# argsim/argsim

Hardware: AMD Instinct MI355X
Metric: sentences/sec per ELBO step (higher is better)
Workload: dtype f32; 1 GPU; BASELINE configs[1]: 1xMI355X fp32, latent_dim 128, vocab 8k, seq_len 64, batch 256 per GPU; FULL synthetic Zipf batches, dim_emb 512, 3 layers, step 20000; global_batch=256, seq_len=64, parallelism=dp1, gru=persistent

## Files before the change

argsim_amd/csrc/ctx.h:

```cpp
#pragma once
#include "../../include/argsim_vae.h"
#include "kernels.h"

#include <fcntl.h>
#include <sys/file.h>
#include <unistd.h>

#include <algorithm>
#include <cmath>
#include <cstdio>
#include <cstring>
#include <initializer_list>
#include <string>
#include <vector>

#pragma GCC visibility push(hidden)
namespace avae { namespace host {

struct ParamEntry {
    std::string name;
    int64_t offset;
    int ndim;
    int64_t shape[4];
    int g16;
    int bucket;
};

struct GruP { int64_t W, R, bW, bR; };

}}
#pragma GCC visibility pop

struct avae_ctx {
    avae_config cfg{};
    int device = 0;
    hipStream_t stream = nullptr;
    std::string err;
    std::vector<avae::host::ParamEntry> params;
    int64_t numel = 0;
    std::vector<std::pair<int64_t, int64_t>> buckets;
    float *P = nullptr, *G = nullptr, *M = nullptr, *Vv = nullptr;
    int64_t step = 0;
    avae_grad_hook hook = nullptr; void* hook_user = nullptr;
    std::vector<int> hook_pending;
    int persistent = 1;
    bool first_step_checked = false;
    int gru_ablate = 0, gru_force_slow = 0, gru_stagger = 0, gru_item = 2;
    int skinny = 1;
    int score_plan[4] = {0, 0, 0, 0};
    const int* expect_ptr[3] = {nullptr, nullptr, nullptr}; int expect_val[3] = {0, 0, 0};
    int compact = 2;
    int skip_pad = 1;
    int shared_device = 0; int lock_fd = -1;
    int dyn_split = 1;
    int dyn_thin = 1;
    int enc_top1 = 1;
    int table_l1 = 1;
    int bf16_act = 1;
    int bf16_sv = 1;
    int bf16_tn = 1;
    int logits16 = 1;
    int bf16_nt8 = 1;
    int bf16_direct = 0;
    int gru_spec = 2;
    int gru_ring = 1;
    int bwd_rs = 2;
    int knn_chunk = 0;
    int agg_chunk = 0;
    int ward_form = 0;
    int probe_chunk = 0;
    int gru_bf16 = 1;
    int64_t oE = 0, oKout = 0, oBout = 0, oWmu = 0, oBmu = 0, oWlv = 0, oBlv = 0, oWex = 0, oBex = 0;
    std::vector<avae::host::GruP> enc;
    std::vector<avae::host::GruP> dec;
    float* losses = nullptr;
    float* acc = nullptr;
    int* errw = nullptr;
    unsigned* counters = nullptr;
    float* scratch = nullptr;
    int64_t scratch_n = 0;
    char* ws = nullptr; size_t ws_cap = 0;
    int B = 0, Ss = 0, St = 0;
    int timing = 0, timing_on = 0;
    unsigned short *bfA = nullptr, *bfB = nullptr; size_t bfA_cap = 0, bfB_cap = 0;
    float* slab = nullptr; size_t slab_floats = 0;
    unsigned short* bfP = nullptr; size_t bfP_cap = 0;
    struct Stamp { hipEvent_t a, b; int cls; double flops; const int* dyn; int dyn_max; };
    std::vector<Stamp> stamps; size_t stamps_used = 0;
    int32_t* hint_dev = nullptr; volatile int32_t* hint_host = nullptr;
    const int32_t *cnt_src = nullptr, *cnt_tgt = nullptr;
};

#pragma GCC visibility push(hidden)
namespace avae { namespace host {

#define AV_CHECK(expr)                                                                              \
    do { hipError_t e_ = (expr); if (e_ != hipSuccess) {                                            \
        char b_[512]; snprintf(b_, sizeof b_, "%s:%d: %s -> %s", __FILE__, __LINE__, #expr, hipGetErrorString(e_)); \
        h->err = b_; return 1; } } while (0)
#define AV_TRY(expr) do { int r_ = (expr); if (r_) return r_; } while (0)

inline int fail(avae_ctx* h, const std::string& m) { h->err = m; return 1; }
inline int check_rows(avae_ctx* h, const char* what, int dim, const char* names, std::initializer_list<const void*> ptrs)
{
    if (dim < 4 || dim > 1024 || (dim & 3)) return fail(h, std::string(what) + ": dim must be a multiple of 4 in [4, 1024]");
    uintptr_t bits = 0;
    for (const void* p : ptrs) bits |= (uintptr_t)p;
    if (bits & 15) return fail(h, std::string(what) + ": " + names + " must be 16-byte aligned");
    return 0;
}

#define AV_GRU(expr)                                                                                                \
    do { hipError_t e_ = (expr);                                                                                    \
         if (e_ == hipErrorCooperativeLaunchTooLarge)                                                               \
             return fail(h, "persistent GRU kernel: its workgroups cannot all be resident on this device at once (occupancy query x CU count < grid); " \
                            "run with avae_set_option(\"persistent\", 0)");                                         \
         if (e_ != hipSuccess) { char b_[512]; snprintf(b_, sizeof b_, "%s:%d: %s -> %s", __FILE__, __LINE__, #expr, hipGetErrorString(e_)); \
             h->err = b_; return 1; } } while (0)

struct DeviceTurn {
    avae_ctx* h; bool held = false;
    explicit DeviceTurn(avae_ctx* h_) : h(h_) {
        if (!h->shared_device || !h->persistent) return;
        if (h->lock_fd < 0) {
            char path[64]; snprintf(path, sizeof path, "/tmp/argsim_vae_dev%d.lock", h->device);
            h->lock_fd = open(path, O_CREAT | O_RDWR, 0666);
        }
        if (h->lock_fd >= 0 && flock(h->lock_fd, LOCK_EX) == 0) held = true;
    }
    ~DeviceTurn() { if (held) { (void)hipStreamSynchronize(h->stream); (void)flock(h->lock_fd, LOCK_UN); } }
};

struct Timed {
    avae_ctx* h; avae_ctx::Stamp* s = nullptr;
    Timed(avae_ctx* h_, int cls, double flops, const int* dyn = nullptr, int dyn_max = 0) : h(h_) {
        if (!h->timing) return;
        if (h->stamps_used == h->stamps.size()) {
            avae_ctx::Stamp n{};
            if (hipEventCreate(&n.a) != hipSuccess || hipEventCreate(&n.b) != hipSuccess) return;
            h->stamps.push_back(n);
        }
        s = &h->stamps[h->stamps_used++];
        s->cls = cls; s->flops = flops; s->dyn = dyn; s->dyn_max = dyn_max;
        (void)hipEventRecord(s->a, h->stream);
    }
    ~Timed() { if (s) (void)hipEventRecord(s->b, h->stream); }
};

struct Ws {
    int32_t *src_tm, *lens_src, *lens_tgt, *lead, *gold, *rank, *cidx, *ntok, *pred;
    float *emb_src, *emb_tgt, *ew, *dew;
    std::vector<float*> e_gi, e_hs, e_sv[2], e_hp[2];
    std::vector<float*> d_gi, d_hd, d_sv, d_hp;
    float *hpick, *mu, *lv, *z, *eps, *kld, *h0;
    float *xlast, *gib, *svb, *dgib, *dghb, *dxl;
    float *hc, *ho, *logits;
    float *loss_samp, *errt_samp;
    float *dho, *dhc, *dhd[2], *dgi_d, *dgh_d, *dh0, *carry, *dh0sum, *dz, *dmu, *dlv, *dhpick;
    float *dhs[2], *dgi_e, *dgh_e, *demb_src, *demb_tgt;
    std::vector<unsigned short*> e_hs16, d_hd16, e_hp16[2], d_hp16;
    std::vector<char> act_e, act_d, acth_e, acth_d;
    std::vector<unsigned short*> x16_e, x16_d;
    const unsigned short* x16_kept_e(int i) const { return x16_valid ? x16_e[i] : nullptr; }
    const unsigned short* x16_kept_d(int i) const { return x16_valid ? x16_d[i] : nullptr; }
    bool x16_valid = false;
    unsigned short *dgi16_d, *dgh16_d, *dgi16_e, *dgh16_e;
    int32_t* scat;
    int32_t *grp_src, *grp_tgt;
    int32_t *tokrow_src, *tokrow_tgt;
    float* xbuf; size_t xbuf_floats;
    int32_t *ord_perm[3], *ord_slens[3]; int ord_T[3], ord_cpj[3]; bool ord_ok[3];
    int32_t *map_src, *nact_src, *nsrc; bool compact;
    int32_t *map_tgt, *nact_tgt, *ntgt; bool compact_d;
    int Bx;
    int bx_enc() const { return compact ? Bx : 0; }
    int bx_dec() const { return compact_d ? Bx : 0; }
};

struct Bump {
    char* base; size_t off = 0;
    template <class T> T* take(size_t n) {
        off = (off + 255) & ~(size_t)255;
        T* p = base ? reinterpret_cast<T*>(base + off) : nullptr;
        off += n * sizeof(T);
        return p;
    }
    template <class T> T* opt(bool on, size_t n) { return on ? take<T>(n) : nullptr; }
};

struct Pair { const float* A; const float* B; float* C; const float* bias; };

struct GemmCall {
    const float* A; int lda; bool a_mc;
    const float* B; int ldb; bool b_nc;
    float* C; int ldc;
    int M, N, K;
    float alpha = 1.f; const float* bias = nullptr; int accumulate = 0;
    const int* dyn = nullptr; int dyn_kind = 0;
    const Pair* pair = nullptr;
    bool wgrad = false;
    bool allow_atomic = false;
    bool rows_are_batch = false;
    int thin = -1, split_k = 0;
    const unsigned short* A16 = nullptr; const unsigned short* B16 = nullptr;
    unsigned short* keep_a16 = nullptr;
    unsigned short* c16 = nullptr;

    GemmCall& scaled(float a) { alpha = a; return *this; }
    GemmCall& biased(const float* b) { bias = b; return *this; }
    GemmCall& plus() { accumulate = 1; return *this; }
    GemmCall& rows(const int* d) { dyn = d; dyn_kind = d ? 1 : 0; return *this; }
    GemmCall& depth(const int* d) { dyn = d; dyn_kind = d ? 2 : 0; return *this; }
    GemmCall& with(const Pair* p) { pair = p; return *this; }
    GemmCall& atomic() { allow_atomic = true; return *this; }
    GemmCall& batch_rows() { rows_are_batch = true; return *this; }
    GemmCall& form(int thin_, int split_k_ = 1) { thin = thin_; split_k = split_k_; return *this; }
    GemmCall& a16(const unsigned short* p) { A16 = p; return *this; }
    GemmCall& b16(const unsigned short* p) { B16 = p; return *this; }
    GemmCall& keep(unsigned short* p) { keep_a16 = p; return *this; }
};
inline GemmCall nt(const float* A, int lda, const float* B, int ldb, float* C, int ldc, int M, int N, int K) { return GemmCall{A, lda, false, B, ldb, false, C, ldc, M, N, K}; }
inline GemmCall nn(const float* A, int lda, const float* B, int ldb, float* C, int ldc, int M, int N, int K) { return GemmCall{A, lda, false, B, ldb, true, C, ldc, M, N, K}; }
inline GemmCall tn_grad(const float* A, int lda, const float* B, int ldb, float* C, int ldc, int M, int N, int K)
{
    GemmCall c{A, lda, true, B, ldb, true, C, ldc, M, N, K};
    c.wgrad = true;
    return c;
}

bool use_table(const avae_ctx* h, int rows, int B);
void layout(avae_ctx* h, Bump& b, Ws& w, int B, int Ss, int St, bool train);
int reserve_ws(avae_ctx* h, size_t need);
inline int reserve_named(avae_ctx* h, size_t need, const char* what)
{
    if (reserve_ws(h, need)) {
        (void)hipGetLastError();
        char b[256]; snprintf(b, sizeof b, "%s: the device cannot give the workspace of %zu bytes this call needs", what, need);
        h->err = b;
        return 1;
    }
    return 0;
}
int get_ws(avae_ctx* h, Ws& w, int B, int Ss, int St, bool train);
int gemm(avae_ctx* h, const GemmCall& c);
int gemm_tn16(avae_ctx* h, const GemmCall& c);
void gru_geometry(int D, int njobs, int B, int* G, int* rpg);
void gru_common(avae_ctx* h, const Ws& w, GruArgs& a, int njobs, int S, int B, int ldg, int ldh, const int32_t* lens, int Bx);
int build_row_orders(avae_ctx* h, Ws& w, int B, int Ss, int T, bool with_dec, bool with_enc = true);
int build_compact_dec(avae_ctx* h, Ws& w, int B, int T);
int run_decoder_rnn(avae_ctx* h, Ws& w, int B, int T, const float* state_in, int64_t state_stride, bool save, const int32_t* ids0 = nullptr, bool compact = false,
                    const int32_t* share_rows = nullptr, int share_n = 0);
int run_logits_ce(avae_ctx* h, Ws& w, int rt, bool train, float inv_n);
int encode_ws(avae_ctx* h, Ws& w, const int32_t* src, int b, int t);
inline PrepArgs prep_from_ws(const Ws& w)
{
    PrepArgs p{};
    p.src_tm = w.src_tm; p.lens_src = w.lens_src; p.lens_tgt = w.lens_tgt; p.lead = w.lead; p.gold = w.gold;
    p.rank = w.rank; p.cidx = w.cidx; p.ntok = w.ntok; p.chunk_counts = w.ntok + 4;
    return p;
}

int grow_scratch(avae_ctx* h, size_t need, const char* what);
int check_gru_err(avae_ctx* h);
int dyn_fraction(avae_ctx* h, const avae_ctx::Stamp& s, std::vector<std::pair<const int*, int>>& seen, double* f);
inline int check_bound(avae_ctx* h)
{
    if (!h->P || !h->G || !h->M || !h->Vv) return fail(h, "state buffers not bound (avae_bind_state)");
    return 0;
}
template <class F> int place_scratch(avae_ctx* h, const char* what, F lay)
{
    Bump probe{nullptr};
    lay(probe);
    AV_TRY(grow_scratch(h, probe.off, what));
    Bump real{reinterpret_cast<char*>(h->scratch)};
    lay(real);
    return 0;
}
template <class F> int place_ws(avae_ctx* h, const char* what, F lay, size_t from = 0)
{
    Bump probe{nullptr, from};
    lay(probe);
    AV_TRY(reserve_named(h, probe.off + 4096, what));
    Bump real{h->ws, from};
    lay(real);
    return 0;
}

bool sample_params(avae_ctx* h, const avae_sample_config* sc, int V, SampleParams* sp);
bool sample_params_p(avae_ctx* h, const avae_sample_p_config* sc, int V, SampleParams* sp, float* top_p);

}}
#pragma GCC visibility pop
```

argsim_amd/csrc/handle.cpp:

```cpp
#include "ctx.h"

using namespace avae;
using namespace avae::host;

static std::string g_create_err;

namespace avae { namespace host {

int grow_scratch(avae_ctx* h, size_t need, const char* what)
{
    if (h->scratch_n >= (int64_t)need) return 0;
    AV_CHECK(hipStreamSynchronize(h->stream));
    if (h->scratch) AV_CHECK(hipFree(h->scratch));
    h->scratch = nullptr; h->scratch_n = 0;
    if (hipMalloc(reinterpret_cast<void**>(&h->scratch), need) != hipSuccess) {
        (void)hipGetLastError();
        h->scratch = nullptr;
        char b_[256]; snprintf(b_, sizeof b_, "%s: %.0f MB of scratch could not be allocated on the device", what, (double)need / 1048576.0);
        return fail(h, b_);
    }
    h->scratch_n = (int64_t)need;
    return 0;
}

// ... 69 lines not shown
int check_gru_err(avae_ctx* h)
{
    int e = 0;
    AV_CHECK(hipMemcpyAsync(&e, h->errw, sizeof(int), hipMemcpyDeviceToHost, h->stream));
    AV_CHECK(hipStreamSynchronize(h->stream));
    if (e) {
        (void)hipMemsetAsync(h->errw, 0, sizeof(int), h->stream);
        return fail(h, "GRU persistent kernel: an exchange wait timed out -- its workgroups were not all resident at once.  A persistent "
                       "launch needs every CU of the device (one handle = one GPU = one process, include/argsim_vae.h): another process or "
                       "stream computing on this GPU holds CUs the launch is waiting for.  Give the handle the device to itself, or "
                       "run with avae_set_option(\"persistent\", 0) (one launch per time step)");
    }
    return 0;
}
int dyn_fraction(avae_ctx* h, const avae_ctx::Stamp& s, std::vector<std::pair<const int*, int>>& seen, double* f)
{
    *f = 1.0;
    if (!s.dyn || s.dyn_max <= 0) return 0;
    int c = -1;
    for (auto& e : seen) if (e.first == s.dyn) c = e.second;
    if (c < 0) {
        AV_CHECK(hipMemcpy(&c, s.dyn, sizeof(int), hipMemcpyDeviceToHost));
        if (c < 0) c = 0;
        seen.push_back({s.dyn, c});
    }
    *f = (double)std::min(c, s.dyn_max) / (double)s.dyn_max;
    return 0;
}

}}

extern "C" {

int avae_create(const avae_config* cfg, int device, avae_handle* out)
{
    if (!cfg || !out) { g_create_err = "null argument"; return 1; }
    *out = nullptr;
    if (!gru_dim_supported(cfg->dim_emb)) { g_create_err = "dim_emb must be one of 16, 32, 64, 128, 256, 512 (the GRU kernels are instantiated for these widths only; the reference leaves dim_emb free, config.json uses 512)"; return 1; }
    if (cfg->compute_dtype < 0 || cfg->compute_dtype > 2) { g_create_err = "compute_dtype must be 0 (fp32 MFMA), 1 (bf16 GEMM operands) or 2 (fp32 via split bf16 MFMA)"; return 1; }
    if (cfg->dim_rep % 4 || cfg->dim_tgt % 4 || cfg->rnn_layers < 1 || cfg->rnn_layers > 8) { g_create_err = "dim_rep and dim_tgt must be multiples of 4 (16-byte rows); 1 <= rnn_layers <= 8"; return 1; }
    int ndev = 0;
    if (hipGetDeviceCount(&ndev) != hipSuccess || ndev <= 0) { g_create_err = "no HIP device available: the gfx950 kernels cannot run (no CPU fallback)"; return 1; }
    if (device < 0 || device >= ndev) { g_create_err = "bad device index"; return 1; }
    avae_ctx* h = new avae_ctx();
    h->cfg = *cfg; h->device = device;
    if (h->cfg.kl_beta == 0.f) h->cfg.kl_beta = 1.f;
    build_params(h);
    hipError_t e = hipSetDevice(device);
    if (e == hipSuccess) e = hipMalloc(reinterpret_cast<void**>(&h->losses), 64 * sizeof(float));
    if (e == hipSuccess) e = hipMalloc(reinterpret_cast<void**>(&h->errw), 128 * sizeof(int));
    if (e == hipSuccess) e = hipMalloc(reinterpret_cast<void**>(&h->counters), 2048 * sizeof(unsigned));
    if (e == hipSuccess) e = hipMemset(h->losses, 0, 64 * sizeof(float));
    if (e == hipSuccess) e = hipMemset(h->errw, 0, 128 * sizeof(int));
    if (e == hipSuccess) e = hipMemset(h->counters, 0, 2048 * sizeof(unsigned));
    if (e != hipSuccess) { g_create_err = std::string("hip init failed: ") + hipGetErrorString(e); delete h; return 1; }
    h->acc = h->losses + 8;
    *out = h;
    return 0;
}

void avae_destroy(avae_handle h)
{
    if (!h) return;
    (void)hipSetDevice(h->device);
    if (h->stream) (void)hipStreamSynchronize(h->stream); else (void)hipDeviceSynchronize();
    if (h->ws) (void)hipFree(h->ws);
    if (h->losses) (void)hipFree(h->losses);
    if (h->errw) (void)hipFree(h->errw);
    if (h->hint_host) (void)hipHostFree(const_cast<int32_t*>(h->hint_host));
    if (h->counters) (void)hipFree(h->counters);
    if (h->scratch) (void)hipFree(h->scratch);
    if (h->bfA) (void)hipFree(h->bfA);
    if (h->slab) (void)hipFree(h->slab);
    if (h->bfP) (void)hipFree(h->bfP);
    if (h->bfB) (void)hipFree(h->bfB);
    if (h->lock_fd >= 0) (void)close(h->lock_fd);
    delete h;
}

const char* avae_last_error(avae_handle h) { return h ? h->err.c_str() : g_create_err.c_str(); }

int avae_set_stream(avae_handle h, void* s) { if (!h) return 1; h->stream = reinterpret_cast<hipStream_t>(s); return 0; }

int avae_get_dims(avae_handle h, int32_t* V, int32_t* D, int32_t* R, int32_t* L)
{
    if (!h) return 1;
    if (V) *V = h->cfg.dim_tgt; if (D) *D = h->cfg.dim_emb; if (R) *R = h->cfg.dim_rep; if (L) *L = h->cfg.rnn_layers;
    return 0;
}

int64_t avae_state_numel(avae_handle h) { return h ? h->numel : 0; }

int avae_bind_state(avae_handle h, float* p, float* g, float* m, float* v)
{
    if (!h) return 1;
    if (((uintptr_t)p | (uintptr_t)g | (uintptr_t)m | (uintptr_t)v) & 15) return fail(h, "state buffers must be 16-byte aligned");
    h->P = p; h->G = g; h->M = m; h->Vv = v;
    return 0;
}

int avae_param_count(avae_handle h) { return h ? (int)h->params.size() : 0; }
const char* avae_param_name(avae_handle h, int i) { return (h && i >= 0 && i < (int)h->params.size()) ? h->params[i].name.c_str() : nullptr; }

int avae_param_info(avae_handle h, const char* name, int64_t* offset, int32_t* ndim, int64_t shape[4])
{
    if (!h) return 1;
    const ParamEntry* e = find_param(h, name);
    if (!e) return fail(h, std::string("unknown variable: ") + (name ? name : "(null)"));
    if (offset) *offset = e->offset; if (ndim) *ndim = e->ndim;
    if (shape) for (int i = 0; i < 4; ++i) shape[i] = e->shape[i];
    return 0;
}

static int xfer_tensor(avae_handle h, const char* name, int kind, float* buf, bool get)
{
    if (!h) return 1;
    AV_TRY(check_bound(h));
    const ParamEntry* e = find_param(h, name);
    if (!e) return fail(h, std::string("unknown variable: ") + (name ? name : "(null)"));
    float* base = state_buf(h, kind);
    if (!base) return fail(h, "bad tensor kind");
    float* flat = base + e->offset;
    int64_t n = e->shape[0] * e->shape[1] * e->shape[2] * e->shape[3];
    if (!e->g16) {
        AV_CHECK(hipMemcpyAsync(get ? buf : flat, get ? flat : buf, n * sizeof(float), hipMemcpyDeviceToDevice, h->stream));
    } else {
        int D = h->cfg.dim_emb, cols = (int)(e->ndim == 2 ? e->shape[1] : 1);
        if (get) AV_CHECK(g16_permute(h->stream, buf, flat, D, cols, false));
        else     AV_CHECK(g16_permute(h->stream, flat, buf, D, cols, true));
    }
    return 0;
}
int avae_get_tensor(avae_handle h, const char* name, int kind, float* buf) { return xfer_tensor(h, name, kind, buf, true); }
int avae_set_tensor(avae_handle h, const char* name, int kind, const float* buf) { return xfer_tensor(h, name, kind, const_cast<float*>(buf), false); }

int avae_get_step(avae_handle h, int64_t* s) { if (!h || !s) return 1; *s = h->step; return 0; }
int avae_set_step(avae_handle h, int64_t s) { if (!h) return 1; h->step = s; return 0; }

int avae_set_grad_hook(avae_handle h, avae_grad_hook hook, void* user) { if (!h) return 1; h->hook = hook; h->hook_user = user; return 0; }

int avae_set_option(avae_handle h, const char* key, int value)
{
    if (!h || !key) return 1;
    if (!strcmp(key, "persistent")) { h->persistent = value; return 0; }
    if (!strcmp(key, "gru_item")) { h->gru_item = value; return 0; }
    if (!strcmp(key, "gru_stagger")) { h->gru_stagger = value; return 0; }
    if (!strcmp(key, "gru_force_slow")) { h->gru_force_slow = value; return 0; }
    if (!strcmp(key, "gru_bf16")) { h->gru_bf16 = value != 0; return 0; }
    if (!strcmp(key, "bwd_rs")) { h->bwd_rs = value; return 0; }
    if (!strcmp(key, "dyn_split")) { h->dyn_split = value != 0; return 0; }
    if (!strcmp(key, "shared_device")) { h->shared_device = value != 0; return 0; }
    if (!strcmp(key, "gru_spec")) { h->gru_spec = value; return 0; }
    if (!strcmp(key, "gru_ring")) { h->gru_ring = value != 0; return 0; }
    if (!strcmp(key, "bf16_nt8")) { h->bf16_nt8 = value != 0; return 0; }
    if (!strcmp(key, "logits16")) { h->logits16 = value != 0; return 0; }
    if (!strcmp(key, "bf16_direct")) { h->bf16_direct = value != 0; return 0; }
    if (!strcmp(key, "bf16_tn")) { h->bf16_tn = value != 0; return 0; }
    if (!strcmp(key, "bf16_sv")) { h->bf16_sv = value != 0; return 0; }
    if (!strcmp(key, "bf16_act")) { h->bf16_act = value != 0; return 0; }
    if (!strcmp(key, "table_l1")) { h->table_l1 = value != 0; return 0; }
    if (!strcmp(key, "enc_top1")) { h->enc_top1 = value != 0; return 0; }
    if (!strcmp(key, "dyn_thin")) { h->dyn_thin = value != 0; return 0; }
    if (!strcmp(key, "skip_pad")) { h->skip_pad = value != 0; return 0; }
    if (!strcmp(key, "compact")) { h->compact = value; return 0; }
    if (!strcmp(key, "skinny")) { h->skinny = value; return 0; }
    if (!strcmp(key, "knn_chunk")) { if (value < 0) return fail(h, "knn_chunk must be >= 0"); h->knn_chunk = value; return 0; }
    if (!strcmp(key, "agg_chunk")) { if (value < 0) return fail(h, "agg_chunk must be >= 0"); h->agg_chunk = value; return 0; }
    if (!strcmp(key, "ward_form")) { if (value < 0 || value > 2) return fail(h, "ward_form must be 0 (planner), 1 (one-workgroup) or 2 (launch-per-merge)"); h->ward_form = value; return 0; }
    if (!strcmp(key, "probe_chunk")) { if (value < 0) return fail(h, "probe_chunk must be >= 0"); h->probe_chunk = value; return 0; }
    if (!strcmp(key, "gru_ablate")) {
        if (value && !gru_diag_build()) return fail(h, "gru_ablate needs the diagnostic build of libargsim_vae.so (make -C argsim_amd/csrc DIAG=1)");
        h->gru_ablate = value; return 0;
    }
    if (!strcmp(key, "timing")) { h->timing = value; h->timing_on = value; h->stamps_used = 0; return 0; }
    if (!strcmp(key, "timing_pause")) { h->timing = value ? 0 : h->timing_on; return 0; }
    return fail(h, "unknown option");
}
int avae_timing_collect(avae_handle h, double* out)
{
    if (!h || !out) return 1;
    AV_CHECK(hipStreamSynchronize(h->stream));
    for (int i = 0; i < 9; ++i) out[i] = 0.0;
    std::vector<std::pair<const int*, int>> seen;
    for (size_t i = 0; i < h->stamps_used; ++i) {
        float ms = 0.f;
        AV_CHECK(hipEventElapsedTime(&ms, h->stamps[i].a, h->stamps[i].b));
        double f = 1.0;
        AV_TRY(dyn_fraction(h, h->stamps[i], seen, &f));
        int c = h->stamps[i].cls;
        out[3 * c] += ms; out[3 * c + 1] += 1.0; out[3 * c + 2] += h->stamps[i].flops * f;
    }
    h->stamps_used = 0;
    return 0;
}
int avae_bucket_count(avae_handle h) { return h ? (int)h->buckets.size() : 0; }
int avae_bucket_info(avae_handle h, int i, int64_t* offset, int64_t* count)
{
    if (!h || i < 0 || i >= (int)h->buckets.size()) return 1;
    *offset = h->buckets[i].first; *count = h->buckets[i].second; return 0;
}

}
```

argsim_amd/csrc/hooks.cpp:

```cpp
#include "ctx.h"

using namespace avae;
using namespace avae::host;

extern "C" {

int avae_debug_team_batch(int32_t B) { return B > 0 ? gru_team_batch(B) : 0; }
int avae_debug_gemm_plan(const int32_t* in, int32_t n, int32_t* out)
{
    if (!in || !out || n < 0) return 1;
    for (int r = 0; r < n; ++r, in += 19, out += 15) {
        const GemmShape s{in[0] != 0, in[1] != 0, in[2], in[3], in[4], in[5], in[6], in[7], in[8], in[9], in[10], in[11] != 0, in[12] != 0,
                          in[13] != 0, in[14] != 0, in[15], in[16] != 0, in[17] != 0, in[18] != 0};
        const GemmPlan p = gemm_plan(s);
        out[0] = p.n;
        for (int i = 0; i < 2; ++i) {
            const GemmLaunch l = i < p.n ? p.launch[i] : GemmLaunch{0, 0, 0, 0, 0, 0, 0};
            const int32_t f[7] = {l.row0, l.rows, l.thin, l.split_k, l.accumulate, l.zero, l.dyn};
            std::copy(f, f + 7, out + 1 + 7 * i);
        }
    }
    return 0;
}
int avae_debug_gemm_call(avae_handle h, int a_mc, int b_nc, const float* A, const float* Bm, float* Cm, const float* bias, int M, int N, int K,
// ... 22 lines not shown
        return fail(h, "avae_debug_gemm_forced: thin in 0..3, split_k >= 1, dyn_kind in 0..2 with a count exactly where it is not 0");
    GemmCall c{A, lda, a_mc != 0, Bm, ldb, b_nc != 0, Cm, ldc, M, N, K};
    c.alpha = alpha; c.bias = bias; c.accumulate = accumulate;
    if (dyn_kind == 2) c.depth(count); else c.rows(count);
    c.form(thin, split_k);
    const Pair second{A2, B2, C2, bias2};
    if (A2) c.pair = &second;
    const int* const was_ptr = h->expect_ptr[0]; const int was_val = h->expect_val[0];
    h->expect_ptr[0] = count; h->expect_val[0] = expect;
    const int r = gemm(h, c);
    h->expect_ptr[0] = was_ptr; h->expect_val[0] = was_val;
    return r;
}
int avae_debug_gemm_f32_form(int a_mc, int b_nc, int M, int N, int K, int lda, int ldb, int ldc, int accumulate, int thin, int split_k, int dyn_kind,
                             int expect, int pair, int32_t out[8])
{
    if (!out) return 1;
    alignas(16) static const float other[4] = {0.f, 0.f, 0.f, 0.f};
    const GemmArgs g{nullptr, nullptr, nullptr, nullptr, M, N, K, lda, ldb, ldc, 1.f, accumulate, split_k, nullptr, dyn_kind, expect, thin,
                     pair ? other : nullptr, pair ? other : nullptr, nullptr, nullptr};
    const GemmF32Form f = gemm_f32_form(a_mc != 0, b_nc != 0, g);
    const int32_t v[8] = {f.tile, f.fast, f.db, f.persist, (int32_t)f.gx, (int32_t)f.gy, (int32_t)f.gz, f.err != hipSuccess};
    std::copy(v, v + 8, out);
    return 0;
}
int avae_debug_score_plan(avae_handle h, int32_t out[4])
{
    if (!h || !out) return 1;
    for (int i = 0; i < 4; ++i) out[i] = h->score_plan[i];
    return 0;
}
int avae_debug_present_ids(avae_handle h, int32_t out[2])
{
    if (!h || !out) return 1;
    AV_CHECK(hipStreamSynchronize(h->stream));
    out[0] = out[1] = -1;
    if (h->cnt_src) AV_CHECK(hipMemcpy(&out[0], h->cnt_src, sizeof(int), hipMemcpyDeviceToHost));
    if (h->cnt_tgt) AV_CHECK(hipMemcpy(&out[1], h->cnt_tgt, sizeof(int), hipMemcpyDeviceToHost));
    return 0;
}
int avae_debug_train_ce(avae_handle h, float* out, int32_t max_n, int32_t* n_out)
{
    if (!h || !out || !n_out) return 1;
    if (h->B < 1) return fail(h, "avae_debug_train_ce: no training forward has run on this handle");
    Ws w;
    AV_TRY(get_ws(h, w, h->B, h->Ss, h->St, true));
    int n = 0;
    AV_CHECK(hipMemcpyAsync(&n, w.ntok, sizeof(int), hipMemcpyDeviceToHost, h->stream));
    AV_CHECK(hipStreamSynchronize(h->stream));
    n = std::min(n, (int)max_n);
    AV_CHECK(hipMemcpyAsync(out, w.loss_samp, (size_t)n * sizeof(float), hipMemcpyDeviceToDevice, h->stream));
    *n_out = n;
    return 0;
}
int avae_debug_timing(avae_handle h, double* out, int max_n, int* n)
{
    if (!h || !out || !n) return 1;
    AV_CHECK(hipStreamSynchronize(h->stream));
    *n = (int)std::min<size_t>(h->stamps_used, (size_t)max_n);
    std::vector<std::pair<const int*, int>> seen;
    for (int i = 0; i < *n; ++i) {
        float ms = 0.f;
        AV_CHECK(hipEventElapsedTime(&ms, h->stamps[i].a, h->stamps[i].b));
        double f = 1.0;
        AV_TRY(dyn_fraction(h, h->stamps[i], seen, &f));
        const double fl = h->stamps[i].flops * f;
        out[3 * i] = h->stamps[i].cls; out[3 * i + 1] = ms; out[3 * i + 2] = fl;
    }
    return 0;
}
int avae_debug_stamps(avae_handle h, unsigned long long* out)
{
    if (!h || !out) return 1;
    AV_CHECK(hipStreamSynchronize(h->stream));
    AV_CHECK(hipMemcpy(out, h->errw + 16, 32 * sizeof(unsigned long long), hipMemcpyDeviceToHost));
    AV_CHECK(hipMemset(h->errw + 16, 0, 32 * sizeof(unsigned long long)));
    return 0;
}
int avae_debug_gemm(avae_handle h, int a_mc, int b_nc, const float* A, const float* Bm, float* Cm, const float* bias,
                    int M, int N, int K, int lda, int ldb, int ldc, float alpha, int accumulate, int split_k)
{
    if (!h) return 1;
    GemmCall c{A, lda, a_mc != 0, Bm, ldb, b_nc != 0, Cm, ldc, M, N, K};
    c.alpha = alpha; c.bias = bias; c.accumulate = accumulate;
    return gemm(h, c.form(split_k == -3 ? 3 : (split_k < 0 ? 1 : (split_k >= 1000 ? 2 : 0)), split_k < 0 ? 1 : (split_k >= 1000 ? split_k - 1000 : split_k)));
}
int avae_debug_gemm_dyn(avae_handle h, const float* A, const float* Bm, float* Cm, int M, int N, int K, const int* rows)
{
    if (!h) return 1;
    return gemm(h, nt(A, K, Bm, K, Cm, N, M, N, K).rows(rows).form(0));
}
int avae_debug_gemm_c16(avae_handle h, const float* A, const float* Bm, unsigned short* C16, int M, int N, int K, float alpha, const int* rows)
{
    if (!h) return 1;
    if (h->cfg.compute_dtype != 1 || !gemm_bf16_c16_takes(M, N, K, rows, h->bf16_nt8)) return 3;
    GemmCall c = nt(A, K, Bm, K, nullptr, N, M, N, K).scaled(alpha).rows(rows).form(0);
    c.c16 = C16;
    return gemm(h, c);
}
int avae_debug_gemm_tn16(avae_handle h, const float* A, const float* Bm, float* Cm, int M, int N, int K, int lda, int ldb, int ldc, float alpha)
{
    if (!h) return 1;
    return gemm_tn16(h, tn_grad(A, lda, Bm, ldb, Cm, ldc, M, N, K).scaled(alpha));
}
int avae_debug_softmax_ce(avae_handle h, float* logits, unsigned short* panel, int logits16, const int32_t* gold, const int32_t* cidx,
                          const int32_t* n_dev, int n_max, int V, int write_grad, float inv_n, float* loss_samp, float* errt,
                          int32_t* pred, int* form_out)
{
    if (!h || !form_out) return 1;
    CeArgs c{};
    c.logits = logits; c.gold = gold; c.cidx = cidx; c.n_dev = n_dev; c.n_max = n_max; c.V = V;
    c.write_grad = write_grad; c.inv_n = inv_n;
    c.loss_samp = loss_samp; c.errt_samp = errt; c.pred = pred; c.loss_acc = nullptr;
    c.grad16 = panel; c.logits16 = logits16;
    *form_out = softmax_ce_form(c);
    AV_CHECK(softmax_ce(h->stream, c));
    return 0;
}
int avae_debug_argmax_rows(avae_handle h, const float* logits, int32_t* pred, int n, int V)
{
    if (!h) return 1;
    AV_CHECK(argmax_rows(h->stream, logits, pred, n, V));
    return 0;
}
int avae_debug_op_layout(int64_t n, int64_t V, int64_t out[6])
{
    if (!out || n < 0 || V < 0) return 1;
    int32_t base[1];
    out[0] = (int64_t)embed_scatter_scratch_ints((size_t)n, (size_t)V);
    out[1] = (int64_t)id_groups_ints((size_t)n, (size_t)V);
    out[2] = id_groups_rank(base, (int)n, (int)V) - base;
    out[3] = id_groups_uid(base, (int)n, (int)V) - base;
    out[4] = id_groups_count(base, (int)n, (int)V) - base;
    out[5] = id_groups_supported((int)V) ? 1 : 0;
    return 0;
}
int avae_debug_op(avae_handle h, const char* op, void* const* p, const int64_t* i, const float* f)
{
    if (!h || !op || !p || !i || !f) return 1;
    const std::string o(op);
    hipStream_t st = h->stream;
    auto F = [&](int k) { return static_cast<float*>(p[k]); };
    auto I = [&](int k) { return static_cast<int32_t*>(p[k]); };
    if (o == "prep_ids") {
        PrepArgs a{};
        a.src = I(0); a.tgt = I(1); a.keep_mask = static_cast<const uint8_t*>(p[2]); a.src_tm = I(3); a.lens_src = I(4); a.lens_tgt = I(5);
        a.lead = I(6); a.gold = I(7); a.rank = I(8); a.cidx = I(9); a.ntok = I(10); a.zero2 = F(11); a.chunk_counts = I(12);
        a.B = (int)i[0]; a.Ss = (int)i[1]; a.St = (int)i[2]; a.eos = (int)i[3]; a.bos = (int)i[4]; a.train = (int)i[5]; a.seed = (uint64_t)i[6];
        a.keepwd = f[0];
        AV_CHECK(prep_ids(st, a));
    } else if (o == "embed_gather") AV_CHECK(embed_gather(st, F(0), I(1), F(2), (int)i[0], (int)i[1], (int)i[2]));
    else if (o == "embed_scatter_add2") AV_CHECK(embed_scatter_add2(st, F(0), I(1), F(2), (int)i[0], I(3), F(4), (int)i[1], (int)i[2], (int)i[3], I(5)));
    else if (o == "id_groups_build") AV_CHECK(id_groups_build(st, I(0), (int)i[0], (int)i[1], I(1), i[2] != 0));
    else if (o == "rank_rows") AV_CHECK(rank_rows(st, I(0), I(1), I(2), (int)i[0], (int)i[1]));
    else if (o == "rows_gather_ranked") AV_CHECK(rows_gather_ranked(st, F(0), F(1), I(2), I(3), (int)i[0], (int)i[1], (int)i[2]));
    else if (o == "rows_group_sum") AV_CHECK(rows_group_sum(st, F(0), I(1), F(2), (int)i[0], (int)i[1], (int)i[2], I(3)));
    else if (o == "rows_add_indexed") AV_CHECK(rows_add_indexed(st, F(0), F(1), I(2), I(3), (int)i[0], (int)i[1]));
    else if (o == "rows_gather") AV_CHECK(rows_gather(st, F(0), F(1), I(2), I(3), (int)i[0], (int)i[1], I(4)));
    else if (o == "rows_expand") AV_CHECK(rows_expand(st, F(0), F(1), I(2), (int)i[0], (int)i[1], I(3)));
    else if (o == "zero_rows_dyn") AV_CHECK(zero_rows_dyn(st, F(0), I(1), (int)i[0], (int)i[1]));
    else if (o == "zero_fill") AV_CHECK(zero_fill(st, p[0], (size_t)i[0]));
    else if (o == "row_order") {
        RowOrder ro[4];
        const int n = (int)i[0];
        for (int k = 0; k < std::min(n, 4); ++k) ro[k] = RowOrder{I(3 * k), (int)i[5 + 3 * k], (int)i[6 + 3 * k], (int)i[7 + 3 * k], I(3 * k + 1), I(3 * k + 2)};
        AV_CHECK(row_order(st, ro, n, (int)i[1], (int)i[2], (int)i[3], I(3 * std::min(std::max(n, 0), 4)), (int)i[4]));
    } else if (o == "row_map") AV_CHECK(row_map(st, I(0), (int)i[0], (int)i[1], (int)i[2], I(1), I(2), I(3)));
    else if (o == "pick_last") AV_CHECK(pick_last(st, F(0), F(1), I(2), (int)i[0], (int)i[1], I(3)));
    else if (o == "pick_last16") AV_CHECK(pick_last16(st, F(0), static_cast<const unsigned short*>(p[1]), I(2), (int)i[0], (int)i[1], I(3)));
    else if (o == "pick_last_add") AV_CHECK(pick_last_add(st, F(0), F(1), I(2), (int)i[0], (int)i[1], I(3)));
    else if (o == "pick_last_bwd") AV_CHECK(pick_last_bwd(st, F(0), F(1), I(2), (int)i[0], (int)i[1], (int)i[2]));
    else if (o == "latent_fwd") AV_CHECK(latent_fwd(st, F(0), F(1), F(2), F(3), F(4), F(5), (int)i[0], (int)i[1], (uint64_t)i[2], f[0], F(6)));
    else if (o == "latent_bwd") AV_CHECK(latent_bwd(st, F(0), F(1), F(2), F(3), F(4), F(5), (int)i[0], (int)i[1], f[0], f[1]));
    else if (o == "colsum") AV_CHECK(colsum(st, F(0), (int)i[0], (int)i[1], (int)i[2], F(1), I(2)));
    else if (o == "add3") AV_CHECK(add3(st, F(0), F(1), F(2), F(3), i[0]));
    else if (o == "finalize_losses") AV_CHECK(finalize_losses(st, F(0), F(1), I(2), (int)i[0], F(3), (int)i[1], f[0], f[1], f[2]));
    else if (o == "adam_tf") {
        const AdamArgs a{F(0), F(1), F(2), F(3), i[0], f[0], f[1], f[2], f[3], static_cast<const int*>(p[4])};
        AV_CHECK(adam_tf(st, a));
    } else if (o == "g16_permute") AV_CHECK(g16_permute(st, F(0), F(1), (int)i[0], (int)i[1], i[2] != 0));
    else if (o == "gru_first_step_fwd") AV_CHECK(gru_first_step_fwd(st, F(0), F(1), F(2), (int)i[0], F(3), (int)i[1], (int)i[2], I(4)));
    else if (o == "gru_first_step_bwd") AV_CHECK(gru_first_step_bwd(st, F(0), (int)i[0], F(1), F(2), F(3), (int)i[1], (int)i[2], I(4)));
    else return fail(h, "avae_debug_op: no such launcher: " + o);
    return 0;
}

static void gru_shape(const int64_t* i, GruArgs& a)
{
    a.njobs = (int)i[0]; a.S = (int)i[1]; a.B = (int)i[2]; a.D = (int)i[3]; a.ldg = (int)i[4]; a.ldh = (int)i[5]; a.Bx = (int)i[6];
    a.G = (int)i[7]; a.rows_per_group = (int)i[8]; a.p_begin = (int)i[9]; a.p_end = (int)i[10]; a.item_pipeline = (int)i[11];
    a.bf16 = (int)i[12]; a.bwd_rs = (int)i[13]; a.xbuf_floats = (size_t)std::max<int64_t>(i[14], 0);
    if (a.G == 0 && a.D >= 16 && a.njobs >= 1 && a.B >= 1) gru_geometry(a.D, a.njobs, a.B, &a.G, &a.rows_per_group);
}
static void gru_plan_out(const GruArgs& a, const GruPlan& p, int64_t out[10])
{
    const int64_t v[10] = {(int64_t)p.form, p.T, p.C, p.cpj, p.Bg, p.pipe, a.G, a.rows_per_group, (int64_t)gru_bwd_rs_xbuf_floats(a.njobs, p.Bg), p.ring};
    std::copy(v, v + 10, out);
}
int avae_debug_gru_plan(const int64_t* i, int fwd, int persistent, int64_t out[10])
{
    if (!i || !out) return 1;
    alignas(16) static float dummy[4] = {0.f, 0.f, 0.f, 0.f};
    GruArgs a{};
    gru_shape(i, a);
    a.xbuf = a.xbuf_floats > 0 ? dummy : nullptr; a.ring = 1;
    gru_plan_out(a, gru_plan(a, fwd != 0, persistent != 0), out);
    return 0;
}
int avae_debug_gru(avae_handle h, int fwd, int persistent, const int64_t* i, void* const* jobs, void* const* shared, int64_t plan_out[10])
{
    if (!h || !i || !jobs || !shared || !plan_out) return 1;
    GruArgs a{};
    gru_shape(i, a);
    if (a.njobs < 1 || a.njobs > kMaxGruJobs) return fail(h, "avae_debug_gru: njobs in 1..3");
    if (a.p_begin != 0 || a.p_end != a.S) return fail(h, "avae_debug_gru: whole-sequence launches only (p_begin = 0, p_end = S)");
    a.stagger = (int)i[15]; a.force_slow = (int)i[16]; a.sv16 = (int)i[17]; a.spec = (int)i[18];
    for (int k = 0; k < a.njobs; ++k) {
        void* const* p = jobs + 19 * k;
        auto F = [&](int q) { return static_cast<float*>(p[q]); };
        auto H = [&](int q) { return static_cast<unsigned short*>(p[q]); };
        GruJob& j = a.job[k];
        j.gi = F(0); j.gi_rows = static_cast<const int32_t*>(p[1]); j.R = F(2); j.bR = F(3); j.h0 = F(4); j.hs = F(5); j.sv = F(6); j.hp = F(7);
        j.hs16 = H(8); j.hp16 = H(9); j.dh_out = F(10); j.dgi = F(11); j.dgh = F(12); j.dgi16 = H(13); j.dgh16 = H(14); j.dh0 = F(15);
        j.carry = F(16); j.dbW = F(17); j.dbR = F(18);
        j.reverse = (int)i[19 + 2 * k]; j.dgi_by_pos = (int)i[20 + 2 * k];
    }
    a.lens = static_cast<const int*>(shared[0]); a.slens = static_cast<const int*>(shared[1]); a.perm = static_cast<const int*>(shared[2]);
    a.rowmap = static_cast<const int*>(shared[3]); a.xbuf = static_cast<float*>(shared[4]);
    a.counters = h->counters; a.err = h->errw; a.stamps = reinterpret_cast<unsigned long long*>(h->errw + 16); a.ablate = 0;
    a.ring = h->gru_ring;
    gru_plan_out(a, gru_plan(a, fwd != 0, persistent != 0), plan_out);
    AV_CHECK(hipSetDevice(h->device));
    AV_GRU(fwd ? gru_forward(h->stream, a, persistent != 0) : gru_backward(h->stream, a, persistent != 0));
    return check_gru_err(h);
}

int avae_debug_sample_rows(avae_handle h, const float* logits, int n, int V, int t0, const avae_sample_config* sc, int32_t* pred, float* logp)
{
    if (!h) return 1;
    SampleParams sp{};
    if (!sample_params(h, sc, V, &sp)) return 1;
    if (n < 1 || V < 1 || t0 < 0 || t0 >= (1 << 20)) return fail(h, "sample rows: bad shape or step");
    AV_CHECK(sample_rows(h->stream, logits, n, V, t0, sp, nullptr, h->cfg.eos, pred, logp));
    return 0;
}

int avae_debug_sample_rows_p(avae_handle h, const float* logits, int n, int V, int t0, const avae_sample_p_config* sc, int32_t* pred, float* logp,
                             int32_t* nkept, const int32_t* lead)
{
    if (!h) return 1;
    SampleParams sp{};
    float top_p = 0.f;
    if (!sample_params_p(h, sc, V, &sp, &top_p)) return 1;
    if (n < 1 || V < 1 || t0 < 0 || t0 >= (1 << 20)) return fail(h, "sample rows: bad shape or step");
    if (top_p > 0.f) AV_CHECK(sample_rows_p(h->stream, logits, n, V, t0, sp, top_p, lead, h->cfg.eos, pred, logp, nkept));
    else {
        AV_CHECK(sample_rows(h->stream, logits, n, V, t0, sp, lead, h->cfg.eos, pred, logp));
        if (nkept) AV_CHECK(hipMemsetAsync(nkept, 0xff, (size_t)n * sizeof(int32_t), h->stream));
    }
    return 0;
}

int avae_debug_beam_select(avae_handle h, const float* logits, int n, int width, int V, const float* cum, const int32_t* fin,
                           int32_t* parent, int32_t* token, float* cum_out, int32_t* fin_out)
{
    if (!h) return 1;
    if (!logits || !cum || !fin || !parent || !token || !cum_out || !fin_out) return fail(h, "beam select: every array must be given");
    if (n < 1 || n > (1 << 20) || V < 1 || width < 1 || width > 32 || width > V) return fail(h, "beam select: bad shape or width");
    AV_CHECK(hipSetDevice(h->device));
    const size_t rows = (size_t)n * width;
    float *cand_sc, *lat_cum; int32_t *cand_tok, *cand_cnt, *len_out, *live;
    AV_TRY(place_scratch(h, "beam select", [&](Bump& b) {
        cand_sc = b.take<float>(rows * width); lat_cum = b.take<float>(rows);
        cand_tok = b.take<int32_t>(rows * width); cand_cnt = b.take<int32_t>(rows); len_out = b.take<int32_t>(rows); live = b.take<int32_t>(1);
    }));
    AV_CHECK(beam_rows(h->stream, logits, (int)rows, V, width, cum, fin, h->cfg.eos, cand_sc, cand_tok, cand_cnt));
    BeamStep a{};
    a.n = n; a.Win = width; a.W = width; a.eos = h->cfg.eos;
    a.cand_sc = cand_sc; a.cand_tok = cand_tok; a.cand_cnt = cand_cnt; a.fin_in = fin; a.len_in = nullptr;
    a.lat_parent = parent; a.lat_token = token; a.lat_cum = lat_cum; a.cum_out = cum_out; a.fin_out = fin_out; a.len_out = len_out;
    a.live = live;
    AV_CHECK(hipMemsetAsync(a.live, 0, sizeof(int32_t), h->stream));
    AV_CHECK(beam_select(h->stream, a));
    return 0;
}
int avae_debug_latent_plan(int kind, int64_t n, int64_t N, int k_or_P, int dim, int chunk_opt, int32_t out[5])
{
    if (!out || kind < 0 || kind > 2 || n < 0 || n > 0x7fffffff || N < 0 || N > 0x7fffffff) return 1;
    if (kind == 0) { const KnnPlan p = knn_plan((int)n, (int)N, k_or_P, chunk_opt); const int32_t f[5] = {p.qrows, p.qtiles, 0, p.parts, p.chunk}; std::copy(f, f + 5, out); }
    else if (kind == 1) { const AggPlan p = agg_plan((int)n, (int)N, dim, chunk_opt); const int32_t f[5] = {0, p.qtiles, 0, p.parts, p.chunk}; std::copy(f, f + 5, out); }
    else { const ProbePlan p = probe_plan((int)N, k_or_P, dim, chunk_opt); const int32_t f[5] = {p.ptiles, p.Ppad, p.LD, p.parts, p.chunk}; std::copy(f, f + 5, out); }
    return 0;
}

}
```

argsim_amd/csrc/kernels.h:

```cpp
#pragma once
#include <hip/hip_runtime.h>
#include <stdint.h>

#include "gemm_plan.h"

namespace avae {

struct GemmArgs {
    const float* A; const float* B; float* C; const float* bias;
    int M, N, K, lda, ldb, ldc;
    float alpha;
    int accumulate;
    int split_k;
    const int* dyn; int dyn_kind;
    int dyn_expect;
    int thin;
    const float* A2; const float* B2; float* C2; const float* bias2;
    float* slab = nullptr; size_t slab_floats = 0;
    unsigned short* c16 = nullptr;
    int nt8 = 1;
};
hipError_t gemm_f32(hipStream_t st, bool a_mc, bool b_nc, const GemmArgs& g);
struct GemmF32Form { int tile; bool fast, db, persist; unsigned gx, gy, gz; hipError_t err; };
GemmF32Form gemm_f32_form(bool a_mc, bool b_nc, const GemmArgs& g);
hipError_t gemm_f32s(hipStream_t st, bool a_mc, bool b_nc, const GemmArgs& g);
hipError_t gemm_bf16_direct(hipStream_t st, bool a_mc, bool b_nc, const GemmArgs& g);

hipError_t cvt_bf16(hipStream_t st, const float* src, int ld, bool transpose, int rows_or_K, int cols_or_X,
                    unsigned short* dst, int ldd);
hipError_t gemm_bf16_nt(hipStream_t st, const unsigned short* A, int lda, const unsigned short* B, int ldb, const GemmArgs& g);
bool gemm_bf16_p8_ok(const GemmArgs& g, int lda, int ldb);
hipError_t gemm_bf16_p8(hipStream_t st, const unsigned short* A, int lda, const unsigned short* B, int ldb, const GemmArgs& g, int s2);
bool gemm_bf16_c16_ok(const GemmArgs& g, int lda, int ldb);
bool gemm_bf16_c16_takes(int M, int N, int K, const int* rows, int nt8);
bool gemm_bf16_p8_tn_ok(const GemmArgs& g, int lda, int ldb);
hipError_t gemm_bf16_p8_tn(hipStream_t st, const unsigned short* A, int lda, const unsigned short* B, int ldb, const GemmArgs& g, int s2);
hipError_t gemm_bf16_tn(hipStream_t st, const unsigned short* A, int lda, const unsigned short* B, int ldb, const GemmArgs& g);
hipError_t transpose_bf16(hipStream_t st, const unsigned short* src, int ld, int K, int X, unsigned short* dst, int ldk);

constexpr int kMaxGruJobs = 3;
struct GruJob {
    const float* gi;
    const int32_t* gi_rows;
    const float* R;
    const float* bR;
    const float* h0;
    float* hs;
    float* sv;
    float* hp;
    int reverse;
    unsigned short* hs16;
    unsigned short* hp16;
    const float* dh_out;
    float* dgi;
    float* dgh;
    unsigned short* dgi16;
    unsigned short* dgh16;
    float* dh0;
    float* carry;
    int dgi_by_pos;
    float* dbW;
    float* dbR;
};
struct GruArgs {
    GruJob job[kMaxGruJobs];
    int njobs, S, B, D, ldg, ldh;
    const int* lens;
    const int* slens;
    const int* perm;
    const int* rowmap;
    int Bx;
    int G;
    int rows_per_group;
    int p_begin, p_end;
    unsigned* counters;
    int* err;
    unsigned long long* stamps;
    int item_pipeline;
    float* xbuf;
    size_t xbuf_floats;
    int stagger;
    int force_slow;
    int sv16;
    int bf16;
    int spec;
    int bwd_rs;
    int ring;
    int ablate;
};
constexpr int kGruRing = 4;
enum class GruForm { stepwise, persistent, item, team, team_rs };
struct GruPlan {
    GruForm form;
    int T, C, cpj, Bg;
    bool pipe, diag;
    int ring;
    bool team() const { return form == GruForm::team || form == GruForm::team_rs; }
    bool full() const { return team() && !diag; }
};
GruPlan gru_plan(const GruArgs& a, bool fwd, bool persistent);
hipError_t gru_forward(hipStream_t st, const GruArgs& a, bool persistent);
hipError_t gru_backward(hipStream_t st, const GruArgs& a, bool persistent);
int gru_team_batch(int B);
bool gru_dim_supported(int D);
size_t gru_bwd_rs_xbuf_floats(int njobs, int rows);
hipError_t gru_bwd_rs_launch(hipStream_t st, const GruArgs& a, const GruPlan& p);
hipError_t gru_fwd_team_launch(hipStream_t st, const GruArgs& a, const GruPlan& p);
hipError_t gru_bwd_team_launch(hipStream_t st, const GruArgs& a, const GruPlan& p);
hipError_t gru_reg_launch(hipStream_t st, const GruArgs& a, bool fwd, int grid, bool need_resident);
hipError_t gru_fwd_item_launch(hipStream_t st, const GruArgs& a, int grid);
hipError_t gru_first_step_fwd(hipStream_t st, const float* gi, const float* bR, float* h_out, int ldo, float* sv, int B, int D, const int32_t* lens = nullptr);
hipError_t gru_first_step_bwd(hipStream_t st, const float* dh, int ldd, const float* sv, float* dgi, float* dgh, int B, int D, const int32_t* lens = nullptr);
bool gru_diag_build();

struct PrepArgs {
    const int32_t* src; const int32_t* tgt;
    int B, Ss, St, eos, bos;
    int train; float keepwd; uint64_t seed; const uint8_t* keep_mask;
    int32_t* src_tm;
    int32_t* lens_src;
    int32_t* lens_tgt;
    int32_t* lead;
    int32_t* gold;
    int32_t* rank;
    int32_t* cidx;
    int32_t* ntok;
    float* zero2;
    int32_t* chunk_counts;
};
constexpr int kPrepChunks = 1024;
hipError_t prep_ids(hipStream_t st, const PrepArgs& p);

hipError_t embed_gather(hipStream_t st, const float* E, const int32_t* ids, float* out, int n, int D, int V);
hipError_t embed_scatter_add2(hipStream_t st, float* dE, const int32_t* ids0, const float* dout0, int n0, const int32_t* ids1,
                              const float* dout1, int n1, int D, int V, int32_t* scratch);
bool id_groups_supported(int V);
inline size_t id_groups_ints(size_t n, size_t V) { return 4 * V + 2 + n + (n / 32 + V + 1) + 2 * V + 4; }
hipError_t id_groups_build(hipStream_t st, const int32_t* ids, int n, int V, int32_t* scratch, bool lists);
const int32_t* id_groups_rank(int32_t* scratch, int n, int V);
const int32_t* id_groups_uid(int32_t* scratch, int n, int V);
const int32_t* id_groups_count(int32_t* scratch, int n, int V);
hipError_t rank_rows(hipStream_t st, int32_t* out, const int32_t* ids, const int32_t* rank, int n, int V);
hipError_t rows_gather_ranked(hipStream_t st, float* dst, const float* src, const int32_t* ids, const int32_t* rank, int n, int W, int V);
hipError_t rows_group_sum(hipStream_t st, float* dst, const int32_t* ids, const float* src, int n, int W, int V, int32_t* scratch);
hipError_t rows_add_indexed(hipStream_t st, float* dst, const float* src, const int32_t* uid, const int32_t* nuniq, int n_max, int D);
inline size_t embed_scatter_scratch_ints(size_t n, size_t V) { return 4 * V + 2 + n + (n / 32 + V + 1); }
struct RowOrder { const int32_t* lens; int add, T, cpj; int32_t* perm; int32_t* slens; };
hipError_t row_order(hipStream_t st, const RowOrder* orders, int n, int Breal, int B, int S, int32_t* steps_sum = nullptr, int sum_rows = 0);
hipError_t rows_gather(hipStream_t st, float* dst, const float* src, const int32_t* idx, const int32_t* n_dev, int n_max, int D, const int32_t* map = nullptr);
hipError_t rows_expand(hipStream_t st, float* dst, const float* src, const int32_t* rank, int rows, int D, const int32_t* map = nullptr);
hipError_t pick_last(hipStream_t st, float* h, const float* hs, const int32_t* lens, int B, int W, const int32_t* map = nullptr);
hipError_t pick_last16(hipStream_t st, float* h, const unsigned short* hs16, const int32_t* lens, int B, int W, const int32_t* map = nullptr);
hipError_t pick_last_add(hipStream_t st, float* dhs, const float* d, const int32_t* lens, int B, int W, const int32_t* map = nullptr);
hipError_t row_map(hipStream_t st, const int32_t* lens, int add, int S, int B, int32_t* map, int32_t* nact, int32_t* count);
hipError_t zero_rows_dyn(hipStream_t st, float* X, const int32_t* count, int rows_max, int W);
hipError_t pick_last_bwd(hipStream_t st, float* dhs, const float* dh, const int32_t* lens, int S, int B, int W);

hipError_t latent_fwd(hipStream_t st, const float* mu, const float* lv, const float* eps_in, float* eps_out, float* z,
                      float* kld, int n, int train, uint64_t seed, float free_bits, float* acc);
hipError_t latent_bwd(hipStream_t st, const float* dz, const float* mu, const float* lv, const float* eps_used,
                      float* dmu, float* dlv, int B, int R, float coef, float free_bits);

struct CeArgs {
    float* logits;
    const int32_t* gold;
    const int32_t* cidx;
    const int32_t* n_dev;
    int n_max, V;
    int write_grad; float inv_n;
    float* loss_samp; float* errt_samp; int32_t* pred;
    float* loss_acc;
    unsigned short* grad16;
    int logits16;
};
int softmax_ce_form(const CeArgs& a);
hipError_t softmax_ce(hipStream_t st, const CeArgs& a);
hipError_t argmax_rows(hipStream_t st, const float* logits, int32_t* pred, int n, int V);
struct SampleParams { float inv_t; int top_k; int noise; uint64_t seed; };
hipError_t sample_rows(hipStream_t st, const float* logits, int n, int V, int t, const SampleParams& sp, const int32_t* lead, int eos,
                       int32_t* pred, float* logp);
hipError_t sample_rows_p(hipStream_t st, const float* logits, int n, int V, int t, const SampleParams& sp, float top_p, const int32_t* lead,
                         int eos, int32_t* pred, float* logp, int32_t* nkept);

hipError_t colsum(hipStream_t st, const float* X, int M, int N, int ldx, float* out, const int32_t* m_dev);
hipError_t add3(hipStream_t st, float* out, const float* a, const float* b, const float* c, int64_t n);
hipError_t zero_fill(hipStream_t st, void* p, size_t bytes);

struct AdamArgs { float* p; const float* g; float* m; float* v; int64_t n; float lr_t, b1, b2, eps;
                  const int* skip_if; };
hipError_t adam_tf(hipStream_t st, const AdamArgs& a);

struct ScoreDraw {
    const float* mu; const float* lv;
    const float* eps_in;
    float* eps_out;
    float* z;
    float* lat;
    int* err;
    int k, B, R, rc; uint64_t seed;
};
hipError_t score_draw(hipStream_t st, const ScoreDraw& a);
hipError_t tile_ids(hipStream_t st, int32_t* dst, const int32_t* src, int n, int rc, int S);
hipError_t lead_rows(hipStream_t st, const int32_t* lead, int T, int n, int rc, int32_t* ids0, int32_t* tokrow);
struct ScoreRows {
    const float* loss;
    const int32_t* rank;
    int T, n, rc, k0, r0, B;
    float* logpx;
    int32_t* ntok;
};
hipError_t score_rows(hipStream_t st, const ScoreRows& a);
hipError_t score_bound(hipStream_t st, const float* logpx, const float* lat, int k, int B, float* logw, float* bound);

hipError_t beam_rows(hipStream_t st, const float* logits, int rows, int V, int W, const float* cum, const int32_t* fin, int eos,
                     float* cand_sc, int32_t* cand_tok, int32_t* cand_cnt);
struct BeamStep {
    int n, Win, W, eos;
    const float* cand_sc; const int32_t* cand_tok; const int32_t* cand_cnt;
    const int32_t* fin_in; const int32_t* len_in;
    int32_t* lat_parent; int32_t* lat_token; float* lat_cum;
    float* cum_out; int32_t* fin_out; int32_t* len_out;
    int32_t* live;
};
hipError_t beam_select(hipStream_t st, const BeamStep& a);
hipError_t beam_gather(hipStream_t st, const float* const* hd, int L, int n, int Win, int W, int D, const int32_t* parent, float* state_out);
struct BeamEnd {
    int n, W, n_run, steps, eos;
    const int32_t* lat_parent; const int32_t* lat_token; const float* lat_cum;
    const float* cum; const int32_t* len;
    const float* lenpow;
    int32_t* out_ids;
    float* score_out; float* cum_out; int32_t* len_out;
    int32_t* o_parent; int32_t* o_token; float* o_cum; size_t out_step;
};
hipError_t beam_backtrack(hipStream_t st, const BeamEnd& a);

struct KnnArgs {
    const float* q; const float* bank;
    int n, N, dim, k, metric;
    int64_t idx_base, self_base; int carry;
    int64_t* out_idx; float* out_score;
};
struct KnnPlan { int qrows, qtiles, parts, chunk; };
KnnPlan knn_plan(int n, int N, int k, int chunk_opt);
struct KnnWs { float *qn, *bn; unsigned long long* lists; };
hipError_t knn_search(hipStream_t st, const KnnArgs& g, const KnnPlan& p, const KnnWs& w);

struct AggArgs {
    const float* z; const float* mu; const float* lv;
    int n, N, dim;
    int64_t self_base;
    float* logq; float* logqx;
};
struct AggPlan { int qtiles, parts, chunk; };
AggPlan agg_plan(int n, int N, int dim, int chunk_opt);
hipError_t agg_logq(hipStream_t st, const AggArgs& g, const AggPlan& p, float2* parts_ms);
int moments_blocks(int N);
hipError_t latent_moments(hipStream_t st, const float* mu, const float* lv, int N, int dim, float* out, double* mean, double* part);

constexpr int kProbeTile = 32;
constexpr int kProbeAlphas = 7;
constexpr int kProbeMaxParts = 256;
struct ProbePlan { int ptiles, Ppad, LD, parts, chunk; };
ProbePlan probe_plan(int N, int P, int dim, int chunk_opt);
struct ProbeWs {
    float *sT, *z, *D, *u;
    float *W, *G, *Dv, *Rv, *Pv;
    float *gp, *lp;
    double* tp;
    int* is; float* fs; double* ds;
    int N, dim, LD, Ppad, parts, chunk;
    float *Yv, *Hd, *Hy;
    float* xs;
};
struct ProbeAlphas { int n, last; float a[kProbeAlphas]; };
hipError_t probe_prepare(hipStream_t st, const ProbeWs& b, const float* s, int P);
hipError_t probe_pass(hipStream_t st, const ProbeWs& b, const float* x, int mode);
hipError_t probe_vec(hipStream_t st, const ProbeWs& b, int P, int phase, int k, int max_newton, int max_cg, float tol, const ProbeAlphas& al);
hipError_t probe_trial(hipStream_t st, const ProbeWs& b, const ProbeAlphas& al);
hipError_t probe_finish(hipStream_t st, const ProbeWs& b, int P, float* w, float* stats);
hipError_t probe_l1_prepare(hipStream_t st, const ProbeWs& b, const float* x, const float* s, int P);
hipError_t probe_l1_curv(hipStream_t st, const ProbeWs& b);
hipError_t probe_l1_vec(hipStream_t st, const ProbeWs& b, int P, int phase, int k, int max_newton, int max_inner, float tol, const ProbeAlphas& al);
hipError_t probe_decision(hipStream_t st, const ProbePlan& p, const float* x, int n, int dim, const float* w, int P, float* W, float* out);

constexpr int kWardOneWgMax = 128;
struct WardGroup {
    int off, n, mrg, pad;
    float* D;
    double* S;
    int* cnt;
    unsigned long long* nn;
    int* st;
};
struct WardCutGroup { int off, n, mrg, m; };
hipError_t ward_init(hipStream_t st, const WardGroup* gs, int G, int nmax, const float* x, int dim);
hipError_t ward_tree(hipStream_t st, const WardGroup* gs, int G, int nmax, int dim, int32_t* pair, float* delta, int32_t* size);
hipError_t ward_round(hipStream_t st, const WardGroup* gs, int G, int nmax, int dim, int t, int32_t* pair, float* delta, int32_t* size);
hipError_t ward_cut(hipStream_t st, const WardCutGroup* gs, int G, int nmax, const int32_t* pair, int32_t* p , int32_t* label);

constexpr int kApMaxN = 1 << 14;
constexpr int kApMaxRB = 16;
struct ApState {
    int stop_at;
    int iters, conv, K;
    int cnt[2][2];
    float pref;
    unsigned prefix[2], rank[2];
    unsigned hist[512];
};
struct ApBuffers {
    float *S, *A, *R;
    double* part;
    double* cv;
    int *E, *run, *E2;
    int32_t* c;
    unsigned long long* best;
    ApState* st;
};
int ap_row_block(int N);
hipError_t ap_single(hipStream_t st, int32_t* label, int32_t* stat);
hipError_t ap_similarity(hipStream_t st, const float* x, int N, int dim, int metric, float* S);
hipError_t ap_prepare(hipStream_t st, float* S, int N, int use_pref, float pref, int noise, uint64_t seed, ApState* state);
hipError_t ap_iteration(hipStream_t st, const ApBuffers& b, int N, float lam, int it, int conv_iter);
hipError_t ap_labels(hipStream_t st, const ApBuffers& b, int N, int32_t* label, int32_t* stat);

struct DecodeArgs {
    const float* E;
    const float *W[8], *R[8], *bW[8], *bR[8];
    const float *Kout, *bout;
    float* state[2];
    float* o;
    float* part_val; int32_t* part_idx;
    int32_t* ids_tm;
    int32_t* out_ids;
    int32_t* kept;
    unsigned* bar;
    int* err;
    int b, steps, D, V, L, eos, cache_e; float isd;
    SampleParams sp;
    float *part_x, *part_m, *part_s;
    float* logits;
    float* logp_tm;
    float* logp_out;
    float top_p;
    int32_t* nkept_tm;
    int32_t* nkept_out;
};
hipError_t decode_greedy(hipStream_t st, DecodeArgs a, int* grid_out);
hipError_t decode_sample(hipStream_t st, DecodeArgs a, int* grid_out);
int decode_workgroups();

hipError_t g16_permute(hipStream_t st, float* dst, const float* src, int D, int cols, bool to_g16);

hipError_t finalize_losses(hipStream_t st, float* losses, const float* loss_samp, const int32_t* n_dev, int n_max,
                           const float* kld, int nk, float free_bits, float inv_br, float anneal);

}
```

argsim_amd/csrc/model.cpp:

```cpp
#include "ctx.h"

using namespace avae;

namespace avae { namespace host {

static bool phantom_batch(const avae_ctx* h, int B)
{
    return h->compact && h->skip_pad && h->persistent && h->cfg.dim_emb == 512 && gru_team_batch(B) > B;
}
bool use_table(const avae_ctx* h, int rows, int B)
{
    if (!h->table_l1 || !id_groups_supported(h->cfg.dim_tgt)) return false;
    return rows >= h->cfg.dim_tgt || (rows >= 1024 && phantom_batch(h, B));
}

void layout(avae_ctx* h, Bump& b, Ws& w, int B, int Ss, int St, bool train)
{
    const int D = h->cfg.dim_emb, V = h->cfg.dim_tgt, R = h->cfg.dim_rep, L = h->cfg.rnn_layers;
    const size_t T = St + 1, rs = (size_t)Ss * B, rt = T * B;
    w.src_tm = b.take<int32_t>(rs); w.lens_src = b.take<int32_t>(B); w.lens_tgt = b.take<int32_t>(B);
    w.lead = b.take<int32_t>(rt); w.gold = b.take<int32_t>(rt); w.rank = b.take<int32_t>(rt);
    w.cidx = b.take<int32_t>(rt); w.ntok = b.take<int32_t>(4 + kPrepChunks); w.pred = b.take<int32_t>(rt);
    w.emb_src = b.take<float>(rs * D); w.emb_tgt = b.take<float>(rt * D);
    const bool tab_s = use_table(h, (int)rs, B), tab_t = use_table(h, (int)rt, B);
// ... 238 lines not shown
struct Sched { float keepwd, anneal, lr; };
static Sched schedule(const avae_ctx* h)
{
    float rate = h->cfg.accelerate * (float)h->step;
    Sched s;
    s.keepwd = 1.f / (1.f + expf(-rate));
    s.anneal = tanhf(rate);
    s.lr = h->cfg.learn_rate / (sqrtf(rate) + 1.f);
    return s;
}

static bool top_one_step(const avae_ctx* h) { return h->enc_top1 && h->cfg.rnn_layers >= 2; }

struct FillHint { int32_t real, rows; };
static FillHint fill_hint(const avae_ctx* h)
{
    const uint64_t pair = h->hint_host ? *reinterpret_cast<const volatile uint64_t*>(h->hint_host) : 0xffffffffull;
    return {(int32_t)(uint32_t)(pair & 0xffffffffull), (int32_t)(uint32_t)(pair >> 32)};
}
static double expected_fill(const avae_ctx* h)
{
    const FillHint f = fill_hint(h);
    return (f.real > 0 && f.rows > 0) ? std::min(1.0, (double)f.real / (double)f.rows) : 1.0;
}
static int rs_pick(const avae_ctx* h)
{
    if (h->bwd_rs != 2) return h->bwd_rs;
    return expected_fill(h) < 0.40 ? 1 : 0;
}
static int spec_pick(const avae_ctx* h)
{
    if (h->gru_spec != 2) return h->gru_spec;
    return expected_fill(h) < 0.60 ? 1 : 0;
}

void gru_common(avae_ctx* h, const Ws& w, GruArgs& a, int njobs, int S, int B, int ldg, int ldh, const int32_t* lens, int Bx)
{
    const int D = h->cfg.dim_emb;
    a.njobs = njobs; a.S = S; a.B = B; a.D = D; a.ldg = ldg; a.ldh = ldh; a.lens = lens;
    a.Bx = Bx;
    gru_geometry(D, njobs, B, &a.G, &a.rows_per_group);
    a.p_begin = 0; a.p_end = S; a.counters = h->counters; a.err = h->errw; a.ablate = h->gru_ablate; a.force_slow = h->gru_force_slow;
    a.bf16 = h->cfg.compute_dtype == 1 && h->gru_bf16; a.stagger = h->gru_stagger; a.item_pipeline = h->gru_item;
    a.xbuf = w.xbuf; a.xbuf_floats = w.xbuf_floats; a.stamps = reinterpret_cast<unsigned long long*>(h->errw + 16); a.bwd_rs = h->bwd_rs != 0;
    a.ring = h->gru_ring;
}
int build_row_orders(avae_ctx* h, Ws& w, int B, int Ss, int T, bool with_dec, bool with_enc)
{
    if (!h->skip_pad || !h->persistent || w.Bx % 16) return 0;
    if (w.Bx != B && !h->compact) return 0;
    const int D = h->cfg.dim_emb;
    RowOrder ord[3]; int n = 0, which[3];
    auto want = [&](int k, int njobs, int S, int ldg, int ldh, const int32_t* lens, int add) {
        GruArgs a{};
        gru_common(h, w, a, njobs, S, B, ldg, ldh, lens, w.Bx);
        const GruPlan p = gru_plan(a, true, true);
        if (p.form != GruForm::team) return;
        ord[n] = RowOrder{lens, add, p.T, p.cpj, w.ord_perm[k], w.ord_slens[k]};
        which[n++] = k; w.ord_T[k] = p.T; w.ord_cpj[k] = p.cpj;
    };
    if (with_enc) want(0, 2, Ss, 6 * D, 2 * D, w.lens_src, 0);
    if (with_enc && top_one_step(h)) want(1, 1, Ss, 6 * D, 2 * D, w.lens_src, 0);
    if (with_dec) want(2, 1, T, 3 * D, D, w.lens_tgt, 1);
    if (!n) return 0;
    const bool hint = which[0] == 0 && h->compact == 2;
    if (hint && !h->hint_host) {
        int32_t* hp = nullptr;
        if (hipHostMalloc(reinterpret_cast<void**>(&hp), 64, hipHostMallocDefault) == hipSuccess) { hp[0] = -1; hp[1] = 0; h->hint_host = hp; }
    }
    h->hint_dev = reinterpret_cast<int32_t*>(h->errw + 100);
    hipError_t e = row_order(h->stream, ord, n, B, w.Bx, std::max(Ss, T), hint ? h->hint_dev : nullptr, Ss * B);
    if (e == hipErrorInvalidValue) return 0;
    AV_CHECK(e);
    if (hint && h->hint_host) {
        AV_CHECK(hipMemcpyAsync(const_cast<int32_t*>(h->hint_host), h->hint_dev, 2 * sizeof(int32_t), hipMemcpyDeviceToHost, h->stream));
    }
    for (int i = 0; i < n; ++i) w.ord_ok[which[i]] = true;
    return 0;
}
static bool both_team_bf16(avae_ctx* h, const GruArgs& a, bool train)
{
    return train && a.bf16 && gru_plan(a, true, h->persistent != 0).full() && gru_plan(a, false, h->persistent != 0).full();
}
static void attach_sv16(avae_ctx* h, GruArgs& a, bool train) { a.sv16 = h->bf16_sv && both_team_bf16(h, a, train); }
static void attach_order(avae_ctx* h, const Ws& w, GruArgs& a, bool fwd, int k)
{
    const GruPlan p = gru_plan(a, fwd, h->persistent != 0);
    if (!w.ord_ok[k] || !p.team() || p.T != w.ord_T[k] || p.cpj != w.ord_cpj[k]) return;
    a.slens = w.ord_slens[k]; a.perm = w.ord_perm[k];
}

static int build_compact(avae_ctx* h, Ws& w, int B, int Ss, int T, bool train)
{
    w.compact = false; w.compact_d = false;
    h->expect_ptr[0] = h->expect_ptr[1] = h->expect_ptr[2] = nullptr;
    if (!h->compact || !h->persistent || Ss < 2 || !use_table(h, Ss * B, B)) return 0;
    const bool phantom = w.Bx != B;
    if (phantom && !(w.ord_ok[0] && (w.ord_ok[1] || !top_one_step(h)))) return 0;
    if (h->compact == 2 && !phantom) {
        const FillHint f = fill_hint(h);
        if (f.real < 0 || f.rows <= 0 || (double)f.real >= 0.92 * (double)f.rows) return 0;
    }
    const int D = h->cfg.dim_emb;
    auto team = [&](int njobs, int S, int ldg, int ldh, const int32_t* lens) {
        GruArgs q{};
        gru_common(h, w, q, njobs, S, B, ldg, ldh, lens, w.Bx);
        return gru_plan(q, true, true).full() && (!train || gru_plan(q, false, true).full());
    };
    if (!team(2, Ss, 6 * D, 2 * D, w.lens_src) || (top_one_step(h) && !team(1, Ss, 6 * D, 2 * D, w.lens_src))) return 0;
    AV_CHECK(row_map(h->stream, w.lens_src, 0, Ss, B, w.map_src, w.nact_src, w.nsrc));
    w.compact = true;
    {
        const FillHint f = fill_hint(h);
        const double fill = (f.real > 0 && f.rows > 0) ? std::min(1.0, (double)f.real / (double)f.rows) : 0.0;
        h->expect_ptr[0] = w.nsrc; h->expect_val[0] = (int)(fill * Ss * B);
        h->expect_ptr[1] = w.ntgt; h->expect_val[1] = (int)(fill * T * B);
        h->expect_ptr[2] = w.ntok; h->expect_val[2] = (int)(fill * T * B);
    }
    if (T < 2 || !use_table(h, T * B, B) || h->compact == 3) return 0;
    if ((phantom && !w.ord_ok[2]) || !team(1, T, 3 * D, D, nullptr)) return 0;
    AV_CHECK(row_map(h->stream, w.lens_tgt, 1, T, B, w.map_tgt, w.nact_tgt, w.ntgt));
    w.compact_d = true;
    return 0;
}
int build_compact_dec(avae_ctx* h, Ws& w, int B, int T)
{
    w.compact = false; w.compact_d = false;
    h->expect_ptr[0] = h->expect_ptr[1] = h->expect_ptr[2] = nullptr;
    if (!h->compact || h->compact == 3 || !h->persistent || T < 2 || !use_table(h, T * B, B)) return 0;
    if (w.Bx == B || !w.ord_ok[2]) return 0;
    GruArgs q{};
    gru_common(h, w, q, 1, T, B, 3 * h->cfg.dim_emb, h->cfg.dim_emb, nullptr, w.Bx);
    if (!gru_plan(q, true, true).full()) return 0;
    AV_CHECK(row_map(h->stream, w.lens_tgt, 1, T, B, w.map_tgt, w.nact_tgt, w.ntgt));
    w.compact_d = true;
    return 0;
}

static int run_encoder(avae_ctx* h, Ws& w, int B, int Ss, bool save)
{
    const int D = h->cfg.dim_emb, V = h->cfg.dim_tgt, L = h->cfg.rnn_layers;
    const int rs = Ss * B;
    const bool table = use_table(h, rs, B);
    h->cnt_src = table ? id_groups_count(w.grp_src, rs, V) : nullptr;
    const int32_t* const cdyn = w.compact ? w.nsrc : nullptr;
    const int32_t* const cmap = w.compact ? w.map_src : nullptr;
    if (!table) AV_CHECK(embed_gather(h->stream, h->P + h->oE, w.src_tm, w.emb_src, rs, D, V));
    const float* x = w.emb_src; int In = D;
    for (int i = 0; i < L; ++i) {
        const GruP& p = h->enc[i];
        const bool top1 = i == L - 1 && top_one_step(h);
        if (i == 0 && table) {
            const int32_t* cnt = id_groups_count(w.grp_src, rs, V);
            AV_CHECK(id_groups_build(h->stream, w.src_tm, rs, V, w.grp_src, save));
            AV_CHECK(rows_gather(h->stream, w.emb_src, h->P + h->oE, id_groups_uid(w.grp_src, rs, V), cnt, std::min(V, rs), D));
            AV_TRY(gemm(h, nt(w.emb_src, D, h->P + p.W, D, w.ew, 6 * D, std::min(V, rs), 6 * D, D).biased(h->P + p.bW).rows(cnt)));
        } else if (i > 0 && w.act_e[i - 1]) {
            AV_TRY(gemm_bf16_pre(h, nt(nullptr, In, h->P + p.W, In, w.e_gi[i], 6 * D, rs, top1 ? 3 * D : 6 * D, In).a16(w.e_hs16[i - 1]).biased(h->P + p.bW).rows(cdyn)));
        } else {
        AV_TRY(gemm(h, nt(x, In, h->P + p.W, In, w.e_gi[i], 6 * D, rs, top1 ? 3 * D : 6 * D, In).biased(h->P + p.bW).rows(cdyn).keep(save ? w.x16_e[i] : nullptr)));
        }
        GruArgs a{};
        gru_common(h, w, a, top1 ? 1 : 2, Ss, B, 6 * D, 2 * D, w.lens_src, w.bx_enc());
        const bool table0 = i == 0 && table, indirect = table0 && gru_plan(a, true, h->persistent != 0).form == GruForm::team;
        if (indirect) AV_CHECK(rank_rows(h->stream, w.tokrow_src, w.src_tm, id_groups_rank(w.grp_src, rs, V), rs, V));
        else if (table0) AV_CHECK(rows_gather_ranked(h->stream, w.e_gi[0], w.ew, w.src_tm, id_groups_rank(w.grp_src, rs, V), rs, 6 * D, V));
        for (int d = 0; d < a.njobs; ++d) {
            GruJob& j = a.job[d];
            j.gi = (indirect ? w.ew : w.e_gi[i]) + d * 3 * D;
            j.gi_rows = indirect ? w.tokrow_src : nullptr;
            j.R = h->P + p.R + (int64_t)d * 3 * D * D;
            j.bR = h->P + p.bR + d * 3 * D;
            j.h0 = nullptr;
            j.hs = w.e_hs[i] + d * D;
            j.sv = save ? w.e_sv[d][i] : nullptr;
            j.hp = save ? w.e_hp[d][i] : nullptr;
            j.reverse = d;
        }
        attach_sv16(h, a, save);
        if (w.e_hs16[i] && tn16_ok(h, 3 * D, D) && both_team_bf16(h, a, save)) {
            w.act_e[i] = 1; w.acth_e[i] = 1;
            for (int d = 0; d < a.njobs; ++d) { a.job[d].hs16 = w.e_hs16[i] + d * D; a.job[d].hp16 = w.e_hp16[d][i]; }
        }
        attach_order(h, w, a, true, top1 ? 1 : 0);
        a.rowmap = cmap;
        a.spec = spec_pick(h);
        { Timed t(h, 1, 2.0 * a.njobs * Ss * (double)B * D * 3 * D);
          DeviceTurn turn(h);
          AV_GRU(gru_forward(h->stream, a, h->persistent != 0)); }
        if (top1) {
            const int64_t oWb = p.W + (int64_t)3 * D * In;
            if (w.act_e[i - 1]) AV_CHECK(pick_last16(h->stream, w.xlast, w.e_hs16[i - 1], w.lens_src, B, In, cmap));
            else
            AV_CHECK(pick_last(h->stream, w.xlast, x, w.lens_src, B, In, cmap));
            AV_TRY(gemm(h, nt(w.xlast, In, h->P + oWb, In, w.gib, 3 * D, B, 3 * D, In).biased(h->P + p.bW + 3 * D).batch_rows()));
        }
        x = w.e_hs[i]; In = 2 * D;
    }
    if (w.act_e[L - 1]) AV_CHECK(pick_last16(h->stream, w.hpick, w.e_hs16[L - 1], w.lens_src, B, 2 * D, cmap));
    else
    AV_CHECK(pick_last(h->stream, w.hpick, w.e_hs[L - 1], w.lens_src, B, 2 * D, cmap));
    if (top_one_step(h))
        AV_CHECK(gru_first_step_fwd(h->stream, w.gib, h->P + h->enc[L - 1].bR + 3 * D, w.hpick + D, 2 * D, save ? w.svb : nullptr, B, D, w.lens_src));
    return 0;
}

static int run_latent(avae_ctx* h, Ws& w, int B, bool train, uint64_t seed, const float* eps)
{
    const int D = h->cfg.dim_emb, R = h->cfg.dim_rep;
    {
        const Pair lv{w.hpick, h->P + h->oWlv, w.lv, h->P + h->oBlv};
        AV_TRY(gemm(h, nn(w.hpick, 2 * D, h->P + h->oWmu, R, w.mu, R, B, R, 2 * D).biased(h->P + h->oBmu).with(&lv)));
    }
    AV_CHECK(latent_fwd(h->stream, w.mu, w.lv, eps, w.eps, w.z, w.kld, B * R, train ? 1 : 0, seed, h->cfg.free_bits, nullptr));
    return 0;
}

int run_decoder_rnn(avae_ctx* h, Ws& w, int B, int T, const float* state_in, int64_t state_stride, bool save, const int32_t* ids0, bool compact, const int32_t* share_rows, int share_n)
{
    const int32_t* const cdyn = compact ? w.ntgt : nullptr;
    const int32_t* const cmap = compact ? w.map_tgt : nullptr;
    const int D = h->cfg.dim_emb, L = h->cfg.rnn_layers;
    const int rt = T * B;
    const float* x = w.emb_tgt;
    h->cnt_tgt = ids0 ? id_groups_count(w.grp_tgt, rt, h->cfg.dim_tgt) : nullptr;
    for (int i = 0; i < L; ++i) {
        const GruP& p = h->dec[i];
        if (i == 0 && ids0) {
            const int V = h->cfg.dim_tgt;
            const int32_t* cnt = id_groups_count(w.grp_tgt, rt, V);
            AV_CHECK(id_groups_build(h->stream, ids0, rt, V, w.grp_tgt, save));
            AV_CHECK(rows_gather(h->stream, w.emb_tgt, h->P + h->oE, id_groups_uid(w.grp_tgt, rt, V), cnt, std::min(V, rt), D));
            AV_TRY(gemm(h, nt(w.emb_tgt, D, h->P + p.W, D, w.ew, 3 * D, std::min(V, rt), 3 * D, D).biased(h->P + p.bW).rows(cnt)));
        } else if (i == 0 && share_rows) {
            AV_TRY(gemm(h, nt(x, D, h->P + p.W, D, w.d_gi[0], 3 * D, share_n, 3 * D, D).biased(h->P + p.bW)));
        } else if (i > 0 && w.act_d[i - 1]) {
            AV_TRY(gemm_bf16_pre(h, nt(nullptr, D, h->P + p.W, D, w.d_gi[i], 3 * D, rt, 3 * D, D).a16(w.d_hd16[i - 1]).biased(h->P + p.bW).rows(cdyn)));
        } else {
        AV_TRY(gemm(h, nt(x, D, h->P + p.W, D, w.d_gi[i], 3 * D, rt, 3 * D, D).biased(h->P + p.bW).rows(cdyn).keep(save ? w.x16_d[i] : nullptr)));
        }
        GruArgs a{};
        gru_common(h, w, a, 1, T, B, 3 * D, D, nullptr, compact ? w.Bx : 0);
        GruJob& j = a.job[0];
        const bool table0 = i == 0 && ids0, indirect = table0 && gru_plan(a, true, h->persistent != 0).form == GruForm::team;
        if (indirect) AV_CHECK(rank_rows(h->stream, w.tokrow_tgt, ids0, id_groups_rank(w.grp_tgt, rt, h->cfg.dim_tgt), rt, h->cfg.dim_tgt));
        else if (table0) AV_CHECK(rows_gather_ranked(h->stream, w.d_gi[0], w.ew, ids0, id_groups_rank(w.grp_tgt, rt, h->cfg.dim_tgt), rt, 3 * D, h->cfg.dim_tgt));
        j.gi = indirect ? w.ew : w.d_gi[i]; j.gi_rows = indirect ? w.tokrow_tgt : nullptr;
        if (i == 0 && share_rows) j.gi_rows = share_rows;
        j.R = h->P + p.R; j.bR = h->P + p.bR;
        j.h0 = state_in + state_stride * i;
        j.hs = w.d_hd[i];
        j.sv = save ? w.d_sv[i] : nullptr;
        j.hp = save ? w.d_hp[i] : nullptr;
        j.reverse = 0;
        attach_sv16(h, a, save);
        if (w.d_hp16[i] && tn16_ok(h, 3 * D, D) && both_team_bf16(h, a, save)) {
            if (i < L - 1) { w.act_d[i] = 1; j.hs16 = w.d_hd16[i]; }
            w.acth_d[i] = 1; j.hp16 = w.d_hp16[i];
        }
        if (T > 1) attach_order(h, w, a, true, 2);
        a.rowmap = cmap;
        a.spec = spec_pick(h);
        { Timed t(h, 1, 2.0 * T * (double)B * D * 3 * D);
          DeviceTurn turn(h);
          AV_GRU(gru_forward(h->stream, a, h->persistent != 0)); }
        x = w.d_hd[i];
    }
    return 0;
}

static int forward(avae_ctx* h, Ws& w, const int32_t* src, const int32_t* tgt, int B, int Ss, int St, bool train,
            uint64_t seed, const uint8_t* keep_mask, const float* eps, float inv_n)
{
    const int D = h->cfg.dim_emb, V = h->cfg.dim_tgt, R = h->cfg.dim_rep;
    const int T = St + 1, rt = T * B;
    Sched sc = schedule(h);
    PrepArgs p = prep_from_ws(w);
    p.src = src; p.tgt = tgt; p.B = B; p.Ss = Ss; p.St = St; p.eos = h->cfg.eos; p.bos = h->cfg.bos;
    p.train = train ? 1 : 0; p.keepwd = sc.keepwd; p.seed = seed; p.keep_mask = keep_mask;
    AV_CHECK(prep_ids(h->stream, p));
    AV_TRY(build_row_orders(h, w, B, Ss, T, true));
    AV_TRY(build_compact(h, w, B, Ss, T, train));
    AV_TRY(run_encoder(h, w, B, Ss, train));
    AV_TRY(run_latent(h, w, B, train, seed, eps));
    AV_TRY(gemm(h, nn(w.z, R, h->P + h->oWex, D, w.h0, D, B, D, R).biased(h->P + h->oBex).batch_rows()));
    if (use_table(h, rt, B)) AV_TRY(run_decoder_rnn(h, w, B, T, w.h0, 0, train, w.lead, w.compact_d));
    else {
        AV_CHECK(embed_gather(h->stream, h->P + h->oE, w.lead, w.emb_tgt, rt, D, V));
        AV_TRY(run_decoder_rnn(h, w, B, T, w.h0, 0, train));
    }
    AV_TRY(run_logits_ce(h, w, rt, train, inv_n));
    float beta = h->cfg.kl_beta;
    AV_CHECK(finalize_losses(h->stream, h->losses, w.loss_samp, w.ntok, rt, w.kld, B * R, h->cfg.free_bits, 1.f / ((float)B * R), sc.anneal * beta));
    return 0;
}

int run_logits_ce(avae_ctx* h, Ws& w, int rt, bool train, float inv_n)
{
    const int D = h->cfg.dim_emb, V = h->cfg.dim_tgt, L = h->cfg.rnn_layers;
    AV_CHECK(rows_gather(h->stream, w.hc, w.d_hd[L - 1], w.cidx, w.ntok, rt, D, w.compact_d ? w.map_tgt : nullptr));
    AV_TRY(gemm(h, nn(w.hc, D, h->P + h->oKout, D, w.ho, D, rt, D, D).biased(h->P + h->oBout).rows(w.ntok)));
    CeArgs c{};
    c.logits = w.logits; c.gold = w.gold; c.cidx = w.cidx; c.n_dev = w.ntok; c.n_max = rt; c.V = V;
    c.write_grad = train ? 1 : 0; c.inv_n = inv_n;
    if (train && h->cfg.compute_dtype == 1 && (V & 7) == 0) {
        AV_TRY(grow_bf16(h, &h->bfP, &h->bfP_cap, (size_t)rt * V));
        c.grad16 = h->bfP;
        if (h->logits16 && !h->bf16_direct && gemm_bf16_c16_takes(rt, V, D, w.ntok, h->bf16_nt8)) c.logits16 = 1;
    }
    GemmCall lg = nt(w.ho, D, h->P + h->oE, D, w.logits, V, rt, V, D).scaled(1.f / sqrtf((float)D)).rows(w.ntok);
    if (c.logits16) lg.form(0).c16 = h->bfP;
    AV_TRY(gemm(h, lg));
    c.loss_samp = w.loss_samp; c.errt_samp = w.errt_samp; c.pred = w.pred; c.loss_acc = nullptr;
    AV_CHECK(softmax_ce(h->stream, c));
    return 0;
}

static void fire_hook(avae_ctx* h, int bucket)
{
    if (h->hook && bucket >= 0 && bucket < (int)h->buckets.size()) h->hook_pending.push_back(bucket);
}
static void hook_fence(avae_ctx* h)
{
    if (h->hook) h->hook(h->hook_user, AVAE_HOOK_FENCE, 0, 0);
}
static void hook_flush(avae_ctx* h)
{
    for (int b : h->hook_pending) h->hook(h->hook_user, b, h->buckets[b].first, h->buckets[b].second);
    h->hook_pending.clear();
}

static int backward(avae_ctx* h, Ws& w, int B, int Ss, int St, float b_global)
{
    const int D = h->cfg.dim_emb, V = h->cfg.dim_tgt, R = h->cfg.dim_rep, L = h->cfg.rnn_layers;
    const int T = St + 1, rt = T * B, rs = Ss * B;
    const float isd = 1.f / sqrtf((float)D);
    Sched sc = schedule(h);
    hipStream_t st = h->stream;
    float* G = h->G; const float* P = h->P;
    h->hook_pending.clear();
    AV_CHECK(zero_fill(st, G, sizeof(float) * h->numel));

    if (h->cfg.compute_dtype == 1 && (V & 7) == 0) {
        AV_TRY(gemm_bf16_pre(h, nn(nullptr, V, P + h->oE, D, w.dho, D, rt, D, V).a16(h->bfP).scaled(isd).rows(w.ntok)));
        const GemmCall dE = tn_grad(nullptr, V, w.ho, D, G + h->oE, D, V, D, rt).a16(h->bfP).scaled(isd).depth(w.ntok);
        AV_TRY(tn16_ok(h, V, D) ? gemm_tn16(h, dE) : gemm_bf16_pre(h, dE));
    } else {
    AV_TRY(gemm(h, nn(w.logits, V, P + h->oE, D, w.dho, D, rt, D, V).scaled(isd).rows(w.ntok).atomic()));
    AV_TRY(gemm(h, tn_grad(w.logits, V, w.ho, D, G + h->oE, D, V, D, rt).scaled(isd).depth(w.ntok)));
    }
    AV_TRY(gemm(h, tn_grad(w.hc, D, w.dho, D, G + h->oKout, D, D, D, rt).depth(w.ntok)));
    AV_CHECK(colsum(st, w.dho, rt, D, D, G + h->oBout, w.ntok));
    AV_TRY(gemm(h, nt(w.dho, D, P + h->oKout, D, w.dhc, D, rt, D, D).rows(w.ntok).atomic()));
    fire_hook(h, 0);
    const int32_t* const ddyn = w.compact_d ? w.ntgt : nullptr;
    const int32_t* const dmap = w.compact_d ? w.map_tgt : nullptr;
    AV_CHECK(rows_expand(st, w.dhd[0], w.dhc, w.rank, rt, D, dmap));

    int cur = 0;
    for (int i = L - 1; i >= 0; --i) {
        const GruP& p = h->dec[i];
        GruArgs a{};
        gru_common(h, w, a, 1, T, B, 3 * D, D, nullptr, w.bx_dec());
        GruJob& j = a.job[0];
        j.R = P + p.R; j.sv = w.d_sv[i]; j.hp = w.d_hp[i]; j.reverse = 0;
        j.dh_out = w.dhd[cur]; j.dgi = w.dgi_d; j.dgh = w.dgh_d;
        j.dh0 = w.dh0 + (size_t)i * B * D; j.carry = w.carry;
        j.dbW = G + p.bW; j.dbR = G + p.bR;
        const bool team16 = tn16_ok(h, 3 * D, D) && a.bf16 && gru_plan(a, false, h->persistent != 0).full();
        const bool g16 = team16 && !(i == 0 && use_table(h, rt, B));
        const bool gh16 = !g16 && w.dgh16_d && team16 && w.acth_d[i];
        if (g16) { j.dgi16 = w.dgi16_d; j.dgh16 = w.dgh16_d; }
        if (gh16) j.dgh16 = w.dgh16_d;
        if (!g16 && !gh16 && w.acth_d[i]) return fail(h, "internal: the forward kept this layer's h_prev as bf16 only and the backward cannot read it");
        if (w.acth_d[i]) j.hp16 = w.d_hp16[i];
        attach_sv16(h, a, true);
        attach_order(h, w, a, false, 2);
        a.rowmap = dmap;
        if (dmap && i == 0) j.dgi_by_pos = 1;
        a.bwd_rs = rs_pick(h); a.spec = spec_pick(h);
        hook_fence(h);
        { Timed t(h, 2, 2.0 * T * (double)B * D * 3 * D);
          DeviceTurn turn(h);
          AV_GRU(gru_backward(st, a, h->persistent != 0)); }
        hook_flush(h);
        if (i == 0 && use_table(h, rt, B)) {
            const int32_t* cnt = id_groups_count(w.grp_tgt, rt, V); const int U = std::min(V, rt);
            AV_CHECK(rows_group_sum(st, w.dew, w.lead, w.dgi_d, rt, 3 * D, V, w.grp_tgt));
            AV_TRY(gemm(h, tn_grad(w.dew, 3 * D, w.emb_tgt, D, G + p.W, D, 3 * D, D, U).depth(cnt)));
            if (gh16) AV_TRY(gemm_tn16(h, tn_grad(nullptr, 3 * D, nullptr, D, G + p.R, D, 3 * D, D, rt).a16(w.dgh16_d).b16(w.d_hp16[i]).depth(ddyn)));
            else
            AV_TRY(gemm(h, tn_grad(w.dgh_d, 3 * D, w.d_hp[i], D, G + p.R, D, 3 * D, D, rt).depth(ddyn)));
            AV_TRY(gemm(h, nn(w.dew, 3 * D, P + p.W, D, w.demb_tgt, D, U, D, 3 * D).rows(cnt).atomic()));
            AV_CHECK(rows_add_indexed(st, G + h->oE, w.demb_tgt, id_groups_uid(w.grp_tgt, rt, V), cnt, U, D));
        } else if (g16) {
            const float* x = i == 0 ? w.emb_tgt : w.d_hd[i - 1];
            AV_TRY(gemm_tn16(h, tn_grad(nullptr, 3 * D, x, D, G + p.W, D, 3 * D, D, rt).a16(w.dgi16_d).b16((i > 0 && w.act_d[i - 1]) ? w.d_hd16[i - 1] : w.x16_kept_d(i)).depth(ddyn)));
            AV_TRY(gemm_tn16(h, tn_grad(nullptr, 3 * D, w.d_hp[i], D, G + p.R, D, 3 * D, D, rt).a16(w.dgh16_d).b16(w.acth_d[i] ? w.d_hp16[i] : nullptr).depth(ddyn)));
            float* dx = i == 0 ? w.demb_tgt : w.dhd[cur ^ 1];
            AV_TRY(gemm_bf16_pre(h, nn(nullptr, 3 * D, P + p.W, D, dx, D, rt, D, 3 * D).a16(w.dgi16_d).rows(ddyn)));
        } else {
        const float* x = i == 0 ? w.emb_tgt : w.d_hd[i - 1];
        {
            const Pair dR{w.dgh_d, w.d_hp[i], G + p.R, nullptr};
            AV_TRY(gemm(h, tn_grad(w.dgi_d, 3 * D, x, D, G + p.W, D, 3 * D, D, rt).depth(ddyn).with(&dR)));
        }
        float* dx = i == 0 ? w.demb_tgt : w.dhd[cur ^ 1];
        AV_TRY(gemm(h, nn(w.dgi_d, 3 * D, P + p.W, D, dx, D, rt, D, 3 * D).rows(ddyn).atomic()));
        }
        cur ^= 1;
        fire_hook(h, 1 + (L - 1 - i));
    }

    AV_CHECK(add3(st, w.dh0sum, w.dh0, L > 1 ? w.dh0 + (size_t)B * D : nullptr, L > 2 ? w.dh0 + (size_t)2 * B * D : nullptr, (int64_t)B * D));
    for (int i = 3; i < L; ++i) AV_CHECK(add3(st, w.dh0sum, w.dh0sum, w.dh0 + (size_t)i * B * D, nullptr, (int64_t)B * D));
    AV_TRY(gemm(h, tn_grad(w.z, R, w.dh0sum, D, G + h->oWex, D, R, D, B)));
    AV_CHECK(colsum(st, w.dh0sum, B, D, D, G + h->oBex, nullptr));
    AV_TRY(gemm(h, nt(w.dh0sum, D, P + h->oWex, D, w.dz, R, B, R, D)));
    float bg = b_global > 0.f ? b_global : (float)B;
    AV_CHECK(latent_bwd(st, w.dz, w.mu, w.lv, w.eps, w.dmu, w.dlv, B, R, sc.anneal * h->cfg.kl_beta / (bg * R), h->cfg.free_bits));
    {
        const Pair dlv{w.hpick, w.dlv, G + h->oWlv, nullptr};
        AV_TRY(gemm(h, tn_grad(w.hpick, 2 * D, w.dmu, R, G + h->oWmu, R, 2 * D, R, B).with(&dlv)));
    }
    AV_CHECK(colsum(st, w.dmu, B, R, R, G + h->oBmu, nullptr));
    AV_CHECK(colsum(st, w.dlv, B, R, R, G + h->oBlv, nullptr));
    AV_TRY(gemm(h, nt(w.dmu, R, P + h->oWmu, R, w.dhpick, 2 * D, B, 2 * D, R)));
    AV_TRY(gemm(h, nt(w.dlv, R, P + h->oWlv, R, w.dhpick, 2 * D, B, 2 * D, R).plus()));
    fire_hook(h, 1 + L);
    const int32_t* const cdyn = w.compact ? w.nsrc : nullptr;
    const int32_t* const cmap = w.compact ? w.map_src : nullptr;
    if (w.compact) {
        AV_CHECK(zero_rows_dyn(st, w.dhs[0], w.nsrc, rs, 2 * D));
        AV_CHECK(pick_last_add(st, w.dhs[0], w.dhpick, w.lens_src, B, 2 * D, cmap));
    } else
    AV_CHECK(pick_last_bwd(st, w.dhs[0], w.dhpick, w.lens_src, Ss, B, 2 * D));

    cur = 0;
    for (int i = L - 1; i >= 0; --i) {
        const GruP& p = h->enc[i];
        const int In = i == 0 ? D : 2 * D;
        const bool top1 = i == L - 1 && top_one_step(h);
        const int64_t oWb = p.W + (int64_t)3 * D * In;
        if (top1) {
            AV_CHECK(gru_first_step_bwd(st, w.dhpick + D, 2 * D, w.svb, w.dgib, w.dghb, B, D, w.lens_src));
            AV_CHECK(colsum(st, w.dgib, B, 3 * D, 3 * D, G + p.bW + 3 * D, nullptr));
            AV_CHECK(colsum(st, w.dghb, B, 3 * D, 3 * D, G + p.bR + 3 * D, nullptr));
        }
        GruArgs a{};
        gru_common(h, w, a, top1 ? 1 : 2, Ss, B, 6 * D, 2 * D, w.lens_src, w.bx_enc());
        for (int d = 0; d < a.njobs; ++d) {
            GruJob& j = a.job[d];
            j.R = P + p.R + (int64_t)d * 3 * D * D; j.sv = w.e_sv[d][i]; j.hp = w.e_hp[d][i]; j.reverse = d;
            j.dh_out = w.dhs[cur] + d * D; j.dgi = w.dgi_e + d * 3 * D; j.dgh = w.dgh_e + d * 3 * D;
            j.dh0 = nullptr; j.carry = w.carry + (size_t)d * w.Bx * D;
            j.dbW = G + p.bW + d * 3 * D; j.dbR = G + p.bR + d * 3 * D;
        }
        const bool team16 = tn16_ok(h, 3 * D, D) && a.bf16 && gru_plan(a, false, h->persistent != 0).full();
        const bool g16 = team16 && !(i == 0 && use_table(h, rs, B));
        const bool gh16 = !g16 && w.dgh16_e && team16 && w.acth_e[i];
        if (g16) for (int d = 0; d < a.njobs; ++d) { a.job[d].dgi16 = w.dgi16_e + d * 3 * D; a.job[d].dgh16 = w.dgh16_e + d * 3 * D; }
        if (gh16) for (int d = 0; d < a.njobs; ++d) a.job[d].dgh16 = w.dgh16_e + d * 3 * D;
        if (!g16 && !gh16 && w.acth_e[i]) return fail(h, "internal: the forward kept this layer's h_prev as bf16 only and the backward cannot read it");
        if (w.acth_e[i]) for (int d = 0; d < a.njobs; ++d) a.job[d].hp16 = w.e_hp16[d][i];
        attach_sv16(h, a, true);
        attach_order(h, w, a, false, top1 ? 1 : 0);
        a.rowmap = cmap;
        if (cmap && i == 0) for (int d = 0; d < a.njobs; ++d) a.job[d].dgi_by_pos = 1;
        a.bwd_rs = rs_pick(h); a.spec = spec_pick(h);
        hook_fence(h);
        { Timed t(h, 2, 2.0 * a.njobs * (Ss - 1) * (double)B * D * 3 * D);
          DeviceTurn turn(h);
          AV_GRU(gru_backward(st, a, h->persistent != 0)); }
        hook_flush(h);
        const bool table = i == 0 && use_table(h, rs, B);
        const float* x = i == 0 ? w.emb_src : w.e_hs[i - 1];
        float* dx = i == 0 ? w.demb_src : w.dhs[cur ^ 1];
        if (g16) {
            const int Gc = a.njobs * 3 * D;
            if (i == 0) {
                AV_TRY(gemm_bf16_pre(h, nn(nullptr, 6 * D, P + p.W, In, dx, In, rs, In, Gc).a16(w.dgi16_e)));
                AV_CHECK(embed_scatter_add2(st, G + h->oE, w.src_tm, w.demb_src, rs, w.lead, w.demb_tgt, use_table(h, rt, B) ? 0 : rt, D, V, w.scat));
                fire_hook(h, 2 + 2 * L);
                hook_flush(h);
            }
            AV_TRY(gemm_tn16(h, tn_grad(nullptr, 6 * D, x, In, G + p.W, In, Gc, In, rs).a16(w.dgi16_e).b16((i > 0 && w.act_e[i - 1]) ? w.e_hs16[i - 1] : w.x16_kept_e(i)).depth(cdyn)));
            if (top1) AV_TRY(gemm(h, tn_grad(w.dgib, 3 * D, w.xlast, In, G + oWb, In, 3 * D, In, B)));
            for (int d = 0; d < a.njobs; ++d)
                AV_TRY(gemm_tn16(h, tn_grad(nullptr, 6 * D, w.e_hp[d][i], D, G + p.R + (int64_t)d * 3 * D * D, D, 3 * D, D, rs).a16(w.dgh16_e + d * 3 * D).b16(w.acth_e[i] ? w.e_hp16[d][i] : nullptr).depth(cdyn)));
            if (i > 0) AV_TRY(gemm_bf16_pre(h, nn(nullptr, 6 * D, P + p.W, In, dx, In, rs, In, Gc).a16(w.dgi16_e).rows(cdyn)));
            if (top1) {
                AV_TRY(gemm(h, nn(w.dgib, 3 * D, P + oWb, In, w.dxl, In, B, In, 3 * D).atomic()));
                AV_CHECK(pick_last_add(st, dx, w.dxl, w.lens_src, B, In, cmap));
            }
            cur ^= 1;
            fire_hook(h, 2 + L + (L - 1 - i));
            continue;
        }
        if (i == 0) {
            if (table) {
                const int32_t* cnt = id_groups_count(w.grp_src, rs, V); const int U = std::min(V, rs);
                AV_CHECK(rows_group_sum(st, w.dew, w.src_tm, w.dgi_e, rs, 6 * D, V, w.grp_src));
                AV_TRY(gemm(h, nn(w.dew, 6 * D, P + p.W, D, w.demb_src, D, U, D, 6 * D).rows(cnt).atomic()));
                AV_CHECK(rows_add_indexed(st, G + h->oE, w.demb_src, id_groups_uid(w.grp_src, rs, V), cnt, U, D));
            } else
            AV_TRY(gemm(h, nn(w.dgi_e, 6 * D, P + p.W, In, dx, In, rs, In, 6 * D).atomic()));
            AV_CHECK(embed_scatter_add2(st, G + h->oE, w.src_tm, w.demb_src, table ? 0 : rs, w.lead, w.demb_tgt, use_table(h, rt, B) ? 0 : rt, D, V, w.scat));
            fire_hook(h, 2 + 2 * L);
            hook_flush(h);
            if (table) {
                const int32_t* cnt = id_groups_count(w.grp_src, rs, V); const int U = std::min(V, rs);
                AV_TRY(gemm(h, tn_grad(w.dew, 6 * D, w.emb_src, D, G + p.W, D, 6 * D, D, U).depth(cnt)));
            } else
            AV_TRY(gemm(h, tn_grad(w.dgi_e, 6 * D, x, In, G + p.W, In, 6 * D, In, rs)));
        } else if (top1) {
            AV_TRY(gemm(h, tn_grad(w.dgi_e, 6 * D, x, In, G + p.W, In, 3 * D, In, rs).depth(cdyn)));
            AV_TRY(gemm(h, tn_grad(w.dgib, 3 * D, w.xlast, In, G + oWb, In, 3 * D, In, B)));
        } else
        AV_TRY(gemm(h, tn_grad(w.dgi_e, 6 * D, x, In, G + p.W, In, 6 * D, In, rs).depth(cdyn)));
        if (gh16) {
            for (int d = 0; d < a.njobs; ++d)
                AV_TRY(gemm_tn16(h, tn_grad(nullptr, 6 * D, nullptr, D, G + p.R + (int64_t)d * 3 * D * D, D, 3 * D, D, rs).a16(w.dgh16_e + d * 3 * D).b16(w.e_hp16[d][i]).depth(cdyn)));
        } else if (top1) AV_TRY(gemm(h, tn_grad(w.dgh_e, 6 * D, w.e_hp[0][i], D, G + p.R, D, 3 * D, D, rs).depth(cdyn)));
        else {
            const Pair bwd{w.dgh_e + 3 * D, w.e_hp[1][i], G + p.R + (int64_t)3 * D * D, nullptr};
            AV_TRY(gemm(h, tn_grad(w.dgh_e, 6 * D, w.e_hp[0][i], D, G + p.R, D, 3 * D, D, rs).depth(cdyn).with(&bwd)));
        }
        if (i > 0)
        AV_TRY(gemm(h, nn(w.dgi_e, 6 * D, P + p.W, In, dx, In, rs, In, top1 ? 3 * D : 6 * D).rows(cdyn).atomic()));
        if (top1) {
            AV_TRY(gemm(h, nn(w.dgib, 3 * D, P + oWb, In, w.dxl, In, B, In, 3 * D).atomic()));
            AV_CHECK(pick_last_add(st, dx, w.dxl, w.lens_src, B, In, cmap));
        }
        cur ^= 1;
        fire_hook(h, 2 + L + (L - 1 - i));
    }
    hook_flush(h);
    return 0;
}

int encode_ws(avae_ctx* h, Ws& w, const int32_t* src, int b, int t)
{
    PrepArgs p = prep_from_ws(w);
    p.src = src; p.tgt = src; p.B = b; p.Ss = t; p.St = 1; p.eos = h->cfg.eos; p.bos = h->cfg.bos;
    AV_CHECK(prep_ids(h->stream, p));
    AV_TRY(build_row_orders(h, w, b, t, 2, false));
    AV_TRY(build_compact(h, w, b, t, 0, false));
    AV_TRY(run_encoder(h, w, b, t, false));
    AV_TRY(run_latent(h, w, b, false, 0, nullptr));
    return 0;
}

}}

using namespace avae::host;

extern "C" {

int avae_get_schedule(avae_handle h, float out[3])
{
    if (!h || !out) return 1;
    Sched s = schedule(h); out[0] = s.keepwd; out[1] = s.anneal; out[2] = s.lr;
    return 0;
}

int avae_forward_backward(avae_handle h, const int32_t* src, const int32_t* tgt, int32_t B, int32_t Ss, int32_t St,
                          uint64_t seed, const uint8_t* keep_mask, const float* eps, float n_tok_global, float b_global)
{
    if (!h) return 1;
    AV_TRY(check_bound(h));
    if (B < 1 || Ss < 1 || St < 1) return fail(h, "empty batch");
    AV_CHECK(hipSetDevice(h->device));
    Ws w;
    AV_TRY(get_ws(h, w, B, Ss, St, true));
    h->B = B; h->Ss = Ss; h->St = St;
    AV_TRY(forward(h, w, src, tgt, B, Ss, St, true, seed, keep_mask, eps, n_tok_global > 0.f ? 1.f / n_tok_global : 0.f));
    AV_TRY(backward(h, w, B, Ss, St, b_global));
    if (h->persistent && !h->first_step_checked) {
        h->first_step_checked = true;
        AV_TRY(check_gru_err(h));
    }
    return 0;
}

int avae_adam_step(avae_handle h)
{
    if (!h) return 1;
    AV_TRY(check_bound(h));
    Sched sc = schedule(h);
    const double b1 = 0.9, b2 = 0.999;
    double t = (double)h->step + 1.0;
    AdamArgs a{h->P, h->G, h->M, h->Vv, h->numel, (float)(sc.lr * std::sqrt(1.0 - std::pow(b2, t)) / (1.0 - std::pow(b1, t))), 0.9f, 0.999f, 1e-8f, h->errw};
    AV_CHECK(adam_tf(h->stream, a));
    h->step += 1;
    return 0;
}

int avae_train_step(avae_handle h, const int32_t* src, const int32_t* tgt, int32_t B, int32_t Ss, int32_t St,
                    uint64_t seed, const uint8_t* keep_mask, const float* eps)
{
    AV_TRY(avae_forward_backward(h, src, tgt, B, Ss, St, seed, keep_mask, eps, 0.f, 0.f));
// ... 49 lines not shown
```

argsim_amd/csrc/ops.hip:

```cpp
#include <algorithm>
#include "kernels.h"
#include "mfma_tile.h"
#include "reduce_dev.h"
#include "sample_dev.h"

namespace avae {


__device__ __forceinline__ bool prep_kept(const PrepArgs& p, int i)
{
    const int t = i / p.B, b = i - t * p.B;
    return t == 0 || p.tgt[(size_t)b * p.St + t - 1] != p.eos;
}
__device__ __forceinline__ int block_sum256(int v, int* red)
{
    v = wave_sum(v);
    if ((threadIdx.x & 63) == 0) red[threadIdx.x >> 6] = v;
    __syncthreads();
    const int s = red[0] + red[1] + red[2] + red[3];
    __syncthreads();
    return s;
}
__global__ __launch_bounds__(256) void prep_ids_kernel(PrepArgs p, int per, int nchunks)
{
    __shared__ int red[4];
    const int tid = threadIdx.x, lane = tid & 63, B = p.B, T = p.St + 1, total = T * B;
    const int nthr = gridDim.x * 256, gid = blockIdx.x * 256 + tid;
    for (int b = gid >> 6; b < B; b += nthr >> 6) {
        int ls = 0, lt = 0;
        for (int s = lane; s < p.Ss; s += 64) ls += p.src[(size_t)b * p.Ss + s] != p.eos;
        for (int s = lane; s < p.St; s += 64) if (p.tgt[(size_t)b * p.St + s] != p.eos) lt = s + 1;
        ls = wave_sum(ls);
#pragma unroll
        for (int o = 32; o > 0; o >>= 1) lt = max(lt, __shfl_xor(lt, o));
        if (lane == 0) { p.lens_src[b] = ls; p.lens_tgt[b] = lt; }
    }
    for (int i = gid; i < p.Ss * B; i += nthr) {
        const int s = i / B, b = i - s * B;
        p.src_tm[i] = p.src[(size_t)b * p.Ss + s];
    }
    for (int i = gid; i < total; i += nthr) {
        const int t = i / B, b = i - t * B;
        p.gold[i] = t < p.St ? p.tgt[(size_t)b * p.St + t] : p.eos;
        int lead = p.bos;
        if (t > 0) {
            lead = p.tgt[(size_t)b * p.St + t - 1];
            if (p.train) {
                const int j = (t - 1) * B + b;
                const bool keep = p.keep_mask ? p.keep_mask[j] != 0 : uniform01(p.seed, 1, j) < p.keepwd;
                if (!keep) lead = 0;
            }
        }
        p.lead[i] = lead;
    }
    if (gid < 2 && p.zero2) p.zero2[gid] = 0.f;
    if ((int)blockIdx.x < nchunks) {
        const int beg = blockIdx.x * per, end = min(total, beg + per);
        int cnt = 0;
        for (int i = beg + tid; i < end; i += 256) cnt += prep_kept(p, i);
        cnt = block_sum256(cnt, red);
        if (tid == 0) p.chunk_counts[blockIdx.x] = cnt;
    }
}
__global__ __launch_bounds__(256) void prep_rank_kernel(PrepArgs p, int per)
{
    __shared__ int red[4];
    __shared__ int scan[256];
    const int tid = threadIdx.x, total = (p.St + 1) * p.B;
    int pre = 0;
    for (int c = tid; c < (int)blockIdx.x; c += 256) pre += p.chunk_counts[c];
    pre = block_sum256(pre, red);
    const int ept = per >> 8, beg = min(total, (int)blockIdx.x * per + tid * ept), end = min(total, beg + ept);
    int cnt = 0;
    for (int i = beg; i < end; ++i) cnt += prep_kept(p, i);
    scan[tid] = cnt;
    __syncthreads();
    for (int off = 1; off < 256; off <<= 1) {
        const int v = tid >= off ? scan[tid - off] : 0;
        __syncthreads();
        scan[tid] += v;
        __syncthreads();
    }
    int run = pre + scan[tid] - cnt;
    for (int i = beg; i < end; ++i) {
        const bool m = prep_kept(p, i);
        p.rank[i] = m ? run : -1;
        if (m) p.cidx[run++] = i;
    }
    if (blockIdx.x == gridDim.x - 1 && tid == 255) p.ntok[0] = pre + scan[255];
}
hipError_t prep_ids(hipStream_t st, const PrepArgs& p)
{
    const int total = (p.St + 1) * p.B;
    int per = 2048;
    while ((total + per - 1) / per > kPrepChunks) per *= 2;
    const int nchunks = (total + per - 1) / per;
    const int grid = std::max(nchunks, std::min(1024, (total + 255) / 256));
    hipLaunchKernelGGL(prep_ids_kernel, dim3(grid), dim3(256), 0, st, p, per, nchunks);
    hipLaunchKernelGGL(prep_rank_kernel, dim3(nchunks), dim3(256), 0, st, p, per);
    return hipGetLastError();
}

__global__ __launch_bounds__(256) void embed_gather_kernel(const float* __restrict__ E, const int32_t* __restrict__ ids,
                                                           float* __restrict__ out, int n, int D, int V)
{
    const int lane = threadIdx.x & 63;
    const int wpb = blockDim.x >> 6;
    for (int row = blockIdx.x * wpb + (threadIdx.x >> 6); row < n; row += gridDim.x * wpb) {
        int id = ids[row];
        id = id < 0 ? 0 : (id >= V ? V - 1 : id);
        const float4* s = reinterpret_cast<const float4*>(E + (size_t)id * D);
        float4* d = reinterpret_cast<float4*>(out + (size_t)row * D);
        for (int c = lane; c < D / 4; c += 64) d[c] = s[c];
    }
}
hipError_t embed_gather(hipStream_t st, const float* E, const int32_t* ids, float* out, int n, int D, int V)
{
    if (n <= 0) return hipSuccess;
    int blocks = min((n + 3) / 4, 2048);
    hipLaunchKernelGGL(embed_gather_kernel, dim3(blocks), dim3(256), 0, st, E, ids, out, n, D, V);
    return hipGetLastError();
}

constexpr int kScatterSeg = 32;
struct Scatter2 {
    float* dE; const int32_t* ids0; const float* dout0; int n0; const int32_t* ids1; const float* dout1; int n1; int D, V;
    int32_t* cnt;
    int32_t* cur;
    int32_t* off;
    int32_t* segoff;
    int32_t* list;
    int32_t* segid;
    int32_t* rank;
    int32_t* uid;
    int32_t* nuniq;
};
__device__ __forceinline__ int scatter_id(const Scatter2& a, int t)
{
    int id = t < a.n0 ? a.ids0[t] : a.ids1[t - a.n0];
    return id < 0 ? 0 : (id >= a.V ? a.V - 1 : id);
}
constexpr int kScatterLdsV = 12288, kScatterTok = 1024;
__global__ __launch_bounds__(256) void scatter_hist_kernel(Scatter2 a)
{
    __shared__ int lc[kScatterLdsV];
    const int n = a.n0 + a.n1, tid = threadIdx.x, t0 = blockIdx.x * kScatterTok;
    for (int i = tid; i < a.V; i += 256) lc[i] = 0;
    __syncthreads();
    for (int t = t0 + tid; t < min(n, t0 + kScatterTok); t += 256) atomicAdd(&lc[scatter_id(a, t)], 1);
    __syncthreads();
    for (int i = tid; i < a.V; i += 256) { const int c = lc[i]; if (c) atomicAdd(a.cnt + i, c); }
}
__device__ __forceinline__ int block_scan1024(int v, int* wsum )
{
    const int lane = threadIdx.x & 63, wave = threadIdx.x >> 6;
#pragma unroll
    for (int o = 1; o < 64; o <<= 1) { const int t = __shfl_up(v, o, 64); if (lane >= o) v += t; }
    if (lane == 63) wsum[wave] = v;
    __syncthreads();
    if (wave == 0) {
        int w = lane < 16 ? wsum[lane] : 0;
#pragma unroll
        for (int o = 1; o < 16; o <<= 1) { const int t = __shfl_up(w, o, 64); if (lane >= o) w += t; }
        if (lane < 16) wsum[lane] = w;
    }
    __syncthreads();
    const int r = v + (wave ? wsum[wave - 1] : 0);
    __syncthreads();
    return r;
}
__global__ __launch_bounds__(1024) void scatter_scan_kernel(Scatter2 a)
{
    __shared__ int wsum[16];
    const int tid = threadIdx.x, per = (a.V + 1023) / 1024, beg = min(a.V, tid * per), end = min(a.V, beg + per);
    int tok = 0, seg = 0, uni = 0;
    for (int i = beg; i < end; ++i) { const int c = a.cnt[i]; tok += c; seg += (c + kScatterSeg - 1) / kScatterSeg; uni += c > 0; }
    const int itok = block_scan1024(tok, wsum), iseg = block_scan1024(seg, wsum), iuni = block_scan1024(uni, wsum);
    int rt = itok - tok, rs = iseg - seg, ru = iuni - uni;
    for (int i = beg; i < end; ++i) {
        const int c = a.cnt[i];
        a.off[i] = rt; a.segoff[i] = rs;
        rt += c;
        for (int k = (c + kScatterSeg - 1) / kScatterSeg; k > 0; --k) a.segid[rs++] = i;
        if (a.rank) { a.rank[i] = c > 0 ? ru : -1; if (c > 0) a.uid[ru++] = i; }
    }
    if (tid == 1023) { a.off[a.V] = itok; a.segoff[a.V] = iseg; if (a.rank) a.nuniq[0] = iuni; }
}
__global__ __launch_bounds__(256) void scatter_fill_kernel(Scatter2 a)
{
    __shared__ int lc[kScatterLdsV];
    const int n = a.n0 + a.n1, tid = threadIdx.x, t0 = blockIdx.x * kScatterTok;
    for (int i = tid; i < a.V; i += 256) lc[i] = 0;
    __syncthreads();
    int id[kScatterTok / 256], rk[kScatterTok / 256];
#pragma unroll
    for (int q = 0; q < kScatterTok / 256; ++q) {
        const int t = t0 + tid + 256 * q;
        id[q] = -1; rk[q] = 0;
        if (t < n) { id[q] = scatter_id(a, t); rk[q] = atomicAdd(&lc[id[q]], 1); }
    }
    __syncthreads();
    for (int i = tid; i < a.V; i += 256) { const int c = lc[i]; if (c) lc[i] = atomicAdd(a.cur + i, c); }
    __syncthreads();
#pragma unroll
    for (int q = 0; q < kScatterTok / 256; ++q)
        if (id[q] >= 0) a.list[a.off[id[q]] + lc[id[q]] + rk[q]] = t0 + tid + 256 * q;
}
__global__ __launch_bounds__(256) void scatter_reduce_kernel(Scatter2 a)
{
    const int lane = threadIdx.x & 63, wpb = blockDim.x >> 6, nseg = a.segoff[a.V], D = a.D;
    for (int sg = blockIdx.x * wpb + (threadIdx.x >> 6); sg < nseg; sg += gridDim.x * wpb) {
        const int id = a.segid[sg], first = a.segoff[id], cnt = a.off[id + 1] - a.off[id];
        const int beg = a.off[id] + (sg - first) * kScatterSeg, end = min(a.off[id] + cnt, beg + kScatterSeg);
        float4 acc[2] = {make_float4(0.f, 0.f, 0.f, 0.f), make_float4(0.f, 0.f, 0.f, 0.f)};
        for (int i = beg; i < end; i += 4) {
            int t[4]; float4 v[4][2];
#pragma unroll
            for (int u = 0; u < 4; ++u) t[u] = a.list[min(i + u, end - 1)];
#pragma unroll
            for (int u = 0; u < 4; ++u) {
                const float* s = t[u] < a.n0 ? a.dout0 + (size_t)t[u] * D : a.dout1 + (size_t)(t[u] - a.n0) * D;
#pragma unroll
                for (int q = 0; q < 2; ++q) {
                    const int c = 4 * lane + 256 * q;
                    v[u][q] = (c < D && i + u < end) ? *reinterpret_cast<const float4*>(s + c) : make_float4(0.f, 0.f, 0.f, 0.f);
                }
            }
#pragma unroll
            for (int u = 0; u < 4; ++u)
#pragma unroll
                for (int q = 0; q < 2; ++q) { acc[q].x += v[u][q].x; acc[q].y += v[u][q].y; acc[q].z += v[u][q].z; acc[q].w += v[u][q].w; }
        }
        float* d = a.dE + (size_t)id * D;
        const bool alone = cnt <= kScatterSeg;
#pragma unroll
        for (int q = 0; q < 2; ++q) {
            const int c = 4 * lane + 256 * q;
            if (c >= D) continue;
            if (alone) {
                float4 v = *reinterpret_cast<float4*>(d + c);
                v.x += acc[q].x; v.y += acc[q].y; v.z += acc[q].z; v.w += acc[q].w;
                *reinterpret_cast<float4*>(d + c) = v;
            } else {
                atomicAdd(d + c, acc[q].x); atomicAdd(d + c + 1, acc[q].y); atomicAdd(d + c + 2, acc[q].z); atomicAdd(d + c + 3, acc[q].w);
            }
        }
    }
}
__global__ __launch_bounds__(256) void embed_scatter_atomic_kernel(float* __restrict__ dE, const int32_t* __restrict__ ids,
                                                                   const float* __restrict__ dout, int n, int D, int V)
{
    const int lane = threadIdx.x & 63, wpb = blockDim.x >> 6;
    for (int row = blockIdx.x * wpb + (threadIdx.x >> 6); row < n; row += gridDim.x * wpb) {
        int id = ids[row];
        id = id < 0 ? 0 : (id >= V ? V - 1 : id);
        const float* s = dout + (size_t)row * D;
        float* d = dE + (size_t)id * D;
        for (int c = lane; c < D; c += 64) atomicAdd(d + c, s[c]);
    }
}
__global__ __launch_bounds__(256) void zero_fill_kernel(uint4* __restrict__ p16, size_t n16, unsigned* __restrict__ tail, int ntail)
{
    const size_t stride = (size_t)gridDim.x * blockDim.x;
    const uint4 z = make_uint4(0u, 0u, 0u, 0u);
    for (size_t i = (size_t)blockIdx.x * blockDim.x + threadIdx.x; i < n16; i += stride) p16[i] = z;
    if (blockIdx.x == 0 && (int)threadIdx.x < ntail) tail[threadIdx.x] = 0u;
}
hipError_t zero_fill(hipStream_t st, void* p, size_t bytes)
{
    if (!bytes) return hipSuccess;
    if (((uintptr_t)p & 15) || (bytes & 3)) return hipMemsetAsync(p, 0, bytes, st);
    const size_t n16 = bytes >> 4; const int ntail = (int)((bytes & 15) >> 2);
    const size_t want = (n16 + 255) / 256;
    hipLaunchKernelGGL(zero_fill_kernel, dim3((unsigned)std::max<size_t>(1, std::min<size_t>(want, 2048))), dim3(256), 0, st,
                       reinterpret_cast<uint4*>(p), n16, reinterpret_cast<unsigned*>(p) + 4 * n16, ntail);
    return hipGetLastError();
}

hipError_t embed_scatter_add2(hipStream_t st, float* dE, const int32_t* ids0, const float* dout0, int n0, const int32_t* ids1,
                              const float* dout1, int n1, int D, int V, int32_t* scratch)
{
    const int n = n0 + n1;
    if (n <= 0) return hipSuccess;
    if (D > 512 || (D & 3) || V > kScatterLdsV) {
        if (n0 > 0) hipLaunchKernelGGL(embed_scatter_atomic_kernel, dim3(std::min((n0 + 3) / 4, 4096)), dim3(256), 0, st, dE, ids0, dout0, n0, D, V);
        if (n1 > 0) hipLaunchKernelGGL(embed_scatter_atomic_kernel, dim3(std::min((n1 + 3) / 4, 4096)), dim3(256), 0, st, dE, ids1, dout1, n1, D, V);
        return hipGetLastError();
    }
    Scatter2 a{dE, ids0, dout0, n0, ids1, dout1, n1, D, V, scratch, scratch + V, scratch + 2 * V, scratch + 3 * V + 1, scratch + 4 * V + 2, scratch + 4 * V + 2 + n, nullptr, nullptr, nullptr};
    hipError_t e = zero_fill(st, scratch, sizeof(int32_t) * 2 * (size_t)V);
    if (e != hipSuccess) return e;
    const int blocks = (n + kScatterTok - 1) / kScatterTok;
    hipLaunchKernelGGL(scatter_hist_kernel, dim3(blocks), dim3(256), 0, st, a);
    hipLaunchKernelGGL(scatter_scan_kernel, dim3(1), dim3(1024), 0, st, a);
    hipLaunchKernelGGL(scatter_fill_kernel, dim3(blocks), dim3(256), 0, st, a);
    hipLaunchKernelGGL(scatter_reduce_kernel, dim3(std::min((n / 4 + V + 3) / 4, 4096)), dim3(256), 0, st, a);
    return hipGetLastError();
}

static Scatter2 id_groups_view(const int32_t* ids, int n, int V, int32_t* scratch)
{
    int32_t* rank = scratch + 4 * (size_t)V + 2 + n + ((size_t)n / kScatterSeg + V + 1);
    return Scatter2{nullptr, ids, nullptr, n, nullptr, nullptr, 0, 0, V, scratch, scratch + V, scratch + 2 * V, scratch + 3 * V + 1,
                    scratch + 4 * V + 2, scratch + 4 * (size_t)V + 2 + n, rank, rank + V, rank + 2 * (size_t)V};
}
const int32_t* id_groups_rank(int32_t* scratch, int n, int V) { return id_groups_view(nullptr, n, V, scratch).rank; }
const int32_t* id_groups_uid(int32_t* scratch, int n, int V) { return id_groups_view(nullptr, n, V, scratch).uid; }
const int32_t* id_groups_count(int32_t* scratch, int n, int V) { return id_groups_view(nullptr, n, V, scratch).nuniq; }
bool id_groups_supported(int V) { return V <= kScatterLdsV; }
hipError_t id_groups_build(hipStream_t st, const int32_t* ids, int n, int V, int32_t* scratch, bool lists)
{
    if (n <= 0 || V > kScatterLdsV) return hipErrorInvalidValue;
    Scatter2 a = id_groups_view(ids, n, V, scratch);
    hipError_t e = zero_fill(st, scratch, sizeof(int32_t) * 2 * (size_t)V);
    if (e != hipSuccess) return e;
    const int blocks = (n + kScatterTok - 1) / kScatterTok;
    hipLaunchKernelGGL(scatter_hist_kernel, dim3(blocks), dim3(256), 0, st, a);
    hipLaunchKernelGGL(scatter_scan_kernel, dim3(1), dim3(1024), 0, st, a);
    if (lists) hipLaunchKernelGGL(scatter_fill_kernel, dim3(blocks), dim3(256), 0, st, a);
    return hipGetLastError();
}
__global__ __launch_bounds__(256) void rows_gather_ranked_kernel(float* __restrict__ dst, const float* __restrict__ src,
                                                                 const int32_t* __restrict__ ids, const int32_t* __restrict__ rank, int n, int W, int V)
{
    const int lane = threadIdx.x & 63, wpb = blockDim.x >> 6;
    for (int row = blockIdx.x * wpb + (threadIdx.x >> 6); row < n; row += gridDim.x * wpb) {
        int id = ids[row];
        id = id < 0 ? 0 : (id >= V ? V - 1 : id);
        const float4* s = reinterpret_cast<const float4*>(src + (size_t)rank[id] * W);
        float4* d = reinterpret_cast<float4*>(dst + (size_t)row * W);
        for (int c = lane; c < W / 4; c += 64) d[c] = s[c];
    }
}
__global__ __launch_bounds__(256) void rank_rows_kernel(int32_t* __restrict__ out, const int32_t* __restrict__ ids, const int32_t* __restrict__ rank, int n, int V)
{
    for (int t = blockIdx.x * 256 + threadIdx.x; t < n; t += gridDim.x * 256) {
        int id = ids[t];
        id = id < 0 ? 0 : (id >= V ? V - 1 : id);
        out[t] = rank[id];
    }
}
hipError_t rank_rows(hipStream_t st, int32_t* out, const int32_t* ids, const int32_t* rank, int n, int V)
{
    if (n <= 0) return hipSuccess;
    hipLaunchKernelGGL(rank_rows_kernel, dim3(std::min((n + 255) / 256, 2048)), dim3(256), 0, st, out, ids, rank, n, V);
    return hipGetLastError();
}
hipError_t rows_gather_ranked(hipStream_t st, float* dst, const float* src, const int32_t* ids, const int32_t* rank, int n, int W, int V)
{
    if (n <= 0) return hipSuccess;
    if (W & 3) return hipErrorInvalidValue;
    hipLaunchKernelGGL(rows_gather_ranked_kernel, dim3(std::min((n + 3) / 4, 8192)), dim3(256), 0, st, dst, src, ids, rank, n, W, V);
    return hipGetLastError();
}
__global__ __launch_bounds__(256) void scatter_reduce_wide_kernel(Scatter2 a, float* __restrict__ dst, const float* __restrict__ src, int W)
{
    const int lane = threadIdx.x & 63, wpb = blockDim.x >> 6, nseg = a.segoff[a.V], ncb = (W + 255) / 256;
    const long long items = (long long)nseg * ncb;
    for (long long it = (long long)blockIdx.x * wpb + (threadIdx.x >> 6); it < items; it += (long long)gridDim.x * wpb) {
        const int sg = (int)(it / ncb), c = (int)(it - (long long)sg * ncb) * 256 + 4 * lane;
        const int id = a.segid[sg], first = a.segoff[id], cnt = a.off[id + 1] - a.off[id];
        const int beg = a.off[id] + (sg - first) * kScatterSeg, end = min(a.off[id] + cnt, beg + kScatterSeg);
        float4 acc = make_float4(0.f, 0.f, 0.f, 0.f);
        for (int i = beg; i < end; i += 4) {
            int t[4]; float4 v[4];
#pragma unroll
            for (int u = 0; u < 4; ++u) t[u] = a.list[min(i + u, end - 1)];
#pragma unroll
            for (int u = 0; u < 4; ++u)
                v[u] = (c < W && i + u < end) ? *reinterpret_cast<const float4*>(src + (size_t)t[u] * W + c) : make_float4(0.f, 0.f, 0.f, 0.f);
#pragma unroll
            for (int u = 0; u < 4; ++u) { acc.x += v[u].x; acc.y += v[u].y; acc.z += v[u].z; acc.w += v[u].w; }
        }
        if (c >= W) continue;
        float* d = dst + (size_t)a.rank[id] * W + c;
        if (cnt <= kScatterSeg) *reinterpret_cast<float4*>(d) = acc;
        else { atomicAdd(d, acc.x); atomicAdd(d + 1, acc.y); atomicAdd(d + 2, acc.z); atomicAdd(d + 3, acc.w); }
    }
}
__global__ __launch_bounds__(256) void zero_hot_rows_kernel(Scatter2 a, float* __restrict__ dst, int W)
{
    const int lane = threadIdx.x & 63, wpb = blockDim.x >> 6;
    for (int id = blockIdx.x * wpb + (threadIdx.x >> 6); id < a.V; id += gridDim.x * wpb) {
        if (a.off[id + 1] - a.off[id] <= kScatterSeg) continue;
        float4* d = reinterpret_cast<float4*>(dst + (size_t)a.rank[id] * W);
        for (int c = lane; c < W / 4; c += 64) d[c] = make_float4(0.f, 0.f, 0.f, 0.f);
    }
}
hipError_t rows_group_sum(hipStream_t st, float* dst, const int32_t* ids, const float* src, int n, int W, int V, int32_t* scratch)
{
    if ((W & 3) || n <= 0 || V > kScatterLdsV) return hipErrorInvalidValue;
    Scatter2 a = id_groups_view(ids, n, V, scratch);
    hipLaunchKernelGGL(zero_hot_rows_kernel, dim3(std::min((V + 3) / 4, 2048)), dim3(256), 0, st, a, dst, W);
    const long long items = ((long long)n / 8 + V) * ((W + 255) / 256);
    hipLaunchKernelGGL(scatter_reduce_wide_kernel, dim3((unsigned)std::min<long long>((items + 3) / 4, 8192)), dim3(256), 0, st, a, dst, src, W);
    return hipGetLastError();
}
__global__ __launch_bounds__(256) void rows_add_indexed_kernel(float* __restrict__ dst, const float* __restrict__ src,
                                                               const int32_t* __restrict__ uid, const int32_t* __restrict__ nuniq, int n_max, int D)
{
    const int lane = threadIdx.x & 63, wpb = blockDim.x >> 6, n = min(n_max, *nuniq);
    for (int row = blockIdx.x * wpb + (threadIdx.x >> 6); row < n; row += gridDim.x * wpb) {
        const float4* s = reinterpret_cast<const float4*>(src + (size_t)row * D);
        float4* d = reinterpret_cast<float4*>(dst + (size_t)uid[row] * D);
        for (int c = lane; c < D / 4; c += 64) { float4 v = d[c]; const float4 x = s[c]; v.x += x.x; v.y += x.y; v.z += x.z; v.w += x.w; d[c] = v; }
    }
}
hipError_t rows_add_indexed(hipStream_t st, float* dst, const float* src, const int32_t* uid, const int32_t* nuniq, int n_max, int D)
{
    if (n_max <= 0) return hipSuccess;
    if (D & 3) return hipErrorInvalidValue;
    hipLaunchKernelGGL(rows_add_indexed_kernel, dim3(std::min((n_max + 3) / 4, 4096)), dim3(256), 0, st, dst, src, uid, nuniq, n_max, D);
    return hipGetLastError();
}

__global__ __launch_bounds__(256) void rows_gather_kernel(float* __restrict__ dst, const float* __restrict__ src,
                                                          const int32_t* __restrict__ idx, const int32_t* __restrict__ n_dev,
                                                          int n_max, int D, const int32_t* __restrict__ map)
{
    const int lane = threadIdx.x & 63, wpb = blockDim.x >> 6;
    const int n = min(n_max, *n_dev);
    for (int row = blockIdx.x * wpb + (threadIdx.x >> 6); row < n; row += gridDim.x * wpb) {
        const int sr = map ? map[idx[row]] : idx[row];
        const float4* s = reinterpret_cast<const float4*>(src + (size_t)sr * D);
        float4* d = reinterpret_cast<float4*>(dst + (size_t)row * D);
        for (int c = lane; c < D / 4; c += 64) d[c] = s[c];
    }
}
hipError_t rows_gather(hipStream_t st, float* dst, const float* src, const int32_t* idx, const int32_t* n_dev, int n_max, int D, const int32_t* map)
{
    if (n_max <= 0) return hipSuccess;
    hipLaunchKernelGGL(rows_gather_kernel, dim3(min((n_max + 3) / 4, 2048)), dim3(256), 0, st, dst, src, idx, n_dev, n_max, D, map);
    return hipGetLastError();
}
__global__ __launch_bounds__(256) void rows_expand_kernel(float* __restrict__ dst, const float* __restrict__ src,
                                                          const int32_t* __restrict__ rank, int rows, int D, const int32_t* __restrict__ map)
{
    const int lane = threadIdx.x & 63, wpb = blockDim.x >> 6;
    for (int row = blockIdx.x * wpb + (threadIdx.x >> 6); row < rows; row += gridDim.x * wpb) {
        int r = rank[row];
        const int dr = map ? map[row] : row;
        if (dr < 0) continue;
        float4* d = reinterpret_cast<float4*>(dst + (size_t)dr * D);
        if (r >= 0) {
            const float4* s = reinterpret_cast<const float4*>(src + (size_t)r * D);
            for (int c = lane; c < D / 4; c += 64) d[c] = s[c];
        } else {
            for (int c = lane; c < D / 4; c += 64) d[c] = make_float4(0.f, 0.f, 0.f, 0.f);
        }
    }
}
hipError_t rows_expand(hipStream_t st, float* dst, const float* src, const int32_t* rank, int rows, int D, const int32_t* map)
{
    if (rows <= 0) return hipSuccess;
    hipLaunchKernelGGL(rows_expand_kernel, dim3(min((rows + 3) / 4, 2048)), dim3(256), 0, st, dst, src, rank, rows, D, map);
    return hipGetLastError();
}

struct RowOrders { RowOrder o[3]; };
__global__ __launch_bounds__(1024) void row_order_kernel(RowOrders ro, int Breal, int B, int S, int32_t* __restrict__ steps_sum, int sum_rows)
{
    extern __shared__ int steps[];
    const RowOrder o = ro.o[blockIdx.x];
    for (int b = threadIdx.x; b < B; b += blockDim.x) steps[b] = b < Breal ? min(max(o.lens[b] + o.add, 1), S) : 1;
    __syncthreads();
    if (steps_sum && blockIdx.x == 0 && threadIdx.x < 64) {
        int v = 0;
        for (int b = threadIdx.x; b < Breal; b += 64) v += steps[b];
        for (int off = 32; off > 0; off >>= 1) v += __shfl_xor(v, off, 64);
        if (threadIdx.x == 0) { steps_sum[0] = v; steps_sum[1] = sum_rows; }
    }
    for (int b = threadIdx.x; b < B; b += blockDim.x) {
        const int mine = steps[b];
        int rank = 0;
        for (int c = 0; c < B; ++c) { const int v = steps[c]; rank += (v > mine) || (v == mine && c < b); }
        const int g = rank >> 4, w = g % o.cpj, jj = g / o.cpj;
        const int slot = (((w + (jj / o.T) * o.cpj) * o.T + jj % o.T) << 4) + (rank & 15);
        o.perm[slot] = b;
        o.slens[slot] = mine;
    }
}
hipError_t row_order(hipStream_t st, const RowOrder* orders, int n, int Breal, int B, int S, int32_t* steps_sum, int sum_rows)
{
    if (n <= 0) return hipSuccess;
    if (n > 3 || B % 16 || B < Breal || (size_t)B * 4 > 64 * 1024) return hipErrorInvalidValue;
    RowOrders ro{};
    for (int i = 0; i < n; ++i) ro.o[i] = orders[i];
    hipLaunchKernelGGL(row_order_kernel, dim3(n), dim3(1024), (size_t)B * sizeof(int), st, ro, Breal, B, S, steps_sum, sum_rows);
    return hipGetLastError();
}

__global__ __launch_bounds__(256) void row_map_local_kernel(const int32_t* __restrict__ lens, int add, int B, int32_t* __restrict__ map, int32_t* __restrict__ nact)
{
    __shared__ int scan[256];
    __shared__ int base_s;
    const int t = blockIdx.x, tid = threadIdx.x;
    if (tid == 0) base_s = 0;
    __syncthreads();
    for (int b0 = 0; b0 < B; b0 += 256) {
        const int b = b0 + tid;
        const int act = (b < B && t < lens[b] + add) ? 1 : 0;
        scan[tid] = act;
        __syncthreads();
        for (int off = 1; off < 256; off <<= 1) {
            const int v = tid >= off ? scan[tid - off] : 0;
            __syncthreads();
            scan[tid] += v;
            __syncthreads();
        }
        const int base = base_s;
        if (b < B) map[(size_t)t * B + b] = act ? base + scan[tid] - 1 : -1;
        __syncthreads();
        if (tid == 255) base_s = base + scan[255];
        __syncthreads();
    }
    if (tid == 0) nact[t] = base_s;
}
__global__ __launch_bounds__(256) void row_map_offset_kernel(int B, int S, int32_t* __restrict__ map, const int32_t* __restrict__ nact, int32_t* __restrict__ count)
{
    __shared__ int red[4];
    const int t = blockIdx.x, tid = threadIdx.x;
    int pre = 0;
    for (int c = tid; c < t; c += 256) pre += nact[c];
    pre = block_sum256(pre, red);
    __shared__ int off_s;
    if (tid == 0) off_s = pre;
    __syncthreads();
    const int off = off_s;
    for (int b = tid; b < B; b += 256) { const int v = map[(size_t)t * B + b]; if (v >= 0) map[(size_t)t * B + b] = v + off; }
    if (t == S - 1 && tid == 0) count[0] = off + nact[t];
}
hipError_t row_map(hipStream_t st, const int32_t* lens, int add, int S, int B, int32_t* map, int32_t* nact, int32_t* count)
{
    hipLaunchKernelGGL(row_map_local_kernel, dim3(S), dim3(256), 0, st, lens, add, B, map, nact);
    hipLaunchKernelGGL(row_map_offset_kernel, dim3(S), dim3(256), 0, st, B, S, map, nact, count);
    return hipGetLastError();
}
__global__ __launch_bounds__(256) void zero_rows_dyn_kernel(float4* __restrict__ X, const int32_t* __restrict__ count, int rows_max, int W4)
{
    const size_t n = (size_t)min(rows_max, *count) * W4, stride = (size_t)gridDim.x * blockDim.x;
    const float4 z = make_float4(0.f, 0.f, 0.f, 0.f);
    for (size_t i = (size_t)blockIdx.x * blockDim.x + threadIdx.x; i < n; i += stride) X[i] = z;
}
hipError_t zero_rows_dyn(hipStream_t st, float* X, const int32_t* count, int rows_max, int W)
{
    hipLaunchKernelGGL(zero_rows_dyn_kernel, dim3(2048), dim3(256), 0, st, reinterpret_cast<float4*>(X), count, rows_max, W / 4);
    return hipGetLastError();
}

__global__ __launch_bounds__(256) void pick_last_kernel(float* __restrict__ h, const float* __restrict__ hs,
                                                        const int32_t* __restrict__ lens, int B, int W, const int32_t* __restrict__ map)
{
    const int b = blockIdx.x;
    int t = max(lens[b] - 1, 0);
    const long long mrow = map ? (long long)map[(size_t)t * B + b] : (long long)t * B + b;
    float4* d = reinterpret_cast<float4*>(h + (size_t)b * W);
    if (mrow < 0 || lens[b] <= 0) { for (int c = threadIdx.x; c < W / 4; c += blockDim.x) d[c] = make_float4(0.f, 0.f, 0.f, 0.f); return; }
    const float4* s = reinterpret_cast<const float4*>(hs + (size_t)mrow * W);
    for (int c = threadIdx.x; c < W / 4; c += blockDim.x) d[c] = s[c];
}
hipError_t pick_last(hipStream_t st, float* h, const float* hs, const int32_t* lens, int B, int W, const int32_t* map)
{
    hipLaunchKernelGGL(pick_last_kernel, dim3(B), dim3(256), 0, st, h, hs, lens, B, W, map);
    return hipGetLastError();
}
__global__ __launch_bounds__(256) void pick_last16_kernel(float* __restrict__ h, const unsigned short* __restrict__ hs, const int32_t* __restrict__ lens, int B, int W,
                                                          const int32_t* __restrict__ map)
{
    const int b = blockIdx.x;
    const int t = max(lens[b] - 1, 0);
    const long long mrow = map ? (long long)map[(size_t)t * B + b] : (long long)t * B + b;
    float4* d = reinterpret_cast<float4*>(h + (size_t)b * W);
    if (mrow < 0 || lens[b] <= 0) { for (int c = threadIdx.x; c < W / 4; c += blockDim.x) d[c] = make_float4(0.f, 0.f, 0.f, 0.f); return; }
    const uint2* s = reinterpret_cast<const uint2*>(hs + (size_t)mrow * W);
    for (int c = threadIdx.x; c < W / 4; c += blockDim.x) {
        const uint2 v = s[c];
        d[c] = make_float4(__uint_as_float(v.x << 16), __uint_as_float(v.x & 0xffff0000u), __uint_as_float(v.y << 16), __uint_as_float(v.y & 0xffff0000u));
    }
}
hipError_t pick_last16(hipStream_t st, float* h, const unsigned short* hs16, const int32_t* lens, int B, int W, const int32_t* map)
{
    hipLaunchKernelGGL(pick_last16_kernel, dim3(B), dim3(256), 0, st, h, hs16, lens, B, W, map);
    return hipGetLastError();
}
__global__ __launch_bounds__(256) void pick_last_add_kernel(float* __restrict__ dhs, const float* __restrict__ d,
// ... 324 lines not shown
    if (tid == 0 && a.loss_acc) atomicAdd(a.loss_acc, s_acc);
}
int softmax_ce_form(const CeArgs& a)
{
    if (a.V & 3) return -1;
    if (a.logits16 && (!a.grad16 || !a.write_grad)) return -1;
    if (a.logits16 && a.V <= 8192 && (a.V & 7) == 0 && !a.loss_acc) return 1;
    return a.V <= 8192 ? 0 : 2;
}
hipError_t softmax_ce(hipStream_t st, const CeArgs& a)
{
    if (a.n_max <= 0) return hipSuccess;
    const int form = softmax_ce_form(a);
    if (form < 0) return hipErrorInvalidValue;
    if (form == 1)      hipLaunchKernelGGL(softmax_ce_h16_kernel, dim3(min(a.n_max, 8192)), dim3(256), 0, st, a);
    else if (form == 0) hipLaunchKernelGGL(softmax_ce_reg_kernel, dim3(min(a.n_max, 8192)), dim3(256), 0, st, a);
    else                hipLaunchKernelGGL(softmax_ce_kernel, dim3(min(a.n_max, 8192)), dim3(256), 0, st, a);
    return hipGetLastError();
}

__global__ __launch_bounds__(256) void argmax_rows_kernel(const float* __restrict__ logits, int32_t* __restrict__ pred, int n, int V)
{
    __shared__ float s_bv[4]; __shared__ int s_bi[4];
    const int tid = threadIdx.x;
    for (int row = blockIdx.x; row < n; row += gridDim.x) {
        const float* x = logits + (size_t)row * V;
        ArgFirst am;
        for (int c = tid; c < V; c += 256) am.take(x[c], c);
        am.wave_merge();
        __syncthreads();
        am.block_merge<4, false>(s_bv, s_bi);
        if (tid == 0) pred[row] = am.i;
    }
}
hipError_t argmax_rows(hipStream_t st, const float* logits, int32_t* pred, int n, int V)
{
    if (n <= 0) return hipSuccess;
    hipLaunchKernelGGL(argmax_rows_kernel, dim3(min(n, 4096)), dim3(256), 0, st, logits, pred, n, V);
    return hipGetLastError();
}

__global__ __launch_bounds__(256) void sample_rows_kernel(const float* __restrict__ logits, int n, int V, int t, SampleParams sp,
                                                          const int32_t* __restrict__ lead, int eos,
                                                          int32_t* __restrict__ pred, float* __restrict__ logp)
{
    __shared__ unsigned s_sel[258];
    __shared__ float s_pick[5 * 4];
    const int tid = threadIdx.x;
    const uint64_t key = sample_key(sp.seed);
    for (int row = blockIdx.x; row < n; row += gridDim.x) {
        if (lead && t > 0 && lead[row] == eos) {
            if (tid == 0) { pred[row] = eos; if (logp) logp[row] = 0.f; }
            continue;
        }
        const float* x = logits + (size_t)row * V;
        unsigned thr = 0;
        if (sp.top_k > 0 && sp.top_k < V)
            thr = kth_largest_key([&](auto f) { for (int c = tid; c < V; c += 256) f(order_key(x[c])); }, (unsigned)sp.top_k, s_sel);
        Pick p = pick_kept([&](auto f) { for (int c = tid; c < V; c += 256) { const float l = x[c]; if (l == l) f(c, l); } },
                           thr, sp.inv_t, sp.noise != 0, key, sample_base(row, t));
        p.wave_merge();
        __syncthreads();
        p.block_merge<4>(s_pick);
        if (tid == 0) {
            pred[row] = p.token();
            if (logp) logp[row] = p.none() ? __int_as_float(0x7fc00000) : p.logp();
        }
    }
}
hipError_t sample_rows(hipStream_t st, const float* logits, int n, int V, int t, const SampleParams& sp, const int32_t* lead, int eos,
                       int32_t* pred, float* logp)
{
    if (n <= 0) return hipSuccess;
    if (V < 1 || V > (1 << 20) || t < 0 || t >= (1 << 20) || sp.top_k < 0) return hipErrorInvalidValue;
    hipLaunchKernelGGL(sample_rows_kernel, dim3(min(n, 4096)), dim3(256), 0, st, logits, n, V, t, sp, lead, eos, pred, logp);
    return hipGetLastError();
}

constexpr int kRowRegs = 32;
template <bool kReg>
__global__ __launch_bounds__(256) void sample_rows_p_kernel(const float* __restrict__ logits, int n, int V, int t, SampleParams sp, float top_p,
                                                            const int32_t* __restrict__ lead, int eos,
                                                            int32_t* __restrict__ pred, float* __restrict__ logp, int32_t* __restrict__ nkept)
{
    __shared__ unsigned s_sel[258];
    __shared__ unsigned long long s_mass[260];
    __shared__ float s_pick[5 * 4], s_mx[4];
    const int tid = threadIdx.x, lane = tid & 63, wave = tid >> 6;
    const uint64_t key = sample_key(sp.seed);
    for (int row = blockIdx.x; row < n; row += gridDim.x) {
        if (lead && t > 0 && lead[row] == eos) {
            if (tid == 0) { pred[row] = eos; if (logp) logp[row] = 0.f; if (nkept) nkept[row] = 0; }
            continue;
        }
        const float* x = logits + (size_t)row * V;
        [[maybe_unused]] float lv[kReg ? kRowRegs : 1];
        [[maybe_unused]] unsigned long long wt[kReg ? kRowRegs : 1];
        if constexpr (kReg) {
#pragma unroll
            for (int i = 0; i < kRowRegs; ++i) { const int c = tid + i * 256; lv[i] = c < V ? x[c] : __int_as_float(0x7fc00000); }
        }
        auto each = [&](auto f) {
            if constexpr (kReg) {
#pragma unroll
                for (int i = 0; i < kRowRegs; ++i) if (lv[i] == lv[i]) f(i, tid + i * 256, lv[i]);
            } else {
                for (int c = tid; c < V; c += 256) { const float l = x[c]; if (l == l) f(0, c, l); }
            }
        };
        unsigned thr = 0;
        if (sp.top_k > 0 && sp.top_k < V)
            thr = kth_largest_key([&](auto f) { each([&](int, int, float l) { f(order_key(l)); }); }, (unsigned)sp.top_k, s_sel);
        float mx = -INFINITY;
        each([&](int, int, float l) { if (order_key(l) >= thr) mx = fmaxf(mx, l * sp.inv_t); });
        mx = wave_max(mx);
        if (lane == 0) s_mx[wave] = mx;
        __syncthreads();
        mx = fmaxf(fmaxf(s_mx[0], s_mx[1]), fmaxf(s_mx[2], s_mx[3]));
        if constexpr (kReg) {
#pragma unroll
            for (int i = 0; i < kRowRegs; ++i) wt[i] = mass_weight(lv[i] * sp.inv_t, mx);
        }
        unsigned nk = 0;
        thr = mass_threshold_key([&](auto f) {
            each([&](int i, int, float l) {
                const unsigned k = order_key(l);
                if (k < thr) return;
                if constexpr (kReg) f(k, wt[i]); else f(k, mass_weight(l * sp.inv_t, mx));
            });
        }, top_p, s_mass, &nk);
        Pick p = pick_kept([&](auto f) { each([&](int, int c, float l) { f(c, l); }); }, thr, sp.inv_t, true, key, sample_base(row, t));
        p.wave_merge();
        p.block_merge<4>(s_pick);
        if (tid == 0) {
            pred[row] = p.token();
            if (logp) logp[row] = p.none() ? __int_as_float(0x7fc00000) : p.logp();
            if (nkept) nkept[row] = (int)nk;
        }
        __syncthreads();
    }
}
hipError_t sample_rows_p(hipStream_t st, const float* logits, int n, int V, int t, const SampleParams& sp, float top_p, const int32_t* lead,
                         int eos, int32_t* pred, float* logp, int32_t* nkept)
{
    if (n <= 0) return hipSuccess;
    if (V < 1 || V > (1 << 20) || t < 0 || t >= (1 << 20) || sp.top_k < 0 || !sp.noise || !(top_p > 0.f && top_p < 1.f)) return hipErrorInvalidValue;
    if (V <= kRowRegs * 256)
        hipLaunchKernelGGL(sample_rows_p_kernel<true>, dim3(min(n, 4096)), dim3(256), 0, st, logits, n, V, t, sp, top_p, lead, eos, pred, logp, nkept);
    else
        hipLaunchKernelGGL(sample_rows_p_kernel<false>, dim3(min(n, 4096)), dim3(256), 0, st, logits, n, V, t, sp, top_p, lead, eos, pred, logp, nkept);
    return hipGetLastError();
}

__global__ __launch_bounds__(256) void colsum_kernel(const float* __restrict__ X, int M, int N, int ldx,
                                                     float* __restrict__ out, const int32_t* __restrict__ m_dev, int chunk)
{
    __shared__ float sh[4][64];
    if (m_dev) M = min(M, *m_dev);
    const int c = blockIdx.x * 64 + (threadIdx.x & 63), rl = threadIdx.x >> 6;
    const int r0 = blockIdx.y * chunk, r1 = min(M, r0 + chunk);
    float s0 = 0.f, s1 = 0.f, s2 = 0.f, s3 = 0.f;
    if (c < N) {
        int r = r0 + rl;
        for (; r + 12 < r1; r += 16) {
            s0 += X[(size_t)r * ldx + c]; s1 += X[(size_t)(r + 4) * ldx + c];
            s2 += X[(size_t)(r + 8) * ldx + c]; s3 += X[(size_t)(r + 12) * ldx + c];
        }
        for (; r < r1; r += 4) s0 += X[(size_t)r * ldx + c];
    }
    sh[rl][threadIdx.x & 63] = (s0 + s1) + (s2 + s3);
    __syncthreads();
    if (rl == 0 && c < N && r0 < r1) atomicAdd(out + c, (sh[0][threadIdx.x] + sh[1][threadIdx.x]) + (sh[2][threadIdx.x] + sh[3][threadIdx.x]));
}
hipError_t colsum(hipStream_t st, const float* X, int M, int N, int ldx, float* out, const int32_t* m_dev)
{
    if (M <= 0 || N <= 0) return hipSuccess;
    const int gx = (N + 63) / 64, want = std::max(1, 1024 / gx);
    int chunk = std::max(16, (M + want - 1) / want);
    chunk = (chunk + 3) & ~3;
    hipLaunchKernelGGL(colsum_kernel, dim3(gx, (M + chunk - 1) / chunk), dim3(256), 0, st, X, M, N, ldx, out, m_dev, chunk);
    return hipGetLastError();
}

__global__ __launch_bounds__(256) void add3_kernel(float* __restrict__ out, const float* __restrict__ a, const float* __restrict__ b,
                                                   const float* __restrict__ c, int64_t n)
{
    for (int64_t i = (int64_t)blockIdx.x * blockDim.x + threadIdx.x; i < n; i += (int64_t)gridDim.x * blockDim.x)
        out[i] = a[i] + (b ? b[i] : 0.f) + (c ? c[i] : 0.f);
}
hipError_t add3(hipStream_t st, float* out, const float* a, const float* b, const float* c, int64_t n)
{
    hipLaunchKernelGGL(add3_kernel, dim3((unsigned)((n + 255) / 256 < 2048 ? (n + 255) / 256 : 2048)), dim3(256), 0, st, out, a, b, c, n);
    return hipGetLastError();
}

__global__ __launch_bounds__(256) void adam_kernel(AdamArgs a)
{
    const int64_t n4 = a.n >> 2;
    float4* p = reinterpret_cast<float4*>(a.p);
    const float4* g = reinterpret_cast<const float4*>(a.g);
    float4* m = reinterpret_cast<float4*>(a.m);
    float4* v = reinterpret_cast<float4*>(a.v);
    const float c1 = 1.f - a.b1, c2 = 1.f - a.b2;
    if (a.skip_if && *a.skip_if != 0) return;
    for (int64_t i = (int64_t)blockIdx.x * blockDim.x + threadIdx.x; i < n4; i += (int64_t)gridDim.x * blockDim.x) {
        float4 P = p[i], G = g[i], Mv = m[i], V = v[i];
#define AVAE_ADAM1(f) Mv.f = a.b1 * Mv.f + c1 * G.f; V.f = a.b2 * V.f + c2 * G.f * G.f; P.f -= a.lr_t * Mv.f / (sqrtf(V.f) + a.eps);
        AVAE_ADAM1(x) AVAE_ADAM1(y) AVAE_ADAM1(z) AVAE_ADAM1(w)
#undef AVAE_ADAM1
        p[i] = P; m[i] = Mv; v[i] = V;
    }
    if (blockIdx.x == 0 && threadIdx.x == 0)
        for (int64_t i = n4 << 2; i < a.n; ++i) {
            float G = a.g[i];
            a.m[i] = a.b1 * a.m[i] + c1 * G; a.v[i] = a.b2 * a.v[i] + c2 * G * G;
            a.p[i] -= a.lr_t * a.m[i] / (sqrtf(a.v[i]) + a.eps);
        }
}
hipError_t adam_tf(hipStream_t st, const AdamArgs& a)
{
    hipLaunchKernelGGL(adam_kernel, dim3(2048), dim3(256), 0, st, a);
    return hipGetLastError();
}

__global__ __launch_bounds__(256) void g16_permute_kernel(float* __restrict__ dst, const float* __restrict__ src, int D, int cols, int to_g16)
{
    const int64_t total = (int64_t)3 * D * cols;
    for (int64_t i = (int64_t)blockIdx.x * blockDim.x + threadIdx.x; i < total; i += (int64_t)gridDim.x * blockDim.x) {
        int64_t row = i / cols; int col = (int)(i - row * cols);
        int ht = (int)(row / 48), rem = (int)(row % 48), u = rem / 3, gate = rem % 3;
        int64_t nat = (int64_t)gate * D + ht * 16 + u;
        if (to_g16) dst[i] = src[nat * cols + col];
        else dst[nat * cols + col] = src[i];
    }
}
hipError_t g16_permute(hipStream_t st, float* dst, const float* src, int D, int cols, bool to_g16)
{
    int64_t total = (int64_t)3 * D * cols;
    hipLaunchKernelGGL(g16_permute_kernel, dim3((unsigned)((total + 255) / 256 < 2048 ? (total + 255) / 256 : 2048)), dim3(256), 0, st, dst, src, D, cols, to_g16 ? 1 : 0);
    return hipGetLastError();
}

__global__ __launch_bounds__(1024) void finalize_losses_kernel(float* losses, const float* __restrict__ loss_samp, const int32_t* n_dev, int n_max,
                                                               const float* __restrict__ kld, int nk, float free_bits, float inv_br, float anneal)
{
    __shared__ float sh[2][1024];
    const int tid = threadIdx.x, n = min(n_max, *n_dev);
    float sg = 0.f, sk = 0.f;
    for (int i = tid; i < n; i += 1024) sg += loss_samp[i];
    for (int i = tid; i < nk; i += 1024) sk += fmaxf(kld[i], free_bits);
    sh[0][tid] = sg; sh[1][tid] = sk;
    __syncthreads();
    for (int o = 512; o > 0; o >>= 1) {
        if (tid < o) { sh[0][tid] += sh[0][tid + o]; sh[1][tid] += sh[1][tid + o]; }
        __syncthreads();
    }
    if (tid == 0) {
        const float gen = sh[0][0] / (float)max(n, 1), kl = sh[1][0] * inv_br;
        losses[0] = gen; losses[1] = kl; losses[2] = anneal * kl + gen;
    }
}
hipError_t finalize_losses(hipStream_t st, float* losses, const float* loss_samp, const int32_t* n_dev, int n_max,
                           const float* kld, int nk, float free_bits, float inv_br, float anneal)
{
    hipLaunchKernelGGL(finalize_losses_kernel, dim3(1), dim3(1024), 0, st, losses, loss_samp, n_dev, n_max, kld, nk, free_bits, inv_br, anneal);
    return hipGetLastError();
}

}
```

Measured before the change: 16020 sentences/sec.

## Fuse encoder/decoder id-group builds, row gathers, bias colsums, and batch loss loads

Result: no change. 16090 sentences/sec, median of 6 (+0.4%).

```diff
diff --git a/argsim_amd/csrc/ctx.h b/argsim_amd/csrc/ctx.h
--- a/argsim_amd/csrc/ctx.h
+++ b/argsim_amd/csrc/ctx.h
@@ -63,6 +63,8 @@
     int bf16_nt8 = 1;
     int bf16_direct = 0;
     int gru_spec = 2;
+    int groups2_last = 0;
+    int id_groups2 = 1;
     int gru_ring = 1;
     int bwd_rs = 2;
     int knn_chunk = 0;
@@ -168,6 +170,7 @@
     int32_t* scat;
     int32_t *grp_src, *grp_tgt;
     int32_t *tokrow_src, *tokrow_tgt;
+    bool groups2 = false;
     float* xbuf; size_t xbuf_floats;
     int32_t *ord_perm[3], *ord_slens[3]; int ord_T[3], ord_cpj[3]; bool ord_ok[3];
     int32_t *map_src, *nact_src, *nsrc; bool compact;
diff --git a/argsim_amd/csrc/handle.cpp b/argsim_amd/csrc/handle.cpp
--- a/argsim_amd/csrc/handle.cpp
+++ b/argsim_amd/csrc/handle.cpp
@@ -245,6 +245,7 @@
     if (!strcmp(key, "shared_device")) { h->shared_device = value != 0; return 0; }
     if (!strcmp(key, "gru_spec")) { h->gru_spec = value; return 0; }
     if (!strcmp(key, "gru_ring")) { h->gru_ring = value != 0; return 0; }
+    if (!strcmp(key, "id_groups2")) { h->id_groups2 = value != 0; return 0; }
     if (!strcmp(key, "bf16_nt8")) { h->bf16_nt8 = value != 0; return 0; }
     if (!strcmp(key, "logits16")) { h->logits16 = value != 0; return 0; }
     if (!strcmp(key, "bf16_direct")) { h->bf16_direct = value != 0; return 0; }
diff --git a/argsim_amd/csrc/hooks.cpp b/argsim_amd/csrc/hooks.cpp
--- a/argsim_amd/csrc/hooks.cpp
+++ b/argsim_amd/csrc/hooks.cpp
@@ -198,6 +198,7 @@
     } else if (o == "embed_gather") AV_CHECK(embed_gather(st, F(0), I(1), F(2), (int)i[0], (int)i[1], (int)i[2]));
     else if (o == "embed_scatter_add2") AV_CHECK(embed_scatter_add2(st, F(0), I(1), F(2), (int)i[0], I(3), F(4), (int)i[1], (int)i[2], (int)i[3], I(5)));
     else if (o == "id_groups_build") AV_CHECK(id_groups_build(st, I(0), (int)i[0], (int)i[1], I(1), i[2] != 0));
+    else if (o == "id_groups_build2") AV_CHECK(id_groups_build2(st, I(0), (int)i[0], I(1), I(2), (int)i[1], I(3), (int)i[2], i[3] != 0, I(4), I(5)));
     else if (o == "rank_rows") AV_CHECK(rank_rows(st, I(0), I(1), I(2), (int)i[0], (int)i[1]));
     else if (o == "rows_gather_ranked") AV_CHECK(rows_gather_ranked(st, F(0), F(1), I(2), I(3), (int)i[0], (int)i[1], (int)i[2]));
     else if (o == "rows_group_sum") AV_CHECK(rows_group_sum(st, F(0), I(1), F(2), (int)i[0], (int)i[1], (int)i[2], I(3)));
@@ -219,14 +220,37 @@
     else if (o == "latent_fwd") AV_CHECK(latent_fwd(st, F(0), F(1), F(2), F(3), F(4), F(5), (int)i[0], (int)i[1], (uint64_t)i[2], f[0], F(6)));
     else if (o == "latent_bwd") AV_CHECK(latent_bwd(st, F(0), F(1), F(2), F(3), F(4), F(5), (int)i[0], (int)i[1], f[0], f[1]));
     else if (o == "colsum") AV_CHECK(colsum(st, F(0), (int)i[0], (int)i[1], (int)i[2], F(1), I(2)));
+    else if (o == "colsum_multi") {
+        ColsumProblem cs[kColsumMulti];
+        const int n = (int)i[0];
+        for (int k = 0; k < std::min(std::max(n, 0), kColsumMulti); ++k) cs[k] = ColsumProblem{F(2 * k), (int)i[1 + 3 * k], (int)i[2 + 3 * k], (int)i[3 + 3 * k], F(2 * k + 1)};
+        AV_CHECK(colsum_multi(st, cs, n));
+    }
     else if (o == "add3") AV_CHECK(add3(st, F(0), F(1), F(2), F(3), i[0]));
     else if (o == "finalize_losses") AV_CHECK(finalize_losses(st, F(0), F(1), I(2), (int)i[0], F(3), (int)i[1], f[0], f[1], f[2]));
+    else if (o == "finalize_losses_serial") AV_CHECK(finalize_losses(st, F(0), F(1), I(2), (int)i[0], F(3), (int)i[1], f[0], f[1], f[2], true));
     else if (o == "adam_tf") {
         const AdamArgs a{F(0), F(1), F(2), F(3), i[0], f[0], f[1], f[2], f[3], static_cast<const int*>(p[4])};
         AV_CHECK(adam_tf(st, a));
     } else if (o == "g16_permute") AV_CHECK(g16_permute(st, F(0), F(1), (int)i[0], (int)i[1], i[2] != 0));
     else if (o == "gru_first_step_fwd") AV_CHECK(gru_first_step_fwd(st, F(0), F(1), F(2), (int)i[0], F(3), (int)i[1], (int)i[2], I(4)));
     else if (o == "gru_first_step_bwd") AV_CHECK(gru_first_step_bwd(st, F(0), (int)i[0], F(1), F(2), F(3), (int)i[1], (int)i[2], I(4)));
+    else if (o == "last_step_tables") {
+        if (h->B < 1) return fail(h, "avae_debug_op: last_step_tables: no training forward has run on this handle");
+        Ws w;
+        AV_TRY(get_ws(h, w, h->B, h->Ss, h->St, true));
+        const int D = h->cfg.dim_emb, V = h->cfg.dim_tgt, rs = h->Ss * h->B, rt = (h->St + 1) * h->B;
+        if (!host::use_table(h, rs, h->B) || !host::use_table(h, rt, h->B)) return fail(h, "avae_debug_op: last_step_tables: a first layer of that step was not table-fed");
+        auto copy = [&](void* dst, const void* src, size_t bytes) { return dst ? hipMemcpyAsync(dst, src, bytes, hipMemcpyDeviceToDevice, st) : hipSuccess; };
+        AV_CHECK(copy(p[0], w.tokrow_src, sizeof(int32_t) * rs));
+        AV_CHECK(copy(p[1], w.tokrow_tgt, sizeof(int32_t) * rt));
+        AV_CHECK(copy(p[2], w.ew, sizeof(float) * std::min(V, rt) * 3 * D));
+        AV_CHECK(copy(p[3], w.emb_src, sizeof(float) * std::min(V, rs) * D));
+        AV_CHECK(copy(p[4], w.emb_tgt, sizeof(float) * std::min(V, rt) * D));
+        AV_CHECK(copy(p[5], w.grp_src, sizeof(int32_t) * id_groups_ints(rs, V)));
+        AV_CHECK(copy(p[6], w.grp_tgt, sizeof(int32_t) * id_groups_ints(rt, V)));
+        if (p[7]) AV_CHECK(hipMemcpyAsync(p[7], &h->groups2_last, sizeof(int), hipMemcpyHostToDevice, st));
+    }
     else return fail(h, "avae_debug_op: no such launcher: " + o);
     return 0;
 }
diff --git a/argsim_amd/csrc/kernels.h b/argsim_amd/csrc/kernels.h
--- a/argsim_amd/csrc/kernels.h
+++ b/argsim_amd/csrc/kernels.h
@@ -137,6 +137,9 @@
 bool id_groups_supported(int V);
 inline size_t id_groups_ints(size_t n, size_t V) { return 4 * V + 2 + n + (n / 32 + V + 1) + 2 * V + 4; }
 hipError_t id_groups_build(hipStream_t st, const int32_t* ids, int n, int V, int32_t* scratch, bool lists);
+hipError_t id_groups_build2(hipStream_t st, const int32_t* ids_a, int n_a, int32_t* scratch_a, const int32_t* ids_b, int n_b, int32_t* scratch_b,
+                            int V, bool lists, int32_t* tokrow_a, int32_t* tokrow_b);
+bool id_groups2_takes(int n_a, int n_b);
 const int32_t* id_groups_rank(int32_t* scratch, int n, int V);
 const int32_t* id_groups_uid(int32_t* scratch, int n, int V);
 const int32_t* id_groups_count(int32_t* scratch, int n, int V);
@@ -148,6 +151,8 @@
 struct RowOrder { const int32_t* lens; int add, T, cpj; int32_t* perm; int32_t* slens; };
 hipError_t row_order(hipStream_t st, const RowOrder* orders, int n, int Breal, int B, int S, int32_t* steps_sum = nullptr, int sum_rows = 0);
 hipError_t rows_gather(hipStream_t st, float* dst, const float* src, const int32_t* idx, const int32_t* n_dev, int n_max, int D, const int32_t* map = nullptr);
+hipError_t rows_gather2(hipStream_t st, const float* src, int D, float* dst0, const int32_t* idx0, const int32_t* n0_dev, int n0_max,
+                        float* dst1, const int32_t* idx1, const int32_t* n1_dev, int n1_max);
 hipError_t rows_expand(hipStream_t st, float* dst, const float* src, const int32_t* rank, int rows, int D, const int32_t* map = nullptr);
 hipError_t pick_last(hipStream_t st, float* h, const float* hs, const int32_t* lens, int B, int W, const int32_t* map = nullptr);
 hipError_t pick_last16(hipStream_t st, float* h, const unsigned short* hs16, const int32_t* lens, int B, int W, const int32_t* map = nullptr);
@@ -183,6 +188,9 @@
                          int eos, int32_t* pred, float* logp, int32_t* nkept);
 
 hipError_t colsum(hipStream_t st, const float* X, int M, int N, int ldx, float* out, const int32_t* m_dev);
+struct ColsumProblem { const float* X; int M, N, ld; float* out; };
+constexpr int kColsumMulti = 8;
+hipError_t colsum_multi(hipStream_t st, const ColsumProblem* probs, int n);
 hipError_t add3(hipStream_t st, float* out, const float* a, const float* b, const float* c, int64_t n);
 hipError_t zero_fill(hipStream_t st, void* p, size_t bytes);
 
@@ -354,6 +362,6 @@
 hipError_t g16_permute(hipStream_t st, float* dst, const float* src, int D, int cols, bool to_g16);
 
 hipError_t finalize_losses(hipStream_t st, float* losses, const float* loss_samp, const int32_t* n_dev, int n_max,
-                           const float* kld, int nk, float free_bits, float inv_br, float anneal);
+                           const float* kld, int nk, float free_bits, float inv_br, float anneal, bool serial = false);
 
 }
diff --git a/argsim_amd/csrc/model.cpp b/argsim_amd/csrc/model.cpp
--- a/argsim_amd/csrc/model.cpp
+++ b/argsim_amd/csrc/model.cpp
@@ -414,8 +414,10 @@
         const bool top1 = i == L - 1 && top_one_step(h);
         if (i == 0 && table) {
             const int32_t* cnt = id_groups_count(w.grp_src, rs, V);
+            if (!w.groups2) {
             AV_CHECK(id_groups_build(h->stream, w.src_tm, rs, V, w.grp_src, save));
             AV_CHECK(rows_gather(h->stream, w.emb_src, h->P + h->oE, id_groups_uid(w.grp_src, rs, V), cnt, std::min(V, rs), D));
+            }
             AV_TRY(gemm(h, nt(w.emb_src, D, h->P + p.W, D, w.ew, 6 * D, std::min(V, rs), 6 * D, D).biased(h->P + p.bW).rows(cnt)));
         } else if (i > 0 && w.act_e[i - 1]) {
             AV_TRY(gemm_bf16_pre(h, nt(nullptr, In, h->P + p.W, In, w.e_gi[i], 6 * D, rs, top1 ? 3 * D : 6 * D, In).a16(w.e_hs16[i - 1]).biased(h->P + p.bW).rows(cdyn)));
@@ -425,8 +427,9 @@
         GruArgs a{};
         gru_common(h, w, a, top1 ? 1 : 2, Ss, B, 6 * D, 2 * D, w.lens_src, w.bx_enc());
         const bool table0 = i == 0 && table, indirect = table0 && gru_plan(a, true, h->persistent != 0).form == GruForm::team;
-        if (indirect) AV_CHECK(rank_rows(h->stream, w.tokrow_src, w.src_tm, id_groups_rank(w.grp_src, rs, V), rs, V));
-        else if (table0) AV_CHECK(rows_gather_ranked(h->stream, w.e_gi[0], w.ew, w.src_tm, id_groups_rank(w.grp_src, rs, V), rs, 6 * D, V));
+        if (table0 && w.groups2 && !indirect) return fail(h, "internal: the token rows were built for a first encoder layer that does not read through them");
+        if (indirect && !w.groups2) AV_CHECK(rank_rows(h->stream, w.tokrow_src, w.src_tm, id_groups_rank(w.grp_src, rs, V), rs, V));
+        else if (table0 && !indirect) AV_CHECK(rows_gather_ranked(h->stream, w.e_gi[0], w.ew, w.src_tm, id_groups_rank(w.grp_src, rs, V), rs, 6 * D, V));
         for (int d = 0; d < a.njobs; ++d) {
             GruJob& j = a.job[d];
             j.gi = (indirect ? w.ew : w.e_gi[i]) + d * 3 * D;
@@ -491,8 +494,10 @@
         if (i == 0 && ids0) {
             const int V = h->cfg.dim_tgt;
             const int32_t* cnt = id_groups_count(w.grp_tgt, rt, V);
+            if (!w.groups2) {
             AV_CHECK(id_groups_build(h->stream, ids0, rt, V, w.grp_tgt, save));
             AV_CHECK(rows_gather(h->stream, w.emb_tgt, h->P + h->oE, id_groups_uid(w.grp_tgt, rt, V), cnt, std::min(V, rt), D));
+            }
             AV_TRY(gemm(h, nt(w.emb_tgt, D, h->P + p.W, D, w.ew, 3 * D, std::min(V, rt), 3 * D, D).biased(h->P + p.bW).rows(cnt)));
         } else if (i == 0 && share_rows) {
             AV_TRY(gemm(h, nt(x, D, h->P + p.W, D, w.d_gi[0], 3 * D, share_n, 3 * D, D).biased(h->P + p.bW)));
@@ -505,8 +510,9 @@
         gru_common(h, w, a, 1, T, B, 3 * D, D, nullptr, compact ? w.Bx : 0);
         GruJob& j = a.job[0];
         const bool table0 = i == 0 && ids0, indirect = table0 && gru_plan(a, true, h->persistent != 0).form == GruForm::team;
-        if (indirect) AV_CHECK(rank_rows(h->stream, w.tokrow_tgt, ids0, id_groups_rank(w.grp_tgt, rt, h->cfg.dim_tgt), rt, h->cfg.dim_tgt));
-        else if (table0) AV_CHECK(rows_gather_ranked(h->stream, w.d_gi[0], w.ew, ids0, id_groups_rank(w.grp_tgt, rt, h->cfg.dim_tgt), rt, 3 * D, h->cfg.dim_tgt));
+        if (table0 && w.groups2 && !indirect) return fail(h, "internal: the token rows were built for a first decoder layer that does not read through them");
+        if (indirect && !w.groups2) AV_CHECK(rank_rows(h->stream, w.tokrow_tgt, ids0, id_groups_rank(w.grp_tgt, rt, h->cfg.dim_tgt), rt, h->cfg.dim_tgt));
+        else if (table0 && !indirect) AV_CHECK(rows_gather_ranked(h->stream, w.d_gi[0], w.ew, ids0, id_groups_rank(w.grp_tgt, rt, h->cfg.dim_tgt), rt, 3 * D, h->cfg.dim_tgt));
         j.gi = indirect ? w.ew : w.d_gi[i]; j.gi_rows = indirect ? w.tokrow_tgt : nullptr;
         if (i == 0 && share_rows) j.gi_rows = share_rows;
         j.R = h->P + p.R; j.bR = h->P + p.bR;
@@ -531,6 +537,22 @@
     return 0;
 }
 
+static int build_groups2(avae_ctx* h, Ws& w, int B, int Ss, int T, bool train)
+{
+    const int D = h->cfg.dim_emb, V = h->cfg.dim_tgt, rs = Ss * B, rt = T * B;
+    w.groups2 = false; h->groups2_last = 0;
+    if (!h->id_groups2 || !train || !use_table(h, rs, B) || !use_table(h, rt, B) || !id_groups2_takes(rs, rt)) return 0;
+    GruArgs e{}, d{};
+    gru_common(h, w, e, 2, Ss, B, 6 * D, 2 * D, w.lens_src, w.bx_enc());
+    gru_common(h, w, d, 1, T, B, 3 * D, D, nullptr, w.compact_d ? w.Bx : 0);
+    if (gru_plan(e, true, h->persistent != 0).form != GruForm::team || gru_plan(d, true, h->persistent != 0).form != GruForm::team) return 0;
+    AV_CHECK(id_groups_build2(h->stream, w.src_tm, rs, w.grp_src, w.lead, rt, w.grp_tgt, V, true, w.tokrow_src, w.tokrow_tgt));
+    AV_CHECK(rows_gather2(h->stream, h->P + h->oE, D, w.emb_src, id_groups_uid(w.grp_src, rs, V), id_groups_count(w.grp_src, rs, V), std::min(V, rs),
+                          w.emb_tgt, id_groups_uid(w.grp_tgt, rt, V), id_groups_count(w.grp_tgt, rt, V), std::min(V, rt)));
+    w.groups2 = true; h->groups2_last = 1;
+    return 0;
+}
+
 static int forward(avae_ctx* h, Ws& w, const int32_t* src, const int32_t* tgt, int B, int Ss, int St, bool train,
             uint64_t seed, const uint8_t* keep_mask, const float* eps, float inv_n)
 {
@@ -543,6 +565,7 @@
     AV_CHECK(prep_ids(h->stream, p));
     AV_TRY(build_row_orders(h, w, B, Ss, T, true));
     AV_TRY(build_compact(h, w, B, Ss, T, train));
+    AV_TRY(build_groups2(h, w, B, Ss, T, train));
     AV_TRY(run_encoder(h, w, B, Ss, train));
     AV_TRY(run_latent(h, w, B, train, seed, eps));
     AV_TRY(gemm(h, nn(w.z, R, h->P + h->oWex, D, w.h0, D, B, D, R).biased(h->P + h->oBex).batch_rows()));
@@ -677,7 +700,6 @@
     AV_CHECK(add3(st, w.dh0sum, w.dh0, L > 1 ? w.dh0 + (size_t)B * D : nullptr, L > 2 ? w.dh0 + (size_t)2 * B * D : nullptr, (int64_t)B * D));
     for (int i = 3; i < L; ++i) AV_CHECK(add3(st, w.dh0sum, w.dh0sum, w.dh0 + (size_t)i * B * D, nullptr, (int64_t)B * D));
     AV_TRY(gemm(h, tn_grad(w.z, R, w.dh0sum, D, G + h->oWex, D, R, D, B)));
-    AV_CHECK(colsum(st, w.dh0sum, B, D, D, G + h->oBex, nullptr));
     AV_TRY(gemm(h, nt(w.dh0sum, D, P + h->oWex, D, w.dz, R, B, R, D)));
     float bg = b_global > 0.f ? b_global : (float)B;
     AV_CHECK(latent_bwd(st, w.dz, w.mu, w.lv, w.eps, w.dmu, w.dlv, B, R, sc.anneal * h->cfg.kl_beta / (bg * R), h->cfg.free_bits));
@@ -685,10 +707,19 @@
         const Pair dlv{w.hpick, w.dlv, G + h->oWlv, nullptr};
         AV_TRY(gemm(h, tn_grad(w.hpick, 2 * D, w.dmu, R, G + h->oWmu, R, 2 * D, R, B).with(&dlv)));
     }
-    AV_CHECK(colsum(st, w.dmu, B, R, R, G + h->oBmu, nullptr));
-    AV_CHECK(colsum(st, w.dlv, B, R, R, G + h->oBlv, nullptr));
     AV_TRY(gemm(h, nt(w.dmu, R, P + h->oWmu, R, w.dhpick, 2 * D, B, 2 * D, R)));
     AV_TRY(gemm(h, nt(w.dlv, R, P + h->oWlv, R, w.dhpick, 2 * D, B, 2 * D, R).plus()));
+    {
+        ColsumProblem cs[5] = {{w.dh0sum, B, D, D, G + h->oBex}, {w.dmu, B, R, R, G + h->oBmu}, {w.dlv, B, R, R, G + h->oBlv}};
+        int ncs = 3;
+        if (top_one_step(h)) {
+            const GruP& p = h->enc[L - 1];
+            AV_CHECK(gru_first_step_bwd(st, w.dhpick + D, 2 * D, w.svb, w.dgib, w.dghb, B, D, w.lens_src));
+            cs[ncs++] = ColsumProblem{w.dgib, B, 3 * D, 3 * D, G + p.bW + 3 * D};
+            cs[ncs++] = ColsumProblem{w.dghb, B, 3 * D, 3 * D, G + p.bR + 3 * D};
+        }
+        AV_CHECK(colsum_multi(st, cs, ncs));
+    }
     fire_hook(h, 1 + L);
     const int32_t* const cdyn = w.compact ? w.nsrc : nullptr;
     const int32_t* const cmap = w.compact ? w.map_src : nullptr;
@@ -704,11 +735,6 @@
         const int In = i == 0 ? D : 2 * D;
         const bool top1 = i == L - 1 && top_one_step(h);
         const int64_t oWb = p.W + (int64_t)3 * D * In;
-        if (top1) {
-            AV_CHECK(gru_first_step_bwd(st, w.dhpick + D, 2 * D, w.svb, w.dgib, w.dghb, B, D, w.lens_src));
-            AV_CHECK(colsum(st, w.dgib, B, 3 * D, 3 * D, G + p.bW + 3 * D, nullptr));
-            AV_CHECK(colsum(st, w.dghb, B, 3 * D, 3 * D, G + p.bR + 3 * D, nullptr));
-        }
         GruArgs a{};
         gru_common(h, w, a, top1 ? 1 : 2, Ss, B, 6 * D, 2 * D, w.lens_src, w.bx_enc());
         for (int d = 0; d < a.njobs; ++d) {
diff --git a/argsim_amd/csrc/ops.hip b/argsim_amd/csrc/ops.hip
--- a/argsim_amd/csrc/ops.hip
+++ b/argsim_amd/csrc/ops.hip
@@ -141,6 +141,7 @@
     return id < 0 ? 0 : (id >= a.V ? a.V - 1 : id);
 }
 constexpr int kScatterLdsV = 12288, kScatterTok = 1024;
+constexpr int kGroups2Tok = 32768;
 __global__ __launch_bounds__(256) void scatter_hist_kernel(Scatter2 a)
 {
     __shared__ int lc[kScatterLdsV];
@@ -168,6 +169,27 @@
     const int r = v + (wave ? wsum[wave - 1] : 0);
     __syncthreads();
     return r;
+}
+__device__ __forceinline__ void block_scan1024x3(int& v0, int& v1, int& v2, int& t0, int& t1, int& t2, int (*wsum)[16] )
+{
+    const int lane = threadIdx.x & 63, wave = threadIdx.x >> 6;
+#pragma unroll
+    for (int o = 1; o < 64; o <<= 1) {
+        const int a = __shfl_up(v0, o, 64), b = __shfl_up(v1, o, 64), c = __shfl_up(v2, o, 64);
+        if (lane >= o) { v0 += a; v1 += b; v2 += c; }
+    }
+    if (lane == 63) { wsum[0][wave] = v0; wsum[1][wave] = v1; wsum[2][wave] = v2; }
+    __syncthreads();
+    if (wave < 3) {
+        int w = lane < 16 ? wsum[wave][lane] : 0;
+#pragma unroll
+        for (int o = 1; o < 16; o <<= 1) { const int t = __shfl_up(w, o, 64); if (lane >= o) w += t; }
+        if (lane < 16) wsum[wave][lane] = w;
+    }
+    __syncthreads();
+    if (wave) { v0 += wsum[0][wave - 1]; v1 += wsum[1][wave - 1]; v2 += wsum[2][wave - 1]; }
+    t0 = wsum[0][15]; t1 = wsum[1][15]; t2 = wsum[2][15];
+    __syncthreads();
 }
 __global__ __launch_bounds__(1024) void scatter_scan_kernel(Scatter2 a)
 {
@@ -320,6 +342,80 @@
     if (lists) hipLaunchKernelGGL(scatter_fill_kernel, dim3(blocks), dim3(256), 0, st, a);
     return hipGetLastError();
 }
+struct Groups2 { Scatter2 s[2]; int32_t* tokrow[2]; int lists; };
+constexpr int kGroups2Batch = 8;
+__device__ __forceinline__ int groups2_id(const Scatter2& a, int t)
+{
+    const int id = a.ids0[t];
+    return id < 0 ? 0 : (id >= a.V ? a.V - 1 : id);
+}
+__global__ __launch_bounds__(1024) void id_groups2_kernel(Groups2 g)
+{
+    __shared__ int lc[kScatterLdsV];
+    __shared__ int wsum[3][16];
+    const Scatter2& a = g.s[blockIdx.x];
+    int32_t* const tokrow = g.tokrow[blockIdx.x];
+    const int tid = threadIdx.x, n = a.n0, V = a.V;
+    for (int i = tid; i < V; i += 1024) lc[i] = 0;
+    __syncthreads();
+    for (int t0 = tid; t0 < n; t0 += 1024 * kGroups2Batch) {
+        int id[kGroups2Batch];
+#pragma unroll
+        for (int u = 0; u < kGroups2Batch; ++u) id[u] = groups2_id(a, min(t0 + 1024 * u, n - 1));
+#pragma unroll
+        for (int u = 0; u < kGroups2Batch; ++u) if (t0 + 1024 * u < n) atomicAdd(&lc[id[u]], 1);
+    }
+    __syncthreads();
+    int tok0 = 0, seg0 = 0, uni0 = 0;
+    for (int base = 0; base < V; base += 1024) {
+        const int i = base + tid, c = i < V ? lc[i] : 0, sg = (c + kScatterSeg - 1) / kScatterSeg, un = c > 0;
+        int itok = c, iseg = sg, iuni = un, ttok, tseg, tuni;
+        block_scan1024x3(itok, iseg, iuni, ttok, tseg, tuni, wsum);
+        if (i < V) {
+            const int rt = tok0 + itok - c, ru = uni0 + iuni - un;
+            int rs = seg0 + iseg - sg;
+            a.cnt[i] = c; a.cur[i] = g.lists ? c : 0;
+            a.off[i] = rt; a.segoff[i] = rs;
+            lc[i] = rt;
+            for (int k = sg; k > 0; --k) a.segid[rs++] = i;
+            a.rank[i] = c > 0 ? ru : -1;
+            if (c > 0) a.uid[ru] = i;
+        }
+        tok0 += ttok; seg0 += tseg; uni0 += tuni;
+    }
+    if (tid == 0) { a.off[V] = tok0; a.segoff[V] = seg0; a.nuniq[0] = uni0; }
+    if (!g.lists && !tokrow) return;
+    __syncthreads();
+    for (int t0 = tid; t0 < n; t0 += 1024 * kGroups2Batch) {
+        int id[kGroups2Batch], slot[kGroups2Batch], row[kGroups2Batch];
+#pragma unroll
+        for (int u = 0; u < kGroups2Batch; ++u) id[u] = groups2_id(a, min(t0 + 1024 * u, n - 1));
+#pragma unroll
+        for (int u = 0; u < kGroups2Batch; ++u) {
+            slot[u] = (g.lists && t0 + 1024 * u < n) ? atomicAdd(&lc[id[u]], 1) : 0;
+            row[u] = tokrow ? a.rank[id[u]] : 0;
+        }
+#pragma unroll
+        for (int u = 0; u < kGroups2Batch; ++u) {
+            const int t = t0 + 1024 * u;
+            if (t >= n) continue;
+            if (g.lists) a.list[slot[u]] = t;
+            if (tokrow) tokrow[t] = row[u];
+        }
+    }
+}
+bool id_groups2_takes(int n_a, int n_b) { return std::max(n_a, n_b) <= kGroups2Tok; }
+hipError_t id_groups_build2(hipStream_t st, const int32_t* ids_a, int n_a, int32_t* scratch_a, const int32_t* ids_b, int n_b, int32_t* scratch_b,
+                            int V, bool lists, int32_t* tokrow_a, int32_t* tokrow_b)
+{
+    if (n_a < 0 || n_b < 0 || (n_a == 0 && n_b == 0) || V < 1 || V > kScatterLdsV) return hipErrorInvalidValue;
+    Groups2 g{}; int k = 0;
+    if (n_a > 0) { g.s[k] = id_groups_view(ids_a, n_a, V, scratch_a); g.tokrow[k++] = tokrow_a; }
+    if (n_b > 0) { g.s[k] = id_groups_view(ids_b, n_b, V, scratch_b); g.tokrow[k++] = tokrow_b; }
+    g.lists = lists ? 1 : 0;
+    hipLaunchKernelGGL(id_groups2_kernel, dim3(k), dim3(1024), 0, st, g);
+    return hipGetLastError();
+}
 __global__ __launch_bounds__(256) void rows_gather_ranked_kernel(float* __restrict__ dst, const float* __restrict__ src,
                                                                  const int32_t* __restrict__ ids, const int32_t* __restrict__ rank, int n, int W, int V)
 {
@@ -431,6 +527,28 @@
 {
     if (n_max <= 0) return hipSuccess;
     hipLaunchKernelGGL(rows_gather_kernel, dim3(min((n_max + 3) / 4, 2048)), dim3(256), 0, st, dst, src, idx, n_dev, n_max, D, map);
+    return hipGetLastError();
+}
+__global__ __launch_bounds__(256) void rows_gather2_kernel(float* __restrict__ dst0, const int32_t* __restrict__ idx0, const int32_t* __restrict__ n0_dev, int n0_max,
+                                                           float* __restrict__ dst1, const int32_t* __restrict__ idx1, const int32_t* __restrict__ n1_dev, int n1_max,
+                                                           const float* __restrict__ src, int D)
+{
+    const int lane = threadIdx.x & 63, wpb = blockDim.x >> 6;
+    float* const dst = blockIdx.y ? dst1 : dst0;
+    const int32_t* const idx = blockIdx.y ? idx1 : idx0;
+    const int n = blockIdx.y ? min(n1_max, *n1_dev) : min(n0_max, *n0_dev);
+    for (int row = blockIdx.x * wpb + (threadIdx.x >> 6); row < n; row += gridDim.x * wpb) {
+        const float4* s = reinterpret_cast<const float4*>(src + (size_t)idx[row] * D);
+        float4* d = reinterpret_cast<float4*>(dst + (size_t)row * D);
+        for (int c = lane; c < D / 4; c += 64) d[c] = s[c];
+    }
+}
+hipError_t rows_gather2(hipStream_t st, const float* src, int D, float* dst0, const int32_t* idx0, const int32_t* n0_dev, int n0_max,
+                        float* dst1, const int32_t* idx1, const int32_t* n1_dev, int n1_max)
+{
+    if (n0_max <= 0 || n1_max <= 0 || (D & 3)) return hipErrorInvalidValue;
+    hipLaunchKernelGGL(rows_gather2_kernel, dim3(min((std::max(n0_max, n1_max) + 3) / 4, 2048), 2), dim3(256), 0, st,
+                       dst0, idx0, n0_dev, n0_max, dst1, idx1, n1_dev, n1_max, src, D);
     return hipGetLastError();
 }
 __global__ __launch_bounds__(256) void rows_expand_kernel(float* __restrict__ dst, const float* __restrict__ src,
@@ -1061,13 +1179,11 @@
     return hipGetLastError();
 }
 
-__global__ __launch_bounds__(256) void colsum_kernel(const float* __restrict__ X, int M, int N, int ldx,
-                                                     float* __restrict__ out, const int32_t* __restrict__ m_dev, int chunk)
+__device__ __forceinline__ void colsum_block(const float* __restrict__ X, int M, int N, int ldx, float* __restrict__ out, int chunk, int bx, int by)
 {
     __shared__ float sh[4][64];
-    if (m_dev) M = min(M, *m_dev);
-    const int c = blockIdx.x * 64 + (threadIdx.x & 63), rl = threadIdx.x >> 6;
-    const int r0 = blockIdx.y * chunk, r1 = min(M, r0 + chunk);
+    const int c = bx * 64 + (threadIdx.x & 63), rl = threadIdx.x >> 6;
+    const int r0 = by * chunk, r1 = min(M, r0 + chunk);
     float s0 = 0.f, s1 = 0.f, s2 = 0.f, s3 = 0.f;
     if (c < N) {
         int r = r0 + rl;
@@ -1081,13 +1197,43 @@
     __syncthreads();
     if (rl == 0 && c < N && r0 < r1) atomicAdd(out + c, (sh[0][threadIdx.x] + sh[1][threadIdx.x]) + (sh[2][threadIdx.x] + sh[3][threadIdx.x]));
 }
+__global__ __launch_bounds__(256) void colsum_kernel(const float* __restrict__ X, int M, int N, int ldx,
+                                                     float* __restrict__ out, const int32_t* __restrict__ m_dev, int chunk)
+{
+    if (m_dev) M = min(M, *m_dev);
+    colsum_block(X, M, N, ldx, out, chunk, blockIdx.x, blockIdx.y);
+}
+static int colsum_chunk(int M, int N)
+{
+    const int gx = (N + 63) / 64, want = std::max(1, 1024 / gx);
+    return (std::max(16, (M + want - 1) / want) + 3) & ~3;
+}
 hipError_t colsum(hipStream_t st, const float* X, int M, int N, int ldx, float* out, const int32_t* m_dev)
 {
     if (M <= 0 || N <= 0) return hipSuccess;
-    const int gx = (N + 63) / 64, want = std::max(1, 1024 / gx);
-    int chunk = std::max(16, (M + want - 1) / want);
-    chunk = (chunk + 3) & ~3;
+    const int gx = (N + 63) / 64, chunk = colsum_chunk(M, N);
     hipLaunchKernelGGL(colsum_kernel, dim3(gx, (M + chunk - 1) / chunk), dim3(256), 0, st, X, M, N, ldx, out, m_dev, chunk);
+    return hipGetLastError();
+}
+struct ColsumMulti { ColsumProblem p[kColsumMulti]; int chunk[kColsumMulti]; };
+__global__ __launch_bounds__(256) void colsum_multi_kernel(ColsumMulti a)
+{
+    const ColsumProblem& p = a.p[blockIdx.y];
+    const int chunk = a.chunk[blockIdx.y], gx = (p.N + 63) / 64, gy = (p.M + chunk - 1) / chunk;
+    if ((int)blockIdx.x >= gx * gy) return;
+    colsum_block(p.X, p.M, p.N, p.ld, p.out, chunk, blockIdx.x % gx, blockIdx.x / gx);
+}
+hipError_t colsum_multi(hipStream_t st, const ColsumProblem* probs, int n)
+{
+    if (n < 1 || n > kColsumMulti || !probs) return hipErrorInvalidValue;
+    ColsumMulti a{}; int blocks = 0;
+    for (int k = 0; k < n; ++k) {
+        const ColsumProblem& p = probs[k];
+        if (p.M <= 0 || p.N <= 0 || p.ld < p.N || !p.X || !p.out) return hipErrorInvalidValue;
+        a.p[k] = p; a.chunk[k] = colsum_chunk(p.M, p.N);
+        blocks = std::max(blocks, ((p.N + 63) / 64) * ((p.M + a.chunk[k] - 1) / a.chunk[k]));
+    }
+    hipLaunchKernelGGL(colsum_multi_kernel, dim3(blocks, n), dim3(256), 0, st, a);
     return hipGetLastError();
 }
 
@@ -1150,14 +1296,31 @@
     return hipGetLastError();
 }
 
+template <int kBatch>
 __global__ __launch_bounds__(1024) void finalize_losses_kernel(float* losses, const float* __restrict__ loss_samp, const int32_t* n_dev, int n_max,
                                                                const float* __restrict__ kld, int nk, float free_bits, float inv_br, float anneal)
 {
     __shared__ float sh[2][1024];
     const int tid = threadIdx.x, n = min(n_max, *n_dev);
     float sg = 0.f, sk = 0.f;
-    for (int i = tid; i < n; i += 1024) sg += loss_samp[i];
-    for (int i = tid; i < nk; i += 1024) sk += fmaxf(kld[i], free_bits);
+    if (kBatch == 1) {
+        for (int i = tid; i < n; i += 1024) sg += loss_samp[i];
+        for (int i = tid; i < nk; i += 1024) sk += fmaxf(kld[i], free_bits);
+    } else {
+        float v[kBatch];
+        for (int i = tid; i < nk; i += 1024 * kBatch) {
+#pragma unroll
+            for (int u = 0; u < kBatch; ++u) v[u] = kld[min(i + 1024 * u, nk - 1)];
+#pragma unroll
+            for (int u = 0; u < kBatch; ++u) if (i + 1024 * u < nk) sk += fmaxf(v[u], free_bits);
+        }
+        for (int i = tid; i < n; i += 1024 * kBatch) {
+#pragma unroll
+            for (int u = 0; u < kBatch; ++u) v[u] = loss_samp[min(i + 1024 * u, n - 1)];
+#pragma unroll
+            for (int u = 0; u < kBatch; ++u) if (i + 1024 * u < n) sg += v[u];
+        }
+    }
     sh[0][tid] = sg; sh[1][tid] = sk;
     __syncthreads();
     for (int o = 512; o > 0; o >>= 1) {
@@ -1170,10 +1333,11 @@
     }
 }
 hipError_t finalize_losses(hipStream_t st, float* losses, const float* loss_samp, const int32_t* n_dev, int n_max,
-                           const float* kld, int nk, float free_bits, float inv_br, float anneal)
-{
-    hipLaunchKernelGGL(finalize_losses_kernel, dim3(1), dim3(1024), 0, st, losses, loss_samp, n_dev, n_max, kld, nk, free_bits, inv_br, anneal);
-    return hipGetLastError();
-}
-
-}
+                           const float* kld, int nk, float free_bits, float inv_br, float anneal, bool serial)
+{
+    if (serial) hipLaunchKernelGGL(finalize_losses_kernel<1>, dim3(1), dim3(1024), 0, st, losses, loss_samp, n_dev, n_max, kld, nk, free_bits, inv_br, anneal);
+    else hipLaunchKernelGGL(finalize_losses_kernel<16>, dim3(1), dim3(1024), 0, st, losses, loss_samp, n_dev, n_max, kld, nk, free_bits, inv_br, anneal);
+    return hipGetLastError();
+}
+
+}
```
